# soycan-sim/bendy-tracer

Hardware: AMD Instinct MI355X
Metric: Msamples/s (pixels x spp / s) at 1080p (higher is better)
Workload: dtype f32; 1 GPU; C3: scene.json.gz 1920x1080x64spp Subsample::None, Config=main.rs (max_bounces 8, max_volume_bounces 32, clip 0.01..1000, volume_step 0.1, Output::Full), flat space (the reference has no lens code), seed 0x5EED; parallelism=single

## Files before the change

### bendy_tracer_amd/api.py

```python
from __future__ import annotations

import ctypes as C
import enum
import os
from dataclasses import dataclass
from typing import Optional

import numpy as np

_HERE = os.path.dirname(os.path.abspath(__file__))
LIB_PATH = os.path.join(_HERE, "libbendy_hip.so")
BT_TILE = 16


class BendyError(RuntimeError):

    def __init__(self, code, message):
        super().__init__(f"[bt_status {code}] {message}")
        self.code = code


class Output(enum.IntEnum):
    Full = 0
    Albedo = 1
    Normal = 2
    Depth = 3


class ColorSpace(enum.IntEnum):
    NONE = 0
    Normal = 1
    Linear = 2
    SRgb = 3


class Status(enum.IntEnum):
    Done = 0
    InProgress = 1


@dataclass(frozen=True)
class Subsample:
    n: int = 0

    @staticmethod
    def none():
        return Subsample(0)

    @staticmethod
    def subpixel(n):
        return Subsample(int(n))

    def subpixel_size(self):
        return 1.0 if self.n == 0 else float(np.float32(1.0) / np.float32(self.n))

    def subpixel_count(self):
        return 1 if self.n == 0 else self.n * self.n

    def __iter__(self):
        if self.n == 0:
            yield (0.0, 0.0)
            return
        w = np.float32(1.0) / np.float32(self.n)
        for c in range(self.n * self.n):
            yield (float(np.float32(c % self.n) * w), float(np.float32(c // self.n) * w))


@dataclass
class Config:
    max_bounces: int = 8
    max_volume_bounces: int = 32
    clip_min: float = 0.01
    clip_max: float = 1000.0
    volume_step: float = 0.1
    chunks_x: int = 4
    chunks_y: int = 2
    output: Output = Output.Full


@dataclass
class RenderConfig:
    subsample: Subsample = Subsample(0)
    samples: int = 64
    output: Optional[Output] = None
    max_bounces: Optional[int] = None
    max_volume_bounces: Optional[int] = None
    volume_step: Optional[float] = None

    @staticmethod
    def with_samples(samples):
        return RenderConfig(samples=samples)

    @staticmethod
    def with_samples_subsample(samples, subsample):
        return RenderConfig(samples=samples, subsample=subsample)


class _CConfig(C.Structure):
    _fields_ = [("max_bounces", C.c_uint32), ("max_volume_bounces", C.c_uint32), ("clip_min", C.c_float),
                ("clip_max", C.c_float), ("volume_step", C.c_float), ("chunks_x", C.c_uint32),
                ("chunks_y", C.c_uint32), ("output", C.c_int32)]


class _CRenderConfig(C.Structure):
    _fields_ = [("subsample_n", C.c_uint32), ("samples", C.c_uint32), ("has_output", C.c_int32),
                ("output", C.c_int32), ("has_max_bounces", C.c_int32), ("max_bounces", C.c_uint32),
                ("has_max_volume_bounces", C.c_int32), ("max_volume_bounces", C.c_uint32),
                ("has_volume_step", C.c_int32), ("volume_step", C.c_float), ("sample_base", C.c_uint32)]


class Stats(C.Structure):
    _fields_ = [("samples", C.c_uint64), ("segments", C.c_uint64), ("pixels", C.c_uint64), ("kernel_ms", C.c_float),
                ("lens_steps", C.c_uint64), ("slices", C.c_uint32), ("launches", C.c_uint32),
                ("scratch_bytes", C.c_uint64), ("parked_bytes", C.c_uint64), ("workgroups", C.c_uint32), ("packed", C.c_uint32)]


class _CTuning(C.Structure):
    _fields_ = [("slices", C.c_uint32), ("phase_vote", C.c_int32), ("scratch_cap_bytes", C.c_uint64), ("packed", C.c_int32),
                ("reserved", C.c_int32)]


class _CDenoiseParams(C.Structure):
    _fields_ = [("levels", C.c_uint32), ("sigma_color", C.c_float), ("sigma_normal", C.c_float), ("sigma_depth", C.c_float),
                ("eps_albedo", C.c_float)]


class _CAdaptiveParams(C.Structure):
    _fields_ = [("threshold", C.c_float), ("min_samples", C.c_uint32), ("max_samples", C.c_uint32), ("eps", C.c_float)]


class AdaptiveStats(C.Structure):
    _fields_ = [("active_tiles", C.c_uint32), ("tiles", C.c_uint32), ("min_count", C.c_uint32), ("max_count", C.c_uint32),
                ("pixel_samples", C.c_uint64), ("passes", C.c_uint32), ("reserved", C.c_uint32)]


class _CLens(C.Structure):
    _fields_ = [("centre", C.c_float * 3), ("rs", C.c_float), ("step", C.c_float), ("radius", C.c_float),
                ("max_steps", C.c_uint32)]


EXPORTS = [
    "bt_config_default", "bt_render_config_default", "bt_last_error", "bt_last_error_code", "bt_version", "bt_scene_load",
    "bt_scene_from_json", "bt_scene_free", "bt_scene_find_by_tag", "bt_scene_set_camera_aspect", "bt_scene_set_lens",
    "bt_scene_object_count", "bt_scene_data_count", "bt_scene_export_prims", "bt_render", "bt_render_device",
    "bt_shard_floats", "bt_render_shard_device", "bt_unshard_device", "bt_preview_device", "bt_preview",
    "bt_comm_unique_id", "bt_comm_init", "bt_comm_free", "bt_comm_rank", "bt_comm_world", "bt_allgather_shards_device",
    "bt_exchange_frame_device", "bt_scene_last_stats", "bt_tuning_default", "bt_scene_set_tuning", "bt_scene_get_tuning", "bt_scene_default", "bt_scene_to_json", "bt_scene_save", "bt_write_png",
    "bt_scene_trim", "bt_denoise_params_default", "bt_denoiser_new", "bt_denoiser_free", "bt_denoise_device",
    "bt_denoise", "bt_debug_primary_mask", "bt_debug_block_masks_device", "bt_debug_mask_key", "bt_debug_set_object",
    "bt_debug_plan_launch",
    "bt_render_guided_device", "bt_adaptive_params_default", "bt_adaptive_new", "bt_adaptive_free", "bt_adaptive_reset",
    "bt_render_adaptive_device", "bt_adaptive_poll", "bt_adaptive_counts", "bt_adaptive_errors", "bt_debug_adaptive_moments",
    "bt_adaptive_resolve_device",
]


def _load():
    if not os.path.exists(LIB_PATH):
        raise ImportError(
            f"{LIB_PATH} is missing: the HIP extension has not been built (run `python -c 'import __graft_entry__ "
            "as g; g.build()'` or `make -C bendy_tracer_amd/csrc`).  There is no CPU fallback.")
    try:
        import torch
    except ImportError:
        pass
    L = C.CDLL(LIB_PATH)
    vp, fp = C.c_void_p, C.POINTER(C.c_float)
    L.bt_last_error.restype = C.c_char_p
    L.bt_version.restype = C.c_char_p
    L.bt_config_default.argtypes = [C.POINTER(_CConfig)]
    L.bt_render_config_default.argtypes = [C.POINTER(_CRenderConfig)]
    L.bt_scene_load.restype = vp
    L.bt_scene_load.argtypes = [C.c_char_p]
    L.bt_scene_from_json.restype = vp
    L.bt_scene_from_json.argtypes = [C.c_char_p, C.c_size_t]
    L.bt_scene_free.argtypes = [vp]
    L.bt_scene_default.restype = vp
    L.bt_scene_to_json.argtypes = [vp, C.c_char_p, C.c_size_t]
    L.bt_scene_save.argtypes = [vp, C.c_char_p]
    L.bt_write_png.argtypes = [C.c_char_p, C.POINTER(C.c_uint8), C.c_uint32, C.c_uint32]
    L.bt_scene_find_by_tag.argtypes = [vp, C.c_char_p, C.POINTER(C.c_uint64)]
    L.bt_scene_set_camera_aspect.argtypes = [vp, C.c_uint64, C.c_float]
    L.bt_scene_set_lens.argtypes = [vp, C.POINTER(_CLens)]
    L.bt_scene_object_count.argtypes = [vp]
    L.bt_scene_data_count.argtypes = [vp]
    L.bt_scene_export_prims.argtypes = [vp, fp, C.c_int]
    L.bt_debug_primary_mask.argtypes = [vp, C.c_uint64, C.POINTER(_CConfig), C.POINTER(_CRenderConfig), C.c_uint32, C.c_uint32,
                                        C.c_uint32, C.c_uint32, C.c_uint32, C.POINTER(C.c_uint64), C.c_uint32]
    L.bt_debug_set_object.argtypes = [vp, C.c_uint64, fp, C.c_float]
    L.bt_debug_block_masks_device.argtypes = L.bt_debug_primary_mask.argtypes
    L.bt_debug_mask_key.argtypes = [vp, C.c_uint64, C.POINTER(_CConfig), C.POINTER(_CRenderConfig), C.c_uint32, C.c_uint32,
                                    C.c_uint32, C.c_uint32, C.c_uint32, C.POINTER(C.c_uint8), C.c_uint32]
    L.bt_debug_plan_launch.argtypes = [vp, C.c_uint64, C.POINTER(_CConfig), C.POINTER(_CRenderConfig), C.c_uint32, C.c_uint32,
                                       C.c_uint32, C.c_uint32, C.c_int32, C.c_uint32, C.c_int32, C.c_uint32, C.c_uint64,
                                       C.POINTER(Stats)]
    L.bt_render.argtypes = [vp, C.c_uint64, C.POINTER(_CConfig), C.POINTER(_CRenderConfig), fp, C.c_uint32,
                            C.c_uint32, C.c_uint64]
    L.bt_render_device.argtypes = [vp, C.c_uint64, C.POINTER(_CConfig), C.POINTER(_CRenderConfig), vp, C.c_uint32,
                                   C.c_uint32, C.c_uint64, vp]
    L.bt_render_guided_device.argtypes = [vp, C.c_uint64, C.POINTER(_CConfig), C.POINTER(_CRenderConfig), vp, vp, vp, vp,
                                          C.c_uint32, C.c_uint32, C.c_uint64, vp]
    L.bt_shard_floats.restype = C.c_size_t
    L.bt_shard_floats.argtypes = [C.c_uint32, C.c_uint32, C.c_uint32]
    L.bt_render_shard_device.argtypes = [vp, C.c_uint64, C.POINTER(_CConfig), C.POINTER(_CRenderConfig), vp,
                                         C.c_uint32, C.c_uint32, C.c_uint32, C.c_uint32, C.c_uint64, vp]
    L.bt_unshard_device.argtypes = [vp, vp, C.c_uint32, C.c_uint32, C.c_uint32, vp]
    L.bt_preview_device.argtypes = [vp, vp, C.c_uint32, C.c_uint32, C.c_uint32, C.c_int32, vp]
    L.bt_preview.argtypes = [fp, C.POINTER(C.c_uint8), C.c_uint32, C.c_uint32, C.c_uint32, C.c_int32]
    L.bt_scene_last_stats.argtypes = [vp, C.POINTER(Stats)]
    L.bt_comm_unique_id.argtypes = [C.c_void_p, C.c_size_t]
    L.bt_comm_init.restype = vp
    L.bt_comm_init.argtypes = [C.c_uint32, C.c_uint32, C.c_void_p, C.c_size_t]
    L.bt_comm_free.argtypes = [vp]
    L.bt_comm_rank.argtypes = [vp]
    L.bt_comm_world.argtypes = [vp]
    L.bt_allgather_shards_device.argtypes = [vp, vp, vp, C.c_uint32, C.c_uint32, vp]
    L.bt_exchange_frame_device.argtypes = [vp, vp, vp, vp, C.c_uint32, C.c_uint32, vp]
    L.bt_tuning_default.argtypes = [C.POINTER(_CTuning)]
    L.bt_scene_set_tuning.argtypes = [vp, C.POINTER(_CTuning)]
    L.bt_scene_get_tuning.argtypes = [vp, C.POINTER(_CTuning)]
    L.bt_scene_trim.argtypes = [vp]
    L.bt_denoise_params_default.argtypes = [C.POINTER(_CDenoiseParams)]
    L.bt_denoiser_new.restype = vp
    L.bt_denoiser_free.argtypes = [vp]
    L.bt_denoise_device.argtypes = [vp, vp, C.c_uint32, vp, C.c_uint32, vp, C.c_uint32, vp, C.c_uint32, vp, C.c_uint32,
                                    C.c_uint32, C.POINTER(_CDenoiseParams), vp]
    L.bt_denoise.argtypes = [vp, fp, C.c_uint32, fp, C.c_uint32, fp, C.c_uint32, fp, C.c_uint32, fp, C.c_uint32, C.c_uint32,
                             C.POINTER(_CDenoiseParams)]
    L.bt_adaptive_params_default.argtypes = [C.POINTER(_CAdaptiveParams)]
    L.bt_adaptive_new.restype = vp
    L.bt_adaptive_new.argtypes = [C.c_uint32, C.c_uint32]
    L.bt_adaptive_free.argtypes = [vp]
    L.bt_adaptive_reset.argtypes = [vp]
    L.bt_render_adaptive_device.argtypes = [vp, C.c_uint64, C.POINTER(_CConfig), C.POINTER(_CRenderConfig), vp,
                                            C.POINTER(_CAdaptiveParams), vp, C.c_uint32, C.c_uint32, C.c_uint64, vp]
    L.bt_adaptive_poll.argtypes = [vp, C.POINTER(AdaptiveStats)]
    L.bt_adaptive_counts.argtypes = [vp, C.POINTER(C.c_uint32), C.c_uint32]
    L.bt_adaptive_errors.argtypes = [vp, fp, C.c_uint32]
    L.bt_debug_adaptive_moments.argtypes = [vp, fp, C.c_uint32]
    L.bt_adaptive_resolve_device.argtypes = [vp, vp, vp, vp]
    return L


lib = _load()


def _check(rc):
    if rc < 0:
        raise BendyError(rc, lib.bt_last_error().decode("utf-8", "replace"))
    return rc


def _c_configs(config: Config, render: RenderConfig, sample_base: int):
    c = _CConfig(config.max_bounces, config.max_volume_bounces, config.clip_min, config.clip_max, config.volume_step,
                 config.chunks_x, config.chunks_y, int(config.output))
    r = _CRenderConfig()
    r.subsample_n = render.subsample.n
    r.samples = render.samples
    r.has_output = render.output is not None
    r.output = int(render.output) if render.output is not None else 0
    r.has_max_bounces = render.max_bounces is not None
    r.max_bounces = render.max_bounces or 0
    r.has_max_volume_bounces = render.max_volume_bounces is not None
    r.max_volume_bounces = render.max_volume_bounces or 0
    r.has_volume_step = render.volume_step is not None
    r.volume_step = render.volume_step or 0.0
    r.sample_base = sample_base
    return c, r


class Scene:

    def __init__(self, handle):
        if not handle:
            raise BendyError(lib.bt_last_error_code(), lib.bt_last_error().decode("utf-8", "replace"))
        self._h = C.c_void_p(handle)

    @classmethod
    def load(cls, path):
        return cls(lib.bt_scene_load(os.fspath(path).encode()))

    @classmethod
    def from_json(cls, text):
        data = text.encode() if isinstance(text, str) else bytes(text)
        return cls(lib.bt_scene_from_json(data, len(data)))

    @classmethod
    def default(cls):
        return cls(lib.bt_scene_default())

    def to_json(self) -> str:
        n = _check(lib.bt_scene_to_json(self._h, None, 0))
        buf = C.create_string_buffer(n + 1)
        _check(lib.bt_scene_to_json(self._h, buf, n + 1))
        return buf.value.decode()

    def save(self, path):
        _check(lib.bt_scene_save(self._h, os.fspath(path).encode()))

    def __del__(self):
        h = getattr(self, "_h", None)
        if h:
            lib.bt_scene_free(h)
            self._h = None

    def find_by_tag(self, tag) -> Optional[int]:
        ref = C.c_uint64()
        rc = lib.bt_scene_find_by_tag(self._h, tag.encode(), C.byref(ref))
        return ref.value if rc == 0 else None

    def set_camera_aspect(self, camera_ref, aspect_ratio):
        _check(lib.bt_scene_set_camera_aspect(self._h, camera_ref, aspect_ratio))

    def debug_set_object(self, object_ref, translation=None, radius=0.0):
        t = None if translation is None else (C.c_float * 3)(*[float(v) for v in translation])
        _check(lib.bt_debug_set_object(self._h, object_ref, t, float(radius)))

    def set_lens(self, centre, rs, step, radius, max_steps=4096):
        lens = _CLens((C.c_float * 3)(*[float(v) for v in centre]), rs, step, radius, max_steps)
        _check(lib.bt_scene_set_lens(self._h, C.byref(lens)))

    def clear_lens(self):
        _check(lib.bt_scene_set_lens(self._h, None))

    @property
    def object_count(self):
        return lib.bt_scene_object_count(self._h)

    @property
    def data_count(self):
        return lib.bt_scene_data_count(self._h)

    def export_prims(self):
        n = _check(lib.bt_scene_export_prims(self._h, None, 0))
        out = np.zeros(n, dtype=np.float32)
        _check(lib.bt_scene_export_prims(self._h, out.ctypes.data_as(C.POINTER(C.c_float)), n))
        return out.reshape(-1, 36)

    def set_tuning(self, **knobs):
        t = _CTuning()
        if not knobs:
            _check(lib.bt_scene_set_tuning(self._h, None))
            return
        _check(lib.bt_scene_get_tuning(self._h, C.byref(t)))
        for k, v in knobs.items():
            if not hasattr(t, k):
                raise TypeError(f"bt_tuning has no field {k!r}")
            setattr(t, k, int(v))
        _check(lib.bt_scene_set_tuning(self._h, C.byref(t)))

    def tuning(self) -> dict:
        t = _CTuning()
        _check(lib.bt_scene_get_tuning(self._h, C.byref(t)))
        return {k: getattr(t, k) for k, _ in _CTuning._fields_}

    def tuning_from_env(self, environ=None):
        env = os.environ if environ is None else environ
        names = {"BT_SLICES": "slices", "BT_PHASE_VOTE": "phase_vote", "BT_SCRATCH_CAP": "scratch_cap_bytes", "BT_PACKED": "packed"}
        knobs = {f: int(env[e]) for e, f in names.items() if env.get(e) not in (None, "", "-")}
        if knobs:
            self.set_tuning(**knobs)
        return knobs

    def trim(self):
        _check(lib.bt_scene_trim(self._h))

    def last_stats(self) -> Stats:
        st = Stats()
        _check(lib.bt_scene_last_stats(self._h, C.byref(st)))
        return st


class Buffer:

    def __init__(self, width, height, color_space=ColorSpace.SRgb, device="cuda"):
        self.width, self.height = int(width), int(height)
        self.color_space = ColorSpace(color_space)
        self.samples = 0
        self.device = device
        if device == "cpu":
            self.data = np.zeros((self.height, self.width, 4), dtype=np.float32)
            self.data[..., 3] = 1.0
        else:
            import torch
            self.data = torch.zeros((self.height, self.width, 4), dtype=torch.float32, device=device)
            self.data[..., 3] = 1.0

    @classmethod
    def new(cls, width, height, color_space=ColorSpace.SRgb, device="cuda"):
        return cls(width, height, color_space, device)

    def dimensions(self):
        return (self.width, self.height)

    def pixel_width(self):
        return float(np.float32(2.0) * (np.float32(1.0) / np.float32(self.width)))

    def pixel_height(self):
        return float(np.float32(2.0) * (np.float32(1.0) / np.float32(self.height)))

    def clear(self):
        self.data[...] = 0.0
        self.data[..., 3] = 1.0
        self.samples = 0

    def inc_samples(self, n):
        self.samples += n

    def chunks(self, chunks_x, chunks_y):
        cw = self.width // chunks_x + (1 if self.width % chunks_x else 0)
        ch = self.height // chunks_y + (1 if self.height % chunks_y else 0)
        out, oy = [], 0
        while oy < self.height:
            h = min(ch, self.height - oy)
            ox = 0
            while ox < self.width:
                w = min(cw, self.width - ox)
                out.append((ox, oy, ox + w, oy + h))
                ox += w
            oy += h
        return out

    def numpy(self):
        return self.data if self.device == "cpu" else self.data.cpu().numpy()

    def mean(self):
        return self.numpy()[..., :3] / np.float32(max(self.samples, 1))

    def preview(self):
        if self.device == "cpu":
            out = np.zeros((self.height, self.width, 4), dtype=np.uint8)
            _check(lib.bt_preview(self.data.ctypes.data_as(C.POINTER(C.c_float)),
                                  out.ctypes.data_as(C.POINTER(C.c_uint8)), self.width, self.height,
                                  max(self.samples, 1), int(self.color_space)))
            return out
        import torch
        out = torch.empty((self.height, self.width, 4), dtype=torch.uint8, device=self.data.device)
        _check(lib.bt_preview_device(self.data.data_ptr(), out.data_ptr(), self.width, self.height,
                                     max(self.samples, 1), int(self.color_space),
                                     torch.cuda.current_stream().cuda_stream))
        return out.cpu().numpy()


class Tracer:

    DEFAULT_SEED = 0x5EED

    def __init__(self, config: Optional[Config] = None):
        self.config = config or Config()

    @classmethod
    def new(cls):
        return cls()

    @classmethod
    def with_config(cls, config):
        return cls(config)

    def render(self, scene: Scene, camera: int, config: RenderConfig, buffer: Buffer, seed: Optional[int] = None,
               sample_base: Optional[int] = None) -> Status:
        seed = self.DEFAULT_SEED if seed is None else seed
        nn = config.subsample.subpixel_count()
        if sample_base is None:
            sample_base = (buffer.samples + nn - 1) // nn
        c, r = _c_configs(self.config, config, sample_base)
        if buffer.device == "cpu":
            rc = lib.bt_render(scene._h, camera, C.byref(c), C.byref(r),
                               buffer.data.ctypes.data_as(C.POINTER(C.c_float)), buffer.width, buffer.height, seed)
        else:
            import torch
            rc = lib.bt_render_device(scene._h, camera, C.byref(c), C.byref(r), buffer.data.data_ptr(), buffer.width,
                                      buffer.height, seed, torch.cuda.current_stream().cuda_stream)
        _check(rc)
        if rc == Status.InProgress:
            buffer.inc_samples(config.samples * nn)
        return Status(rc)

    def render_guided(self, scene: Scene, camera: int, config: RenderConfig, color: Buffer, albedo: Optional[Buffer] = None,
                      normal: Optional[Buffer] = None, depth: Optional[Buffer] = None, seed: Optional[int] = None,
                      sample_base: Optional[int] = None) -> Status:
        seed = self.DEFAULT_SEED if seed is None else seed
        output = config.output if config.output is not None else self.config.output
        if int(output) != int(Output.Full):
            raise BendyError(-1, f"render_guided renders Output.Full plus its guides, not output {int(output)}")
        guides = [albedo, normal, depth]
        for b in [color] + [g for g in guides if g is not None]:
            if b.device == "cpu":
                raise BendyError(-1, "render_guided needs device-resident buffers (there is no host-buffer variant)")
            if (b.width, b.height) != (color.width, color.height):
                raise BendyError(-1, f"buffer of {b.width}x{b.height} next to a {color.width}x{color.height} colour buffer")
        nn = config.subsample.subpixel_count()
        if sample_base is None:
            sample_base = (color.samples + nn - 1) // nn
        c, r = _c_configs(self.config, config, sample_base)
        import torch
        rc = lib.bt_render_guided_device(scene._h, camera, C.byref(c), C.byref(r), color.data.data_ptr(),
                                         *[g.data.data_ptr() if g is not None else None for g in guides], color.width,
                                         color.height, seed, torch.cuda.current_stream().cuda_stream)
        _check(rc)
        if rc == Status.InProgress:
            for b in [color] + [g for g in guides if g is not None]:
                b.inc_samples(config.samples * nn)
        return Status(rc)

    def render_adaptive(self, scene: Scene, camera: int, config: RenderConfig, buffer: Buffer, adaptive: "Adaptive",
                        seed: Optional[int] = None) -> Status:
        seed = self.DEFAULT_SEED if seed is None else seed
        if buffer.device == "cpu":
            raise BendyError(-1, "render_adaptive needs a device-resident buffer (there is no host-buffer variant)")
        c, r = _c_configs(self.config, config, 0)
        p = adaptive.params._c()
        import torch
        rc = _check(lib.bt_render_adaptive_device(scene._h, camera, C.byref(c), C.byref(r), adaptive._h, C.byref(p),
                                                  buffer.data.data_ptr(), buffer.width, buffer.height, seed,
                                                  torch.cuda.current_stream().cuda_stream))
        if rc == Status.Done:
            return Status.Done
        return Status(_check(lib.bt_adaptive_poll(adaptive._h, None)))

    def primary_masks(self, scene: Scene, camera: int, config: RenderConfig, width, height, slices, rank=0, world=1):
        c, r = _c_configs(self.config, config, 0)
        n = _check(lib.bt_debug_primary_mask(scene._h, camera, C.byref(c), C.byref(r), width, height, slices, rank, world,
                                             None, 0))
        out = np.zeros(n, dtype=np.uint64)
        _check(lib.bt_debug_primary_mask(scene._h, camera, C.byref(c), C.byref(r), width, height, slices, rank, world,
                                         out.ctypes.data_as(C.POINTER(C.c_uint64)), n))
        return out

    def block_masks_device(self, scene: Scene, camera: int, config: RenderConfig, width, height, slices, rank=0, world=1):
        c, r = _c_configs(self.config, config, 0)
        n = _check(lib.bt_debug_block_masks_device(scene._h, camera, C.byref(c), C.byref(r), width, height, slices, rank,
                                                   world, None, 0))
        out = np.zeros(n, dtype=np.uint64)
        _check(lib.bt_debug_block_masks_device(scene._h, camera, C.byref(c), C.byref(r), width, height, slices, rank, world,
                                               out.ctypes.data_as(C.POINTER(C.c_uint64)), n))
        return out

    def mask_key(self, scene: Scene, camera: int, config: RenderConfig, width, height, slices, rank=0, world=1) -> bytes:
        c, r = _c_configs(self.config, config, 0)
        n = _check(lib.bt_debug_mask_key(scene._h, camera, C.byref(c), C.byref(r), width, height, slices, rank, world, None, 0))
        out = (C.c_uint8 * n)()
        _check(lib.bt_debug_mask_key(scene._h, camera, C.byref(c), C.byref(r), width, height, slices, rank, world, out, n))
        return bytes(out)

    def plan_launch(self, scene: Scene, camera: int, config: RenderConfig, width, height, n_cu, rank=0, world=1, sharded=False,
                    kind=0, guides=0, alloc_limit=0) -> Stats:
        c, r = _c_configs(self.config, config, 0)
        st = Stats()
        _check(lib.bt_debug_plan_launch(scene._h, camera, C.byref(c), C.byref(r), width, height, rank, world, int(sharded),
                                        n_cu, kind, guides, alloc_limit, C.byref(st)))
        return st

    def render_shard(self, scene: Scene, camera: int, config: RenderConfig, shard, width, height, rank, world,
                     seed: Optional[int] = None, sample_base: int = 0) -> Status:
        import torch
        seed = self.DEFAULT_SEED if seed is None else seed
        c, r = _c_configs(self.config, config, sample_base)
        assert shard.numel() == shard_floats(width, height, world) and shard.dtype == torch.float32
        rc = lib.bt_render_shard_device(scene._h, camera, C.byref(c), C.byref(r), shard.data_ptr(), width, height, rank,
                                        world, seed, torch.cuda.current_stream().cuda_stream)
        return Status(_check(rc))


class Comm:

    ID_BYTES = 128

    @staticmethod
    def unique_id() -> bytes:
        buf = C.create_string_buffer(Comm.ID_BYTES)
        _check(lib.bt_comm_unique_id(buf, Comm.ID_BYTES))
        return buf.raw

    def __init__(self, rank, world, uid: bytes):
        assert len(uid) == self.ID_BYTES
        h = lib.bt_comm_init(rank, world, uid, len(uid))
        if not h:
            raise BendyError(lib.bt_last_error_code(), lib.bt_last_error().decode("utf-8", "replace"))
        self._h = C.c_void_p(h)
        self.rank, self.world = rank, world

    def close(self):
        if getattr(self, "_h", None):
            lib.bt_comm_free(self._h)
            self._h = None

    __del__ = close

    def allgather(self, shard, gathered, width, height):
        import torch
        assert gathered.numel() == self.world * shard.numel() == self.world * shard_floats(width, height, self.world)
        _check(lib.bt_allgather_shards_device(self._h, shard.data_ptr(), gathered.data_ptr(), width, height,
                                              torch.cuda.current_stream().cuda_stream))

    def exchange(self, shard, gathered, buffer: "Buffer"):
        import torch
        _check(lib.bt_exchange_frame_device(self._h, shard.data_ptr(), gathered.data_ptr(), buffer.data.data_ptr(),
                                            buffer.width, buffer.height, torch.cuda.current_stream().cuda_stream))


@dataclass
class DenoiseParams:
    levels: int = 2
    sigma_color: float = 16.0
    sigma_normal: float = 16.0
    sigma_depth: float = 1.0
    eps_albedo: float = 1e-3

    def _c(self):
        return _CDenoiseParams(int(self.levels), self.sigma_color, self.sigma_normal, self.sigma_depth, self.eps_albedo)


class Denoiser:

    def __init__(self):
        h = lib.bt_denoiser_new()
        if not h:
            raise BendyError(-1, "bt_denoiser_new failed")
        self._h = C.c_void_p(h)

    def close(self):
        if getattr(self, "_h", None):
            lib.bt_denoiser_free(self._h)
            self._h = None

    __del__ = close

    def denoise(self, color: Buffer, albedo: Optional[Buffer] = None, normal: Optional[Buffer] = None,
                depth: Optional[Buffer] = None, *, out: Optional[Buffer] = None, **params) -> Buffer:
        p = DenoiseParams(**params)
        bufs = [b for b in (albedo, normal, depth) if b is not None]
        for b in bufs + ([out] if out is not None else []):
            if (b.width, b.height) != (color.width, color.height):
                raise BendyError(-1, f"buffer of {b.width}x{b.height} next to a {color.width}x{color.height} colour buffer")
            if b.device != color.device or (color.device != "cpu" and b.data.device != color.data.device):
                raise BendyError(-1, f"buffer on {b.device} next to a colour buffer on {color.device}")
        if out is not None and any(out is b or out.data is b.data for b in [color] + bufs):
            raise BendyError(-1, "out must not be one of the inputs: the inputs are running sums, out is a mean")
        if out is None:
            out = Buffer(color.width, color.height, color.color_space, device=color.device)
        out.color_space = color.color_space

        def arg(b):
            if b is None:
                return None, 0
            if b.device == "cpu":
                return b.data.ctypes.data_as(C.POINTER(C.c_float)), b.samples
            return b.data.data_ptr(), b.samples

        args = []
        for b in (color, albedo, normal, depth):
            args += list(arg(b))
        cp = p._c()
        if color.device == "cpu":
            _check(lib.bt_denoise(self._h, *args, arg(out)[0], color.width, color.height, C.byref(cp)))
        else:
            import torch
            _check(lib.bt_denoise_device(self._h, *args, out.data.data_ptr(), color.width, color.height, C.byref(cp),
                                         torch.cuda.current_stream().cuda_stream))
        out.samples = 1
        return out


def _adaptive_defaults():
    p = _CAdaptiveParams()
    lib.bt_adaptive_params_default(C.byref(p))
    return p


@dataclass
class AdaptiveParams:
    threshold: Optional[float] = None
    min_samples: Optional[int] = None
    max_samples: Optional[int] = None
    eps: Optional[float] = None

    def __post_init__(self):
        d = _adaptive_defaults()
        for k, _ in _CAdaptiveParams._fields_:
            if getattr(self, k) is None:
                setattr(self, k, getattr(d, k))

    def _c(self):
        return _CAdaptiveParams(float(self.threshold), int(self.min_samples), int(self.max_samples), float(self.eps))


class Adaptive:

    def __init__(self, width, height, **params):
        self.params = AdaptiveParams(**params)
        self.width, self.height = int(width), int(height)
        self.tiles_x, self.tiles_y = (self.width + BT_TILE - 1) // BT_TILE, (self.height + BT_TILE - 1) // BT_TILE
        h = lib.bt_adaptive_new(self.width, self.height)
        if not h:
            raise BendyError(lib.bt_last_error_code(), lib.bt_last_error().decode("utf-8", "replace"))
        self._h = C.c_void_p(h)

    def close(self):
        if getattr(self, "_h", None):
            lib.bt_adaptive_free(self._h)
            self._h = None

    __del__ = close

    def reset(self):
        _check(lib.bt_adaptive_reset(self._h))

    def poll(self) -> AdaptiveStats:
        st = AdaptiveStats()
        _check(lib.bt_adaptive_poll(self._h, C.byref(st)))
        return st

    def counts(self):
        n = _check(lib.bt_adaptive_counts(self._h, None, 0))
        out = np.zeros(n, dtype=np.uint32)
        _check(lib.bt_adaptive_counts(self._h, out.ctypes.data_as(C.POINTER(C.c_uint32)), n))
        return out.reshape(self.tiles_y, self.tiles_x)

    def errors(self):
        n = _check(lib.bt_adaptive_errors(self._h, None, 0))
        out = np.zeros(n, dtype=np.float32)
        _check(lib.bt_adaptive_errors(self._h, out.ctypes.data_as(C.POINTER(C.c_float)), n))
        return out.reshape(self.tiles_y, self.tiles_x)

    def moments(self):
        n = _check(lib.bt_debug_adaptive_moments(self._h, None, 0))
        out = np.zeros(n, dtype=np.float32)
        _check(lib.bt_debug_adaptive_moments(self._h, out.ctypes.data_as(C.POINTER(C.c_float)), n))
        return out.reshape(self.height, self.width)

    def resolve(self, buffer: Buffer, out: Optional[Buffer] = None) -> Buffer:
        if buffer.device == "cpu":
            raise BendyError(-1, "resolve needs a device-resident buffer")
        if (buffer.width, buffer.height) != (self.width, self.height):
            raise BendyError(-1, f"buffer of {buffer.width}x{buffer.height} on an adaptive handle of {self.width}x{self.height}")
        if out is not None and (out is buffer or out.data is buffer.data):
            raise BendyError(-1, "out must not be the input: the input holds running sums, out is a mean")
        if out is None:
            out = Buffer(buffer.width, buffer.height, buffer.color_space, device=buffer.device)
        if (out.width, out.height) != (self.width, self.height) or out.device == "cpu":
            raise BendyError(-1, "out must be a device-resident buffer of the handle's size")
        out.color_space = buffer.color_space
        import torch
        _check(lib.bt_adaptive_resolve_device(self._h, buffer.data.data_ptr(), out.data.data_ptr(),
                                              torch.cuda.current_stream().cuda_stream))
        out.samples = 1
        return out


_default_denoiser = None


def denoise(color: Buffer, albedo: Optional[Buffer] = None, normal: Optional[Buffer] = None, depth: Optional[Buffer] = None,
            *, out: Optional[Buffer] = None, **params) -> Buffer:
    global _default_denoiser
    if _default_denoiser is None:
        _default_denoiser = Denoiser()
    return _default_denoiser.denoise(color, albedo, normal, depth, out=out, **params)


def write_png(path, rgba8):
    a = np.ascontiguousarray(rgba8, dtype=np.uint8)
    _check(lib.bt_write_png(os.fspath(path).encode(), a.ctypes.data_as(C.POINTER(C.c_uint8)), a.shape[1], a.shape[0]))


def shard_floats(width, height, world):
    return lib.bt_shard_floats(width, height, world)


def new_shard(width, height, world, device="cuda"):
    import torch
    s = torch.zeros(shard_floats(width, height, world), dtype=torch.float32, device=device)
    s.view(-1, 4)[:, 3] = 1.0
    return s


def unshard(gathered, buffer: Buffer, world):
    import torch
    _check(lib.bt_unshard_device(gathered.data_ptr(), buffer.data.data_ptr(), buffer.width, buffer.height, world,
                                 torch.cuda.current_stream().cuda_stream))


def tile_owner_map(width, height, world):
    tx, ty = (width + BT_TILE - 1) // BT_TILE, (height + BT_TILE - 1) // BT_TILE
    return (np.arange(tx * ty) % world).reshape(ty, tx)
```

### bendy_tracer_amd/csrc/bt_api.cpp

```cpp
#include <hip/hip_runtime.h>

#include <algorithm>
#include <cmath>
#include <cstdlib>
#include <cstdio>
#include <cstring>
#include <memory>
#include <string>

#include "../../include/bendy_hip.h"
#include "bt_internal.hpp"
#include "bt_scene.hpp"
#include "bt_types.h"
#include "bt_cull.hpp"
#include "bt_plan.hpp"

#pragma STDC FP_CONTRACT OFF

namespace {

thread_local std::string g_error;
thread_local int g_error_code = 0;
constexpr uint32_t kCounterSlots = 64;

template <class T> struct DeviceArray {
    T *ptr = nullptr;
    size_t count = 0;
    ~DeviceArray() { release(); }
    size_t bytes() const { return sizeof(T) * count; }
    void release() {
        if (ptr) (void)hipFree(ptr);
        ptr = nullptr;
        count = 0;
    }
    hipError_t allocate(size_t n) {
        release();
        hipError_t e = hipMalloc((void **)&ptr, sizeof(T) * n);
        if (e == hipSuccess) count = n;
        return e;
    }
    hipError_t upload(const std::vector<T> &src) {
        hipError_t e = allocate(src.size() ? src.size() : 1);
        count = src.size();
        if (e == hipSuccess && count) e = hipMemcpy(ptr, src.data(), sizeof(T) * count, hipMemcpyHostToDevice);
        return e;
    }
};

}

struct bt_scene {
    bt::Scene scene;
    std::string source;
    bt::FlatScene flat;
    bool flat_valid = false;
    bool device_valid = false;
    int device = -1;
    DeviceArray<BtPrim> d_prims;
    DeviceArray<BtMaterial> d_materials;
    DeviceArray<BtVolume> d_volumes;
    DeviceArray<BtLight> d_lights;
    DeviceArray<BtLightFace> d_light_faces;
    DeviceArray<BtSpherePair> d_sphere_pairs;
    DeviceArray<BtSphereRow> d_sphere_rows;
    DeviceArray<BtRectAAN> d_aan_rows;
    DeviceArray<BtRectLA> d_la_rows;
    DeviceArray<int32_t> d_other_rows;
    DeviceArray<float> d_density;
    DeviceArray<int32_t> d_lens_prims;
    bt_lens lens_prims_for{};
    bool lens_prims_valid = false;
    unsigned long long *d_counters = nullptr;
    uint32_t render_seq = 0;
    uint32_t last_slot = 0;
    DeviceArray<float> d_scratch;
    uint32_t scratch_small_streak = 0;
    btplan::Scratch plan_scratch;
    DeviceArray<uint64_t> d_block_masks;
    btcull::MaskKey masks_for{};
    uint64_t rows_generation = 0;
    DeviceArray<float> d_host_frame;
    int n_cu = 0;
    bt_tuning tuning{};
    hipEvent_t ev_start = nullptr, ev_stop = nullptr;
    bt_stats last{};
    bool lens_on = false;
    bt_lens lens{};
    bool stats_pending = false;

    bt_scene() { bt_tuning_default(&tuning); }
    void release_device_state() {
        if (d_counters) (void)hipFree(d_counters);
        if (ev_start) (void)hipEventDestroy(ev_start);
        if (ev_stop) (void)hipEventDestroy(ev_stop);
        d_counters = nullptr;
        ev_start = ev_stop = nullptr;
        stats_pending = false;
        release_buffers();
    }
    void release_buffers() {
        d_scratch.release();
        d_host_frame.release();
        d_block_masks.release();
        masks_for = btcull::MaskKey{};
        scratch_small_streak = 0;
    }
    ~bt_scene() { release_device_state(); }
};

namespace {

int ensure_flat(bt_scene *s) {
    if (s->flat_valid) return 0;
    try {
        s->flat = bt::flatten_scene(s->scene);
    } catch (const bt::Error &e) {
        return fail(e.code, e.message);
    }
    s->flat_valid = true;
    s->device_valid = false;
    s->rows_generation += 1;
    return 0;
}

std::vector<BtSphereRow> sphere_rows_of(const std::vector<BtPrim> &pr) {
    std::vector<BtSphereRow> rows;
    bool spheres_only = true;
    for (const BtPrim &R : pr) spheres_only = spheres_only && (R.kind & BT_PRIM_SHAPE_MASK) == BT_PRIM_SPHERE;
    if (spheres_only)
        for (const BtPrim &R : pr) rows.push_back(BtSphereRow{R.c.x, R.c.y, R.c.z, R.radius * R.radius});
    if (rows.size() & 1) rows.push_back(rows.back());
    return rows;
}

int ensure_device(bt_scene *s) {
    int rc = ensure_flat(s);
    if (rc) return rc;
    int dev = -1;
    BT_HIP(hipGetDevice(&dev));
    if (s->device_valid && s->device == dev) return 0;
    if (s->device >= 0 && s->device != dev) {
        (void)hipSetDevice(s->device);
        s->release_device_state();
        BT_HIP(hipSetDevice(dev));
    }
    {
        hipDeviceProp_t prop;
        BT_HIP(hipGetDeviceProperties(&prop, dev));
        s->n_cu = prop.multiProcessorCount > 0 ? prop.multiProcessorCount : 256;
    }
    BT_HIP(s->d_prims.upload(s->flat.prims));
    BT_HIP(s->d_materials.upload(s->flat.materials));
    BT_HIP(s->d_volumes.upload(s->flat.volumes));
    BT_HIP(s->d_lights.upload(s->flat.lights));
    BT_HIP(s->d_light_faces.upload(s->flat.light_faces));
    {
        std::vector<BtSpherePair> pairs;
        const std::vector<BtPrim> &pr = s->flat.prims;
        bool spheres_only = true;
        for (const BtPrim &R : pr) spheres_only = spheres_only && (R.kind & BT_PRIM_SHAPE_MASK) == BT_PRIM_SPHERE;
        if (spheres_only)
            for (size_t i = 0; i < pr.size(); i += 2) {
                const BtPrim &A = pr[i], &B = pr[i + 1 < pr.size() ? i + 1 : i];
                BtSpherePair q{};
                q.cx[0] = A.c.x; q.cy[0] = A.c.y; q.cz[0] = A.c.z; q.radius[0] = A.radius; q.object[0] = A.object;
                q.cx[1] = B.c.x; q.cy[1] = B.c.y; q.cz[1] = B.c.z; q.radius[1] = B.radius; q.object[1] = B.object;
                pairs.push_back(q);
            }
        BT_HIP(s->d_sphere_pairs.upload(pairs));
        BT_HIP(s->d_sphere_rows.upload(sphere_rows_of(pr)));
        s->rows_generation += 1;
    }
    BT_HIP(s->d_density.upload(s->flat.density));
    BT_HIP(s->d_aan_rows.upload(s->flat.aan_rows));
    BT_HIP(s->d_la_rows.upload(s->flat.la_rows));
    BT_HIP(s->d_other_rows.upload(s->flat.other_rows));
    if (!s->d_counters) {
        BT_HIP(hipMalloc((void **)&s->d_counters, kCounterSlots * 16 * sizeof(unsigned long long)));
        s->render_seq = 0;
    }
    if (!s->ev_start) BT_HIP(hipEventCreate(&s->ev_start));
    if (!s->ev_stop) BT_HIP(hipEventCreate(&s->ev_stop));
    s->device = dev;
    s->device_valid = true;
    s->lens_prims_valid = false;
    return 0;
}

std::vector<int32_t> lens_candidates(const std::vector<BtPrim> &prims, const bt_lens &lens, double reach) {
    std::vector<int32_t> rows;
    const double cx = lens.centre[0], cy = lens.centre[1], cz = lens.centre[2];
    reach *= 1.001;
    for (size_t i = 0; i < prims.size(); ++i) {
        const BtPrim &R = prims[i];
        bool near_ = true;
        if ((R.kind & BT_PRIM_SHAPE_MASK) == BT_PRIM_SPHERE) {
            const double d = std::sqrt((R.c.x - cx) * (R.c.x - cx) + (R.c.y - cy) * (R.c.y - cy) + (R.c.z - cz) * (R.c.z - cz));
            near_ = std::fabs(d - (double)R.radius) <= reach + 1e-3 * (double)R.radius;
        } else {
            const double a[3][3] = {{R.icx.x, R.icy.x, R.icz.x}, {R.icx.y, R.icy.y, R.icz.y}, {R.icx.z, R.icy.z, R.icz.z}};
            const double det = a[0][0] * (a[1][1] * a[2][2] - a[1][2] * a[2][1]) - a[0][1] * (a[1][0] * a[2][2] - a[1][2] * a[2][0]) +
                               a[0][2] * (a[1][0] * a[2][1] - a[1][1] * a[2][0]);
            if (std::isfinite(det) && std::fabs(det) > 1e-30) {
                double m[3][3];
                for (int r = 0; r < 3; ++r)
                    for (int c = 0; c < 3; ++c) {
                        const int r1 = (c + 1) % 3, r2 = (c + 2) % 3, c1 = (r + 1) % 3, c2 = (r + 2) % 3;
                        m[r][c] = (a[r1][c1] * a[r2][c2] - a[r1][c2] * a[r2][c1]) / det;
                    }
                const double hw = std::sqrt((double)R.w_sqr), hh = std::sqrt((double)R.h_sqr);
                double lx[3] = {R.ax.x, R.ax.y, R.ax.z}, ly[3] = {R.ay.x, R.ay.y, R.ay.z};
                if ((R.kind & BT_PRIM_SHAPE_MASK) == BT_PRIM_RECT_LA || (R.kind & BT_PRIM_SHAPE_MASK) == BT_PRIM_RECT_AAN)
                    for (int i = 0; i < 3; ++i) {
                        lx[i] = i == R.aa_u ? 1.0 : 0.0;
                        ly[i] = i == R.aa_v ? 1.0 : 0.0;
                    }
                double bound = 0.0;
                for (int sx = -1; sx <= 1; sx += 2)
                    for (int sy = -1; sy <= 1; sy += 2) {
                        const double l[3] = {sx * hw * lx[0] + sy * hh * ly[0], sx * hw * lx[1] + sy * hh * ly[1],
                                             sx * hw * lx[2] + sy * hh * ly[2]};
                        double wv[3];
                        for (int r = 0; r < 3; ++r) wv[r] = m[r][0] * l[0] + m[r][1] * l[1] + m[r][2] * l[2];
                        bound = std::max(bound, std::sqrt(wv[0] * wv[0] + wv[1] * wv[1] + wv[2] * wv[2]));
                    }
                const double d = std::sqrt((R.t.x - cx) * (R.t.x - cx) + (R.t.y - cy) * (R.t.y - cy) + (R.t.z - cz) * (R.t.z - cz));
                near_ = d - bound * 1.001 <= reach;
            }
        }
        if (near_) rows.push_back((int32_t)i);
    }
    return rows;
}

int fill_launch(bt_scene *s, uint64_t camera_ref, const bt_config *cfg, const bt_render_config *rc, uint32_t width,
                uint32_t height, uint64_t seed, BtLaunch &P, int &output) {
    if (!s || !cfg || !rc) return fail(BT_ERR_INVALID_ARG, "null argument");
    if (width == 0 || height == 0) return fail(BT_ERR_INVALID_ARG, "zero-sized buffer");
    int ci = s->scene.object_index(camera_ref);
    if (ci < 0) return fail(BT_ERR_INVALID_REF, "invalid object ref " + std::to_string(camera_ref));
    const bt::Object &cam = s->scene.objects[ci];
    if (cam.kind != bt::OBJ_CAMERA) return fail(BT_ERR_NOT_CAMERA, "expected a camera object");

    std::memset(&P, 0, sizeof P);
    const bt::FlatScene &f = s->flat;
    P.prims = s->d_prims.ptr;
    P.materials = s->d_materials.ptr;
    P.volumes = s->d_volumes.ptr;
    P.lights = s->d_lights.ptr;
    P.light_faces = s->d_light_faces.ptr;
    P.sphere_pairs = s->d_sphere_pairs.count ? s->d_sphere_pairs.ptr : nullptr;
    P.sphere_rows = s->d_sphere_rows.count ? s->d_sphere_rows.ptr : nullptr;
    P.density = s->d_density.ptr;
    P.n_prims = (int32_t)f.prims.size();
    P.n_materials = (int32_t)f.materials.size();
    P.n_volumes = (int32_t)f.volumes.size();
    P.n_lights = (int32_t)f.lights.size();
    P.n_light_faces = (int32_t)f.light_faces.size();
    P.n_density = (int32_t)f.density.size();
    P.any_rects = 0;
    for (const BtPrim &R : f.prims)
        if ((R.kind & BT_PRIM_SHAPE_MASK) != BT_PRIM_SPHERE) P.any_rects = 1;
    P.any_volumes = btplan::any_prim_carries_volume(f.prims) ? 1 : 0;
    P.aan_rows = s->d_aan_rows.ptr;
    P.la_rows = s->d_la_rows.ptr;
    P.n_la = (int32_t)f.la_rows.size();
    P.other_rows = s->d_other_rows.ptr;
    P.n_aan[0] = f.n_aan[0]; P.n_aan[1] = f.n_aan[1]; P.n_aan[2] = f.n_aan[2];
    P.n_other = (int32_t)f.other_rows.size();
    P.root_color = f.root_color;
    P.root_albedo = f.root_albedo;
    P.root_has_albedo = f.root_has_albedo;

    P.cam_cx = cam.world.cx; P.cam_cy = cam.world.cy; P.cam_cz = cam.world.cz; P.cam_t = cam.world.t;
    P.yfov = 2.0f * atan2f(cam.sensor_size, 2.0f * cam.focal_length);
    P.xfov = P.yfov * cam.aspect_ratio;
    P.pixel_width = 2.0f * (1.0f / (float)width);
    P.pixel_height = 2.0f * (1.0f / (float)height);
    const uint32_t n = rc->subsample_n >= 2 ? rc->subsample_n : 1;
    const float subpixel_scale = rc->subsample_n >= 2 ? 1.0f / (float)rc->subsample_n : 1.0f;
    const float umin = -0.5f * P.pixel_width * subpixel_scale, umax = 0.5f * P.pixel_width * subpixel_scale;
    const float vmin = -0.5f * P.pixel_height * subpixel_scale, vmax = 0.5f * P.pixel_height * subpixel_scale;
    P.jitter_u_lo = umin;
    P.jitter_u_scale = bt::uniform_scale(umin, umax, false);
    P.jitter_v_lo = vmin;
    P.jitter_v_scale = bt::uniform_scale(vmin, vmax, false);
    P.has_focus = cam.has_focus ? 1 : 0;
    P.focus = cam.focus;
    P.aperture = 0.5f * cam.focal_length / cam.fstop;
    BtV3 neg_z; neg_z.x = 0.0f; neg_z.y = 0.0f; neg_z.z = -1.0f;
    bt::orthonormal_pair(neg_z, P.disk_x, P.disk_y);
    P.tau_scale = bt::uniform_scale(0.0f, 6.28318530717958647692f, true);
    P.one_scale = bt::uniform_scale(0.0f, 1.0f, true);

    output = rc->has_output ? rc->output : cfg->output;
    if (output < 0 || output > 3) return fail(BT_ERR_INVALID_ARG, "invalid output mode");
    P.max_bounces = (int32_t)(rc->has_max_bounces ? rc->max_bounces : cfg->max_bounces);
    P.max_volume_bounces = (int32_t)(rc->has_max_bounces ? rc->max_bounces : cfg->max_volume_bounces);
    P.clip_min = cfg->clip_min;
    P.clip_max = cfg->clip_max;
    P.volume_step = rc->has_volume_step ? rc->volume_step : cfg->volume_step;
    if (P.any_rects && !P.any_volumes &&
        !(P.clip_min >= 0x1p-30f && P.clip_max <= 0x1p60f && f.prims.size() < 0x7fffu))
        P.any_volumes = 1;
    if (rc->samples > 0x7fffffffu / (n * n)) return fail(BT_ERR_INVALID_ARG, "samples * n^2 overflows");
    P.samples = (int32_t)rc->samples;
    P.subsample_n = (int32_t)n;
    P.sample_base = rc->sample_base;
    P.seed_lo = (uint32_t)seed;
    P.seed_hi = (uint32_t)(seed >> 32);
    P.width = width;
    P.height = height;
    P.tiles_x = btplan::tiles_across(width);
    P.tiles_x_magic = P.tiles_x == 1 ? 0xffffffffu : (uint32_t)(0x100000000ull / P.tiles_x);
    P.tiles_y = btplan::tiles_across(height);
    P.rank = 0;
    P.world = 1;
    P.sharded = 0;
    P.counters = s->d_counters;
    P.lens_on = s->lens_on ? 1 : 0;
    P.lens_c.x = s->lens.centre[0]; P.lens_c.y = s->lens.centre[1]; P.lens_c.z = s->lens.centre[2];
    P.lens_rs = s->lens.rs;
    P.lens_step = s->lens.step;
    P.lens_radius = s->lens.radius;
    P.lens_max_steps = (int32_t)s->lens.max_steps;
    P.lens_prims = nullptr;
    P.n_lens_prims = 0;
    P.lens_margin = s->lens_on ? 3.0f * s->lens.step : 0.0f;
    return 0;
}

int upload_lens_prims(bt_scene *s, BtLaunch &P) {
    if (!s->lens_on) return 0;
    if (!s->lens_prims_valid || std::memcmp(&s->lens_prims_for, &s->lens, sizeof(bt_lens)) != 0) {
        BT_HIP(s->d_lens_prims.upload(lens_candidates(s->flat.prims, s->lens, (double)s->lens.radius + (double)P.lens_margin)));
        s->lens_prims_for = s->lens;
        s->lens_prims_valid = true;
    }
    P.lens_prims = s->d_lens_prims.ptr;
    P.n_lens_prims = (int32_t)s->d_lens_prims.count;
    return 0;
}

int ensure_block_masks(bt_scene *s, BtLaunch &P, uint32_t n_blocks, hipStream_t stream) {
    btcull::MaskKey key;
    btcull::mask_key(key, P, n_blocks, s->rows_generation, (const void *)stream);
    if (!bt_mask_cache_enabled() || std::memcmp(&key, &s->masks_for, sizeof key) != 0) {
        if (s->d_block_masks.count < n_blocks) {
            if (s->d_block_masks.ptr) BT_HIP(hipDeviceSynchronize());
            s->masks_for = btcull::MaskKey{};
            BT_HIP(s->d_block_masks.allocate(n_blocks));
        }
        s->masks_for = btcull::MaskKey{};
        BT_HIP(bt_launch_block_masks(&P, n_blocks, s->d_block_masks.ptr, stream));
        s->masks_for = key;
    }
    P.block_masks = s->d_block_masks.ptr;
    return 0;
}

uint64_t realloc_scratch(bt_scene *s, hipStream_t stream, uint64_t need) {
    if (s->d_scratch.ptr && hipStreamSynchronize(stream) != hipSuccess) return s->d_scratch.bytes();
    s->d_scratch.release();
    if (need && s->d_scratch.allocate(need / sizeof(float)) != hipSuccess) (void)hipGetLastError();
    return s->d_scratch.bytes();
}

struct RenderPass {
    int kind = btplan::PLAIN;
    float *guides[3] = {nullptr, nullptr, nullptr};
    const uint32_t *tile_active = nullptr;
    float *moment = nullptr;
    uint32_t guide_mask() const { return (guides[0] ? 1u : 0u) | (guides[1] ? 2u : 0u) | (guides[2] ? 4u : 0u); }
};

int render_common(bt_scene *s, uint64_t camera_ref, const bt_config *cfg, const bt_render_config *rc, float *out_device,
                  uint32_t width, uint32_t height, uint32_t rank, uint32_t world, bool sharded, uint64_t seed,
                  hipStream_t stream, const RenderPass &pass = RenderPass{}) {
    if (!s || !cfg || !rc || !out_device) return fail(BT_ERR_INVALID_ARG, "null argument");
    if (rc->samples == 0) return BT_DONE;
    if (world == 0 || rank >= world) return fail(BT_ERR_INVALID_ARG, "rank/world out of range");
    int rcode = ensure_device(s);
    if (rcode) return rcode;
    BtLaunch P;
    int output = 0;
    rcode = fill_launch(s, camera_ref, cfg, rc, width, height, seed, P, output);
    if (rcode) return rcode;
    rcode = upload_lens_prims(s, P);
    if (rcode) return rcode;
    btplan::shard_launch(P, rank, world, sharded);
    P.out = out_device;

    btplan::Plan plan;
    btplan::Scratch held{s->d_scratch.bytes(), s->scratch_small_streak};
    rcode = btplan::plan_launch(P, output, s->flat, s->tuning, (uint32_t)s->n_cu, pass.kind, pass.guide_mask(), held,
                                [&](uint64_t need) { return realloc_scratch(s, stream, need); }, plan);
    s->scratch_small_streak = held.small_streak;
    if (rcode) return fail(rcode, plan.error);
    P.scratch = s->d_scratch.ptr;
    for (int g = 0; g < 3; ++g) {
        P.guide_out[g] = plan.output == 4 ? pass.guides[g] : nullptr;
        P.guide_scratch[g] = plan.guide_values[g] ? P.scratch + plan.guide_values[g] : nullptr;
    }
    P.tile_active = pass.tile_active;
    P.moment = pass.moment;

    s->last_slot = s->render_seq % kCounterSlots;
    if (s->last_slot == 0) BT_HIP(hipMemsetAsync(s->d_counters, 0, kCounterSlots * 16 * sizeof(unsigned long long), stream));
    s->render_seq += 1;
    P.counters = s->d_counters + (size_t)s->last_slot * 16;
    BT_HIP(hipEventRecord(s->ev_start, stream));
    P.block_masks = nullptr;
    if (bt_launch_reads_masks(&P, plan.output)) {
        rcode = ensure_block_masks(s, P, plan.grid * (uint32_t)P.slices, stream);
        if (rcode) return rcode;
    }
    {
        const uint32_t all = (uint32_t)P.samples, base = P.sample_base;
        for (uint32_t done = 0; done < all; done += plan.chunk) {
            P.samples = (int32_t)std::min(plan.chunk, all - done);
            P.sample_base = base + done;
            BT_HIP(bt_launch_render(&P, plan.output, plan.grid, plan.lds_bytes, stream));
        }
        P.samples = (int32_t)all;
        P.sample_base = base;
    }
    BT_HIP(hipEventRecord(s->ev_stop, stream));

    btplan::plan_stats(P, plan, held, s->last);
    s->stats_pending = true;
    return BT_IN_PROGRESS;
}

}

extern "C" {

void bt_config_default(bt_config *c) {
    if (!c) return;
    c->max_bounces = 8;
    c->max_volume_bounces = 32;
    c->clip_min = 0.01f;
    c->clip_max = 1000.0f;
    c->volume_step = 0.1f;
    c->chunks_x = 4;
    c->chunks_y = 2;
    c->output = BT_OUTPUT_FULL;
}

void bt_render_config_default(bt_render_config *r) {
    if (!r) return;
    std::memset(r, 0, sizeof *r);
    r->samples = 64;
}

const char *bt_last_error(void) { return g_error.c_str(); }
int bt_set_error_internal(int code, const char *msg) {
    g_error = msg ? msg : "";
    g_error_code = code;
    return code;
}
int bt_last_error_code(void) { return g_error_code; }

void bt_tuning_default(bt_tuning *t) {
    if (!t) return;
    std::memset(t, 0, sizeof *t);
    t->phase_vote = -1;
    t->packed = -1;
}

int bt_scene_set_tuning(bt_scene *scene, const bt_tuning *t) {
    if (!scene) return fail(BT_ERR_INVALID_ARG, "null scene");
    if (!t) {
        bt_tuning_default(&scene->tuning);
        return 0;
    }
    const uint32_t S = t->slices;
    if (!(S == 0 || S == 1 || S == 2 || S == 4 || S == 8 || S == 16 || S == 32))
        return fail(BT_ERR_INVALID_ARG, "bt_tuning.slices must be 0 (auto), 1, 2, 4, 8, 16 or 32");
    if (t->phase_vote < -1 || t->phase_vote > 64)
        return fail(BT_ERR_INVALID_ARG, "bt_tuning.phase_vote must be -1 .. 64");
    if (t->packed < -1 || t->packed > 2) return fail(BT_ERR_INVALID_ARG, "bt_tuning.packed must be -1, 0, 1 or 2");
    scene->tuning = *t;
    return 0;
}

int bt_scene_get_tuning(const bt_scene *scene, bt_tuning *out) {
    if (!scene || !out) return fail(BT_ERR_INVALID_ARG, "null argument");
    *out = scene->tuning;
    return 0;
}

const char *bt_version(void) { return "bendy-hip 0.1 (gfx950)"; }

bt_scene *bt_scene_from_json(const char *json, size_t len) {
    if (!json) {
        fail(BT_ERR_INVALID_ARG, "null json");
        return nullptr;
    }
    try {
        std::unique_ptr<bt_scene> s(new bt_scene());
        s->scene = bt::parse_scene(json, len);
        s->source.assign(json, len);
        return s.release();
    } catch (const bt::Error &e) {
        fail(e.code, e.message);
    } catch (const std::exception &e) {
        fail(BT_ERR_PARSE, e.what());
    }
    return nullptr;
}

bt_scene *bt_scene_load(const char *path) {
    if (!path) {
        fail(BT_ERR_INVALID_ARG, "null path");
        return nullptr;
    }
    try {
        std::string text = bt::read_scene_file(path);
        return bt_scene_from_json(text.data(), text.size());
    } catch (const bt::Error &e) {
        fail(e.code, e.message);
    } catch (const std::exception &e) {
        fail(BT_ERR_IO, e.what());
    }
    return nullptr;
}

bt_scene *bt_scene_default(void) {
    std::string text = bt::default_scene_json();
    return bt_scene_from_json(text.data(), text.size());
}

void bt_scene_free(bt_scene *scene) { delete scene; }

int bt_scene_to_json(const bt_scene *scene, char *out, size_t cap) {
    if (!scene) return fail(BT_ERR_INVALID_ARG, "null scene");
    try {
        std::string text = bt::scene_to_pretty_json(scene->scene, scene->source);
        if (out && cap > 0) {
            size_t n = std::min(cap - 1, text.size());
            std::memcpy(out, text.data(), n);
            out[n] = 0;
        }
        return (int)text.size();
    } catch (const bt::Error &e) {
        return fail(e.code, e.message);
    } catch (const std::exception &e) {
        return fail(BT_ERR_PARSE, e.what());
    }
}

int bt_scene_save(const bt_scene *scene, const char *path) {
    if (!scene || !path) return fail(BT_ERR_INVALID_ARG, "null argument");
    try {
        bt::write_text_file(path, bt::scene_to_pretty_json(scene->scene, scene->source));
        return 0;
    } catch (const bt::Error &e) {
        return fail(e.code, e.message);
    } catch (const std::exception &e) {
        return fail(BT_ERR_IO, e.what());
    }
}

int bt_write_png(const char *path, const uint8_t *rgba8, uint32_t width, uint32_t height) {
    if (!path || !rgba8 || width == 0 || height == 0) return fail(BT_ERR_INVALID_ARG, "invalid argument");
    try {
        bt::write_png(path, rgba8, width, height);
        return 0;
    } catch (const bt::Error &e) {
        return fail(e.code, e.message);
    }
}

int bt_scene_find_by_tag(const bt_scene *scene, const char *tag, uint64_t *object_ref) {
    if (!scene || !tag || !object_ref) return fail(BT_ERR_INVALID_ARG, "null argument");
    for (const bt::Object &o : scene->scene.objects)
        if (o.has_tag && o.tag == tag) {
            *object_ref = o.object_ref;
            return 0;
        }
    return fail(BT_ERR_INVALID_REF, std::string("no object tagged `") + tag + "`");
}

int bt_scene_set_camera_aspect(bt_scene *scene, uint64_t camera_ref, float aspect_ratio) {
    if (!scene) return fail(BT_ERR_INVALID_ARG, "null scene");
    int i = scene->scene.object_index(camera_ref);
    if (i < 0) return fail(BT_ERR_INVALID_REF, "invalid object ref " + std::to_string(camera_ref));
    if (scene->scene.objects[i].kind != bt::OBJ_CAMERA) return fail(BT_ERR_NOT_CAMERA, "expected a camera object");
    scene->scene.objects[i].aspect_ratio = aspect_ratio;
    return 0;
}

int bt_scene_set_lens(bt_scene *scene, const bt_lens *lens) {
    if (!scene) return fail(BT_ERR_INVALID_ARG, "null scene");
    if (!lens) {
        scene->lens_on = false;
        return 0;
    }
    if (!(lens->rs >= 0.0f) || !(lens->step > 0.0f) || !(lens->radius > lens->rs) || lens->max_steps == 0 ||
        lens->max_steps > 0x7fffffffu)
        return fail(BT_ERR_INVALID_ARG, "lens needs rs >= 0, step > 0, radius > rs, max_steps > 0");
    scene->lens = *lens;
    scene->lens_on = true;
    return 0;
}

int bt_scene_object_count(const bt_scene *scene) { return scene ? (int)scene->scene.objects.size() : 0; }
int bt_scene_data_count(const bt_scene *scene) { return scene ? (int)scene->scene.data.size() : 0; }

int bt_scene_export_prims(const bt_scene *scene, float *out, int cap) {
    if (!scene) return fail(BT_ERR_INVALID_ARG, "null scene");
    bt_scene *s = const_cast<bt_scene *>(scene);
    int rc = ensure_flat(s);
    if (rc) return rc;
    const size_t words = sizeof(BtPrim) / 4;
    const int total = (int)(s->flat.prims.size() * words);
    if (out && cap > 0) std::memcpy(out, s->flat.prims.data(), sizeof(float) * (size_t)std::min(cap, total));
    return total;
}

int bt_debug_set_object(bt_scene *scene, uint64_t object_ref, const float *translation, float radius) {
    if (!scene) return fail(BT_ERR_INVALID_ARG, "null scene");
    const int i = scene->scene.object_index(object_ref);
    if (i < 0) return fail(BT_ERR_INVALID_REF, "invalid object ref " + std::to_string(object_ref));
    bt::Object &o = scene->scene.objects[i];
    if (translation) { o.world.t.x = translation[0]; o.world.t.y = translation[1]; o.world.t.z = translation[2]; }
    if (radius > 0.0f && o.kind == bt::OBJ_SPHERE) o.radius = radius;
    scene->flat_valid = false;
    return 0;
}

static int debug_mask_launch(bt_scene *scene, uint64_t camera_ref, const bt_config *config, const bt_render_config *render,
                             uint32_t width, uint32_t height, uint32_t slices, uint32_t rank, uint32_t world, BtLaunch &P) {
    if (!scene || !config || !render) return fail(BT_ERR_INVALID_ARG, "null argument");
    if (slices == 0 || slices > 32 || (slices & (slices - 1)) != 0) return fail(BT_ERR_INVALID_ARG, "slices must be 1, 2, 4, ..., 32");
    if (world == 0 || rank >= world) return fail(BT_ERR_INVALID_ARG, "rank/world out of range");
    int rc = ensure_flat(scene);
    if (rc) return rc;
    int output = 0;
    rc = fill_launch(scene, camera_ref, config, render, width, height, 0, P, output);
    if (rc) return rc;
    const uint32_t grid = btplan::shard_launch(P, rank, world, world > 1);
    P.slices = (int32_t)slices;
    const uint64_t n_blocks = (uint64_t)grid * slices;
    if (n_blocks > 0x7fffffffu) return fail(BT_ERR_INVALID_ARG, "too many blocks");
    return (int)n_blocks;
}

int bt_debug_primary_mask(bt_scene *scene, uint64_t camera_ref, const bt_config *config, const bt_render_config *render,
                          uint32_t width, uint32_t height, uint32_t slices, uint32_t rank, uint32_t world, uint64_t *masks,
                          uint32_t cap) {
    BtLaunch P;
    const int n_blocks = debug_mask_launch(scene, camera_ref, config, render, width, height, slices, rank, world, P);
    if (n_blocks < 0) return n_blocks;
    if (masks && cap > 0) {
        const std::vector<BtSphereRow> rows = sphere_rows_of(scene->flat.prims);
        std::vector<uint64_t> all((size_t)n_blocks, ~0ull);
        if (P.any_rects == 0 && P.any_volumes == 0) bt_primary_masks_host(&P, rows.data(), (uint32_t)n_blocks, all.data());
        std::memcpy(masks, all.data(), sizeof(uint64_t) * (size_t)std::min<uint64_t>(cap, (uint64_t)n_blocks));
    }
    return n_blocks;
}

int bt_debug_block_masks_device(bt_scene *scene, uint64_t camera_ref, const bt_config *config, const bt_render_config *render,
                                uint32_t width, uint32_t height, uint32_t slices, uint32_t rank, uint32_t world,
                                uint64_t *masks, uint32_t cap) {
    BtLaunch P;
    int n_blocks = debug_mask_launch(scene, camera_ref, config, render, width, height, slices, rank, world, P);
    if (n_blocks < 0) return n_blocks;
    if (!masks || cap == 0) return n_blocks;
    if (P.any_rects || P.any_volumes) return fail(BT_ERR_INVALID_ARG, "the scene does not run the build that reads block masks");
    int rc = ensure_device(scene);
    if (rc) return rc;
    n_blocks = debug_mask_launch(scene, camera_ref, config, render, width, height, slices, rank, world, P);
    if (n_blocks < 0) return n_blocks;
    uint64_t *d = nullptr;
    BT_HIP(hipMalloc((void **)&d, sizeof(uint64_t) * (size_t)n_blocks));
    hipError_t e = bt_launch_block_masks(&P, (uint32_t)n_blocks, d, nullptr);
    if (e == hipSuccess)
        e = hipMemcpy(masks, d, sizeof(uint64_t) * (size_t)std::min<uint32_t>(cap, (uint32_t)n_blocks), hipMemcpyDeviceToHost);
    (void)hipFree(d);
    if (e != hipSuccess) return fail(BT_ERR_DEVICE, hipGetErrorString(e));
    return n_blocks;
}

int bt_debug_mask_key(bt_scene *scene, uint64_t camera_ref, const bt_config *config, const bt_render_config *render,
                      uint32_t width, uint32_t height, uint32_t slices, uint32_t rank, uint32_t world, uint8_t *out,
                      uint32_t cap) {
    BtLaunch P;
    const int n_blocks = debug_mask_launch(scene, camera_ref, config, render, width, height, slices, rank, world, P);
    if (n_blocks < 0) return n_blocks;
    btcull::MaskKey key;
    P.sphere_rows = nullptr;
    btcull::mask_key(key, P, (uint32_t)n_blocks, scene->rows_generation, nullptr);
    if (out && cap > 0) std::memcpy(out, &key, std::min<size_t>(cap, sizeof key));
    return (int)sizeof key;
}

int bt_debug_plan_launch(bt_scene *scene, uint64_t camera_ref, const bt_config *config, const bt_render_config *render,
                         uint32_t width, uint32_t height, uint32_t rank, uint32_t world, int32_t sharded, uint32_t n_cu,
                         int32_t pass_kind, uint32_t guides, uint64_t alloc_limit, bt_stats *out) {
    if (!scene || !config || !render || !out) return fail(BT_ERR_INVALID_ARG, "null argument");
    if (world == 0 || rank >= world) return fail(BT_ERR_INVALID_ARG, "rank/world out of range");
    if (n_cu == 0 || render->samples == 0 || pass_kind < btplan::PLAIN || pass_kind > btplan::ADAPTIVE)
        return fail(BT_ERR_INVALID_ARG, "bt_debug_plan_launch: n_cu and samples must not be 0, pass_kind is 0, 1 or 2");
    int rc = ensure_flat(scene);
    if (rc) return rc;
    BtLaunch P;
    int output = 0;
    rc = fill_launch(scene, camera_ref, config, render, width, height, 0, P, output);
    if (rc) return rc;
    if (pass_kind != btplan::PLAIN && (output != BT_OUTPUT_FULL || scene->lens_on))
        return fail(BT_ERR_INVALID_ARG, "a guided or adaptive pass renders the Full output without the lens");
    btplan::shard_launch(P, rank, world, sharded != 0);
    btplan::Plan plan;
    btplan::Scratch &held = scene->plan_scratch;
    rc = btplan::plan_launch(P, output, scene->flat, scene->tuning, n_cu, pass_kind, guides, held,
                             [&](uint64_t need) -> uint64_t { return alloc_limit == 0 || need <= alloc_limit ? need : 0; }, plan);
    if (rc) return fail(rc, plan.error);
    btplan::plan_stats(P, plan, held, *out);
    out->lens_steps = 0;
    return 0;
}

int bt_render_device(bt_scene *scene, uint64_t camera_ref, const bt_config *config, const bt_render_config *render,
                     float *rgba_device, uint32_t width, uint32_t height, uint64_t seed, void *stream) {
    return render_common(scene, camera_ref, config, render, rgba_device, width, height, 0, 1, false, seed,
                         (hipStream_t)stream);
}

int bt_render_adaptive_pass_internal(bt_scene *scene, uint64_t camera_ref, const bt_config *config, const bt_render_config *render,
                                     float *rgba_device, uint32_t width, uint32_t height, uint64_t seed, void *stream,
                                     const uint32_t *tile_active, float *moment) {
    RenderPass pass;
    pass.kind = btplan::ADAPTIVE;
    pass.tile_active = tile_active;
    pass.moment = moment;
    return render_common(scene, camera_ref, config, render, rgba_device, width, height, 0, 1, false, seed, (hipStream_t)stream, pass);
}
int bt_scene_lens_on_internal(const bt_scene *scene) { return scene && scene->lens_on ? 1 : 0; }

int bt_render_guided_device(bt_scene *scene, uint64_t camera_ref, const bt_config *config, const bt_render_config *render,
                            float *color_device, float *albedo_device, float *normal_device, float *depth_device,
                            uint32_t width, uint32_t height, uint64_t seed, void *stream) {
    if (!scene || !config || !render || !color_device) return fail(BT_ERR_INVALID_ARG, "null argument");
    const int output = render->has_output ? render->output : config->output;
    if (output != BT_OUTPUT_FULL)
        return fail(BT_ERR_INVALID_ARG, "a guided render is the Full output plus its guides: the effective output must be BT_OUTPUT_FULL");
    float *const frames[4] = {color_device, albedo_device, normal_device, depth_device};
    for (int i = 0; i < 4; ++i)
        for (int j = i + 1; j < 4; ++j)
            if (frames[i] && frames[i] == frames[j]) return fail(BT_ERR_INVALID_ARG, "two frames of a guided render are the same buffer");
    if (scene->lens_on) return fail(BT_ERR_UNSUPPORTED, "the lens extension has no guided builds");
    if (render->samples == 0) return BT_DONE;
    RenderPass pass;
    pass.kind = btplan::GUIDED;
    for (int g = 0; g < 3; ++g) pass.guides[g] = frames[g + 1];
    return render_common(scene, camera_ref, config, render, color_device, width, height, 0, 1, false, seed, (hipStream_t)stream, pass);
}

int bt_render(bt_scene *scene, uint64_t camera_ref, const bt_config *config, const bt_render_config *render,
              float *rgba_host, uint32_t width, uint32_t height, uint64_t seed) {
    if (!scene) return fail(BT_ERR_INVALID_ARG, "null scene");
    if (!rgba_host) return fail(BT_ERR_INVALID_ARG, "null buffer");
    if (render && render->samples == 0) return BT_DONE;
    if (width == 0 || height == 0) return fail(BT_ERR_INVALID_ARG, "zero-sized buffer");
    int rc = ensure_device(scene);
    if (rc) return rc;
    const size_t bytes = (size_t)width * height * 4 * sizeof(float);
    const size_t held = scene->d_host_frame.bytes();
    if (held < bytes || held / 4 > bytes) {
        if (scene->d_host_frame.ptr) BT_HIP(hipDeviceSynchronize());
        BT_HIP(scene->d_host_frame.allocate(bytes / sizeof(float)));
    }
    float *d = scene->d_host_frame.ptr;
    BT_HIP(hipMemcpyAsync(d, rgba_host, bytes, hipMemcpyHostToDevice, nullptr));
    rc = bt_render_device(scene, camera_ref, config, render, d, width, height, seed, nullptr);
    if (rc < 0) return rc;
    BT_HIP(hipMemcpy(rgba_host, d, bytes, hipMemcpyDeviceToHost));
    return rc;
}

size_t bt_shard_floats(uint32_t width, uint32_t height, uint32_t world) {
    if (world == 0) return 0;
    const size_t per_rank = btplan::tiles_per_rank(btplan::frame_tiles(width, height), world);
    return per_rank * BT_TILE * BT_TILE * 4;
}

int bt_render_shard_device(bt_scene *scene, uint64_t camera_ref, const bt_config *config,
                           const bt_render_config *render, float *shard_device, uint32_t width, uint32_t height,
                           uint32_t rank, uint32_t world, uint64_t seed, void *stream) {
    return render_common(scene, camera_ref, config, render, shard_device, width, height, rank, world, true, seed,
                         (hipStream_t)stream);
}

int bt_unshard_device(const float *gathered_device, float *rgba_device, uint32_t width, uint32_t height, uint32_t world,
                      void *stream) {
    if (!gathered_device || !rgba_device || world == 0 || width == 0 || height == 0)
        return fail(BT_ERR_INVALID_ARG, "invalid argument");
    const uint32_t tiles_x = btplan::tiles_across(width), tiles_y = btplan::tiles_across(height);
    const uint32_t per_rank = btplan::tiles_per_rank(tiles_x * tiles_y, world);
    BT_HIP(bt_launch_unshard(gathered_device, rgba_device, width, height, tiles_x, tiles_y, world, per_rank,
                             (hipStream_t)stream));
    return 0;
}

int bt_preview_device(const float *rgba_device, uint8_t *rgba8_device, uint32_t width, uint32_t height, uint32_t samples,
                      int32_t color_space, void *stream) {
    if (!rgba_device || !rgba8_device || width == 0 || height == 0)
        return fail(BT_ERR_INVALID_ARG, "invalid argument");
    BT_HIP(bt_launch_preview(rgba_device, rgba8_device, width * height, samples, color_space, (hipStream_t)stream));
    return 0;
}

int bt_preview(const float *rgba_host, uint8_t *rgba8_host, uint32_t width, uint32_t height, uint32_t samples,
               int32_t color_space) {
    if (!rgba_host || !rgba8_host || width == 0 || height == 0) return fail(BT_ERR_INVALID_ARG, "invalid argument");
    const size_t n = (size_t)width * height;
    float *d_in = nullptr;
    uint8_t *d_out = nullptr;
    BT_HIP(hipMalloc((void **)&d_in, n * 16));
    hipError_t e = hipMalloc((void **)&d_out, n * 4);
    int rc = 0;
    if (e == hipSuccess) e = hipMemcpy(d_in, rgba_host, n * 16, hipMemcpyHostToDevice);
    if (e == hipSuccess) rc = bt_preview_device(d_in, d_out, width, height, samples, color_space, nullptr);
    if (e == hipSuccess && rc == 0) e = hipMemcpy(rgba8_host, d_out, n * 4, hipMemcpyDeviceToHost);
    (void)hipFree(d_in);
    if (d_out) (void)hipFree(d_out);
    if (e != hipSuccess) return fail(BT_ERR_DEVICE, hipGetErrorString(e));
    return rc;
}

int bt_scene_trim(bt_scene *scene) {
    if (!scene) return fail(BT_ERR_INVALID_ARG, "null scene");
    scene->plan_scratch = btplan::Scratch{};
    if (scene->device < 0 || (!scene->d_scratch.ptr && !scene->d_host_frame.ptr && !scene->d_block_masks.ptr)) return 0;
    int cur = -1;
    BT_HIP(hipGetDevice(&cur));
    if (cur != scene->device) BT_HIP(hipSetDevice(scene->device));
    BT_HIP(hipDeviceSynchronize());
    scene->release_buffers();
    if (cur != scene->device) BT_HIP(hipSetDevice(cur));
    return 0;
}

int bt_scene_last_stats(bt_scene *scene, bt_stats *out) {
    if (!scene || !out) return fail(BT_ERR_INVALID_ARG, "null argument");
    if (scene->stats_pending) {
        BT_HIP(hipEventSynchronize(scene->ev_stop));
        unsigned long long c[16] = {0, 0};
        BT_HIP(hipMemcpy(c, scene->d_counters + (size_t)scene->last_slot * 16, sizeof c, hipMemcpyDeviceToHost));
#ifdef BT_LANESTAT
        if (c[2]) {
            const double it = (double)c[2] * 64.0;
            fprintf(stderr, "[bt lanes] wave-iterations %llu; of 64 lanes per iteration: trace %.1f%% | camera %.1f%% diffuse %.1f%% metallic %.1f%% glass %.1f%% volume %.1f%% | waiting for phase %.1f%% | left the loop %.1f%%\n",
                    c[2], 100.0 * c[3] / it, 100.0 * c[4] / it, 100.0 * c[5] / it, 100.0 * c[6] / it, 100.0 * c[7] / it,
                    100.0 * c[8] / it, 100.0 * c[9] / it, 100.0 * c[10] / it);
        }
#elif defined(BT_PROFILE)
        {
            unsigned long long tot = 0;
            for (int i = 2; i < BT_N_COUNTERS; ++i) tot += c[i];
            fprintf(stderr, "[bt profile] section share of wave cycles:");
            for (int i = 2; i < BT_N_COUNTERS; ++i) fprintf(stderr, " s%d=%.1f%%", i - 2, tot ? 100.0 * (double)c[i] / (double)tot : 0.0);
            fprintf(stderr, "\n");
        }
#endif
        float ms = 0.0f;
        BT_HIP(hipEventElapsedTime(&ms, scene->ev_start, scene->ev_stop));
        scene->last.segments = c[0];
        scene->last.lens_steps = c[1];
        scene->last.kernel_ms = ms;
        scene->stats_pending = false;
    }
    *out = scene->last;
    return 0;
}

}
```

### bendy_tracer_amd/csrc/bt_kernels.hip

```cpp
#include "bt_device.hpp"
#include "bt_cull.hpp"
#include "bt_internal.hpp"

#define BT_SUM_BATCH 8

#ifdef BT_LANESTAT
#define BT_LS(i, mask) do { ls_acc[i] += (unsigned long long)__popcll(mask); } while (0)
#else
#define BT_LS(i, mask)
#endif
#ifdef BT_PROFILE
#define BT_PROF_DECL unsigned long long prof_t = __builtin_readcyclecounter(), prof_acc[BT_N_COUNTERS - 2] = {}
#define BT_PROF(i) do { const unsigned long long now_ = __builtin_readcyclecounter(); prof_acc[i] += now_ - prof_t; prof_t = now_; } while (0)
#else
#define BT_PROF_DECL
#define BT_PROF(i)
#endif

namespace {

struct Parked { float x, y, z; };
struct Parked1 { float x; };
BT_DEV V3 v3_of(const Parked &v) { return mk(v.x, v.y, v.z); }
BT_DEV V3 v3_of(const Parked1 &v) { return mk(v.x, v.x, v.x); }
BT_DEV V3 shfl_v3(const Parked &v, int from) { return mk(__shfl(v.x, from, 64), __shfl(v.y, from, 64), __shfl(v.z, from, 64)); }
BT_DEV V3 shfl_v3(const Parked1 &v, int from) { const float d = __shfl(v.x, from, 64); return mk(d, d, d); }

enum { EV_GEN = 0, EV_DIFFUSE = 1, EV_METALLIC = 2, EV_GLASS = 3, EV_VOLUME = 4 };

struct __attribute__((aligned(16))) PathRec { float f[12]; uint32_t w[8]; };

BT_DEV uint32_t lanes_below(unsigned long long m) {
    return __builtin_amdgcn_mbcnt_hi((uint32_t)(m >> 32), __builtin_amdgcn_mbcnt_lo((uint32_t)m, 0u));
}
struct PixelRef { uint32_t px, py; bool in_frame; };
BT_DEV PixelRef pixel_of(const BtLaunch &P, const BlockGeom &g, const BlockRef &B, uint32_t q) {
    PixelRef r;
    r.px = B.px0 + (q & g.WMASK) + ((q >> 3) & 8u);
    r.py = B.py0 + ((q & 63u) >> g.LBW) + ((q >> 4) & 8u);
    r.in_frame = B.tile_ok && r.px < P.width && r.py < P.height;
    return r;
}
BT_DEV float *out_of(const BtLaunch &P, float *frame, const BlockRef &B, const PixelRef &r) {
    return P.sharded ? frame + ((size_t)B.slot * (BT_TILE_DIM * BT_TILE_DIM) + (r.py & 15u) * BT_TILE_DIM + (r.px & 15u)) * 4
                     : frame + ((size_t)r.py * P.width + r.px) * 4;
}

BT_DEV float moment_add(float m, const V3 &v) {
    const float Y = (0.2126f * v.x + 0.7152f * v.y) + 0.0722f * v.z;
    return m + Y * Y;
}

template <class PK, bool MOMENT = false>
BT_DEV void sum_block(const BtLaunch &P, const BlockGeom &g, uint32_t b, uint32_t T, const PK *src, uint32_t lane, float *frame,
                      float *moment = nullptr) {
    const BlockRef B = block_ref(P, g, b);
    const uint32_t pxb = g.pxb;
    if (pxb >= 64) {
        for (uint32_t q = lane; q < pxb; q += 64) {
            const PixelRef r = pixel_of(P, g, B, q);
            if (!r.in_frame) continue;
            float *o = out_of(P, frame, B, r);
            const PK *s = src + q;
            V3 sum = mk(o[0], o[1], o[2]);
            float *mo = nullptr;
            float m = 0.0f;
            if constexpr (MOMENT) {
                mo = moment + ((size_t)r.py * P.width + r.px);
                m = *mo;
            }
            uint32_t kk = 0;
            for (; kk + BT_SUM_BATCH <= T; kk += BT_SUM_BATCH) {
                PK v[BT_SUM_BATCH];
#pragma unroll
                for (int j = 0; j < BT_SUM_BATCH; ++j) v[j] = s[(size_t)(kk + j) * pxb];
#pragma unroll
                for (int j = 0; j < BT_SUM_BATCH; ++j) {
                    sum = sum + v3_of(v[j]);
                    if constexpr (MOMENT) m = moment_add(m, v3_of(v[j]));
                }
            }
            for (; kk < T; ++kk) {
                const PK v = s[(size_t)kk * pxb];
                sum = sum + v3_of(v);
                if constexpr (MOMENT) m = moment_add(m, v3_of(v));
            }
            o[0] = sum.x;
            o[1] = sum.y;
            o[2] = sum.z;
            if constexpr (MOMENT) *mo = m;
        }
    } else {
        const uint32_t J = 64u >> g.LOG_PXB, q = lane & (pxb - 1u), jl = lane >> g.LOG_PXB;
        const PixelRef r = pixel_of(P, g, B, q);
        const bool owner = jl == 0 && r.in_frame;
        float *o = out_of(P, frame, B, r);
        const PK *s = src + q;
        V3 sum = mk(0.0f, 0.0f, 0.0f);
        if (owner) sum = mk(o[0], o[1], o[2]);
        float *mo = nullptr;
        float m = 0.0f;
        if constexpr (MOMENT) {
            mo = moment + ((size_t)r.py * P.width + r.px);
            if (owner) m = *mo;
        }
        for (uint32_t kk = 0; kk < T; kk += 8 * J) {
            PK v[8];
#pragma unroll
            for (int u = 0; u < 8; ++u) {
                const uint32_t k2 = kk + (uint32_t)u * J + jl;
                v[u] = k2 < T ? s[(size_t)k2 * pxb] : PK{};
            }
#pragma unroll
            for (int u = 0; u < 8; ++u)
                for (uint32_t jj = 0; jj < J; ++jj) {
                    const int from = (int)(q + jj * pxb);
                    const V3 val = shfl_v3(v[u], from);
                    if (kk + (uint32_t)u * J + jj < T) {
                        sum = sum + val;
                        if constexpr (MOMENT) m = moment_add(m, val);
                    }
                }
        }
        if (owner) {
            o[0] = sum.x;
            o[1] = sum.y;
            o[2] = sum.z;
            if constexpr (MOMENT) *mo = m;
        }
    }
}


template <class PK>
BT_DEV void sum_blocks(const BtLaunch &P, const BlockGeom &g, uint32_t first, uint32_t stride, uint32_t n, uint32_t T,
                       const PK *src, uint32_t thread, uint32_t n_threads, float *frame) {
    const uint32_t LOG_ROWS = P.log_rows;
    for (uint32_t p = thread; p < (n << g.LOG_PXB); p += n_threads) {
        const uint32_t j = p >> g.LOG_PXB, q = p & (g.pxb - 1u);
        const BlockRef B = block_ref(P, g, first + j * stride);
        const PixelRef r = pixel_of(P, g, B, q);
        if (!r.in_frame) continue;
        float *o = out_of(P, frame, B, r);
        const PK *s = src + ((size_t)j << (LOG_ROWS + g.LOG_PXB)) + q;
        V3 sum = mk(o[0], o[1], o[2]);
        uint32_t kk = 0;
        for (; kk + BT_SUM_BATCH <= T; kk += BT_SUM_BATCH) {
            PK v[BT_SUM_BATCH];
#pragma unroll
            for (int u = 0; u < BT_SUM_BATCH; ++u) v[u] = s[(size_t)(kk + u) << g.LOG_PXB];
#pragma unroll
            for (int u = 0; u < BT_SUM_BATCH; ++u) sum = sum + v3_of(v[u]);
        }
        for (; kk < T; ++kk) {
            const PK v = s[(size_t)kk << g.LOG_PXB];
            sum = sum + v3_of(v);
        }
        o[0] = sum.x;
        o[1] = sum.y;
        o[2] = sum.z;
    }
}

template <int OUTPUT> BT_DEV void fill_empty_block(const BtLaunch &P) {
    const BlockGeom G = block_geom(P);
    const BlockRef B_own = block_ref(P, G, blockIdx.x);
    const uint32_t T = (uint32_t)P.samples * (uint32_t)(P.subsample_n * P.subsample_n);
    uint32_t nx = 0, ny = 0;
    block_extent(P, G, B_own, nx, ny);
    V3 value;
    if (OUTPUT == 0) {
        value = mk(0, 0, 0) + mk(1, 1, 1) * mk(P.root_color);
    } else if (OUTPUT == 1) {
        value = mk(P.root_albedo);
    } else {
        const float fd = P.root_has_albedo ? P.clip_max : __builtin_inff();
        float depth = (fd - P.clip_min) / (P.clip_max - P.clip_min);
        depth = fminf(fmaxf(depth, 0.0f), 1.0f);
        value = mk(depth, depth, depth);
    }
    for (uint32_t q = threadIdx.x; q < G.pxb; q += blockDim.x) {
        const PixelRef r = pixel_of(P, G, B_own, q);
        if (!r.in_frame) continue;
        float *o = out_of(P, P.out, B_own, r);
        V3 sum = mk(o[0], o[1], o[2]);
        for (uint32_t k = 0; k < T; ++k) sum = sum + value;
        o[0] = sum.x;
        o[1] = sum.y;
        o[2] = sum.z;
    }
    if (P.counters && threadIdx.x == 0 && nx * ny != 0u) atomicAdd(&P.counters[0], (unsigned long long)(nx * ny) * T);
}

}

__global__ __launch_bounds__(256) void bt_block_mask_kernel(BtLaunch P, uint32_t n_blocks, unsigned long long *masks) {
    const uint32_t b = blockIdx.x * blockDim.x + threadIdx.x;
    if (b >= n_blocks) return;
    typedef const __attribute__((address_space(4))) BtSphereRow RowK;
    masks[b] = btcull::block_mask(P, (RowK *)P.sphere_rows, b);
}

#ifndef BT_WAVES_PER_SIMD
#define BT_WAVES_PER_SIMD 7
#endif
#ifndef BT_WAVES_PER_SIMD_VOLS
#define BT_WAVES_PER_SIMD_VOLS BT_WAVES_PER_SIMD
#endif
#ifndef BT_WAVES_PER_SIMD_RECTS
#define BT_WAVES_PER_SIMD_RECTS 7
#endif
#ifndef BT_WAVES_PER_SIMD_LENS
#define BT_WAVES_PER_SIMD_LENS 6
#endif
#ifndef BT_WAVES_PER_SIMD_GUIDED_RECTS
#define BT_WAVES_PER_SIMD_GUIDED_RECTS 7
#endif
#ifndef BT_SKIP_DIR
#define BT_SKIP_DIR 1
#endif
#ifndef BT_LENS_BATCH
#define BT_LENS_BATCH 8
#endif
template <int OUTPUT, bool LENS, bool RECTS, bool VOLS, bool PACKED>
__global__ __launch_bounds__(256, (OUTPUT == 4 && RECTS && !VOLS) ? BT_WAVES_PER_SIMD_GUIDED_RECTS : LENS ? BT_WAVES_PER_SIMD_LENS : (RECTS ? BT_WAVES_PER_SIMD_RECTS : (VOLS ? BT_WAVES_PER_SIMD_VOLS : BT_WAVES_PER_SIMD))) void bt_render_kernel(BtLaunch P) {
    constexpr bool GUIDED = OUTPUT == 4;
    constexpr bool ADAPT = OUTPUT == 5;
    constexpr bool AOV = OUTPUT != 0 && !ADAPT;
    constexpr bool CULL = !LENS && !RECTS && !VOLS && !PACKED && OUTPUT != 2 && !GUIDED && !ADAPT;
    if (ADAPT) {
        typedef const __attribute__((address_space(4))) BtLaunch BtLaunchK;
        typedef const __attribute__((address_space(4))) uint32_t ActiveK;
        BtLaunchK *C = (BtLaunchK *)__builtin_amdgcn_kernarg_segment_ptr();
        asm volatile("" : "+s"(C));
        const uint32_t slot = blockIdx.x >> (uint32_t)__builtin_ctz((uint32_t)C->slices);
        if (((ActiveK *)C->tile_active)[slot] == 0u) return;
    }
    if (CULL && P.max_bounces >= 0) {
        typedef const __attribute__((address_space(4))) unsigned long long MaskK;
        if (((MaskK *)P.block_masks)[blockIdx.x] == 0ull) {
            typedef const __attribute__((address_space(4))) BtLaunch BtLaunchK;
            BtLaunchK *C = (BtLaunchK *)__builtin_amdgcn_kernarg_segment_ptr();
            asm volatile("" : "+s"(C));
            fill_empty_block<OUTPUT>(*(const BtLaunch *)C);
            return;
        }
    }
    extern __shared__ __align__(16) unsigned char smem[];
    __shared__ uint32_t s_waves_done;
    __shared__ uint32_t s_next_item;
    __shared__ uint32_t s_segments;
    __shared__ uint32_t s_pool_paths[2], s_pool_waves[2];
    if (threadIdx.x == 0) {
        s_waves_done = 0;
        s_next_item = 0;
        s_segments = 0;
        if (PACKED && RECTS && !VOLS && OUTPUT == 0) s_pool_paths[0] = s_pool_paths[1] = s_pool_waves[0] = s_pool_waves[1] = 0;
    }

    SceneLds S;
    {
        unsigned char *p = smem;
        BtPrimLite *lite = (BtPrimLite *)p;        p += sizeof(BtPrimLite) * P.n_prims;
        BtMaterial *mats = (BtMaterial *)p;        p += sizeof(BtMaterial) * P.n_materials;
        BtVolume *vols = (BtVolume *)p;            p += sizeof(BtVolume) * P.n_volumes;
        BtLight *lights = (BtLight *)p;            p += sizeof(BtLight) * P.n_lights;
        BtLightFace *faces = (BtLightFace *)p;     p += sizeof(BtLightFace) * P.n_light_faces;
        float *dens = (float *)p;
        for (int i = threadIdx.x; i < P.n_prims; i += blockDim.x) {
            const BtPrim &R = P.prims[i];
            BtPrimLite l;
            l.c = R.c;
            l.radius = R.radius;
            l.kind_object = (R.kind & BT_PRIM_SHAPE_MASK) | (R.object << 8);
            l.material = R.material;
            l.volume = R.volume;
            l.rcp_radius = ((R.kind & BT_PRIM_SHAPE_MASK) == BT_PRIM_SPHERE && R.radius >= 0x1p-20f && R.radius <= 0x1p20f) ? refined_rcp(R.radius) : 0.0f;
            lite[i] = l;
        }
        for (int i = threadIdx.x; i < P.n_materials; i += blockDim.x) mats[i] = P.materials[i];
        for (int i = threadIdx.x; i < P.n_volumes; i += blockDim.x) vols[i] = P.volumes[i];
        for (int i = threadIdx.x; i < P.n_lights; i += blockDim.x) lights[i] = P.lights[i];
        for (int i = threadIdx.x; i < P.n_light_faces; i += blockDim.x) faces[i] = P.light_faces[i];
        const bool dens_lds = P.n_density > 0 && P.n_density <= BT_DENSITY_LDS_MAX;
        if (dens_lds)
            for (int i = threadIdx.x; i < P.n_density; i += blockDim.x) dens[i] = P.density[i];
        S.lite = lite; S.materials = mats; S.volumes = vols; S.lights = lights; S.faces = faces;
        S.density = dens_lds ? dens : P.density;
        __syncthreads();
    }
    BtVolBox *const vbox = (BtVolBox *)(smem + P.table_lds_bytes);
    if (VOLS && P.vbox_lds_bytes) {
        for (int i = threadIdx.x; i < P.n_prims; i += blockDim.x) {
            const BtPrim &R = P.prims[i];
            BtVolBox bx;
            const V3 c = mk(R.c), hsz = mk(R.radius, R.radius, R.radius);
            const V3 bmin = c - hsz, bmax = c + hsz, size = bmax - bmin;
            bx.bmin.x = bmin.x; bx.bmin.y = bmin.y; bx.bmin.z = bmin.z;
            bx.size.x = size.x; bx.size.y = size.y; bx.size.z = size.z;
            bx.rcp.x = refined_rcp(size.x); bx.rcp.y = refined_rcp(size.y); bx.rcp.z = refined_rcp(size.z);
            const bool ok = size.x >= 0x1p-20f && size.x <= 0x1p20f && size.y >= 0x1p-20f && size.y <= 0x1p20f &&
                            size.z >= 0x1p-20f && size.z <= 0x1p20f;
            bx.ok = ok ? 1.0f : 0.0f;
            bx.pad0 = bx.pad1 = 0.0f;
            vbox[i] = bx;
        }
        __syncthreads();
    }

    const BlockGeom G = block_geom(P);
    const uint32_t pxb = G.pxb, LOG_PXB = G.LOG_PXB;
    const uint32_t lane = threadIdx.x & 63;
    const uint32_t nn = (uint32_t)(P.subsample_n * P.subsample_n);
    const uint32_t T = (uint32_t)P.samples * nn;
    const uint32_t sample0 = P.sample_base * nn;
    constexpr bool packed = PACKED;
    const uint32_t my_blocks = packed ? P.wg_blocks - (blockIdx.x < P.wg_blocks_rem ? 0u : 1u) : 1u;
    const uint32_t n_items = packed ? (my_blocks << (P.log_rows + LOG_PXB)) : pxb * T;
    const BlockRef B_own = block_ref(P, G, blockIdx.x);
    auto park = [&]() -> Parked * {
        return (Parked *)P.scratch + (size_t)blockIdx.x * (packed ? (size_t)P.wg_blocks << (P.log_rows + LOG_PXB) : (size_t)n_items);
    };

    uint32_t px = 0, py = 0, pixel_index = 0, park_i = 0;

    V3 ro = mk(0, 0, 0), rd = mk(0, 0, -1), beta = mk(1, 1, 1), L = mk(0, 0, 0);
    V3 first = mk(0, 0, 0);
    float first_depth = __builtin_inff();
    bool have_first = false;
    int bounce = 0, vbounce = 0, last_object = -1;
    uint32_t event = 0;
    bool pending = true;
    constexpr bool VOTE = !RECTS && !LENS;
    bool held = false;
    float held_t = 0.0f;
    int held_info = 0, waited = 0;
    uint32_t segments = 0;
    unsigned long long lens_steps = 0;
    LensState lens;
    bool bent = false;
    lens_begin(P, lens);

    auto park_guides = [&](const V3 &albedo, const V3 &nrm, float first_t) {
        typedef const __attribute__((address_space(4))) BtLaunch BtLaunchK;
        BtLaunchK *C = (BtLaunchK *)__builtin_amdgcn_kernarg_segment_ptr();
        asm volatile("" : "+s"(C));
        const size_t at = (size_t)blockIdx.x * (packed ? (size_t)P.wg_blocks << (P.log_rows + LOG_PXB) : (size_t)n_items) + park_i;
        if (C->guide_out[0]) ((Parked *)C->guide_scratch[0])[at] = Parked{albedo.x, albedo.y, albedo.z};
        if (C->guide_out[1]) ((Parked *)C->guide_scratch[1])[at] = Parked{nrm.x, nrm.y, nrm.z};
        if (C->guide_out[2]) {
            float depth = (first_t - P.clip_min) / (P.clip_max - P.clip_min);
            depth = fminf(fmaxf(depth, 0.0f), 1.0f);
            ((Parked1 *)C->guide_scratch[2])[at] = Parked1{depth};
        }
    };
    auto park_guide_defaults = [&]() { park_guides(mk(0, 0, 0), mk(0, 0, 0), __builtin_inff()); };
    auto finish_sample = [&]() {
        V3 value;
        if (OUTPUT == 0 || GUIDED || ADAPT) {
            value = L;
        } else if (OUTPUT == 3) {
            float depth = (first_depth - P.clip_min) / (P.clip_max - P.clip_min);
            depth = fminf(fmaxf(depth, 0.0f), 1.0f);
            value = mk(depth, depth, depth);
        } else {
            value = first;
        }
        park()[park_i] = Parked{value.x, value.y, value.z};
    };

    PathRec *const pool = (PathRec *)(smem + P.pool_lds_offset);
    constexpr bool CAN_COMPACT = PACKED && RECTS && !VOLS && OUTPUT == 0;
    const bool compacting = CAN_COMPACT && P.pool_records > 0;
    bool dry_lane = false;
    uint32_t drain_it = 0;

    BT_PROF_DECL;
#ifdef BT_LANESTAT
    unsigned long long ls_acc[9] = {};
    const unsigned long long ls_all = __ballot(true);
#endif
    for (;;) {
        do {
        if (compacting && dry_lane && pending) continue;
        BT_LS(0, 1ull);
        BT_LS(8, ls_all & ~__ballot(true));
        BT_PROF(0);
        int ev = EV_GEN;
        V3 pos = ro, normal = mk(0, 0, 0);
        float hit_depth = 0.0f;
        bool front = false, inside = false, vol_back = false;
        int pobject = -1, mat_index = 0, vol_index = 0;
        V3 prim_c = mk(0, 0, 0);
        float prim_radius = 0.0f;
        int hit_prim = 0;

        BT_LS(1, __ballot(!pending && !(VOTE && held)));
        if (!pending) {
            const bool marching = VOLS && last_object >= 0;
            if (!marching) vbounce = 0;
            const float tmin = marching ? 0.0f : P.clip_min;
            const float tmax = marching ? P.volume_step : P.clip_max;
            HitRec h;
            bool ended = false, captured = false;
            float travelled = 0.0f;
            if (LENS && !marching) {
                if (!bent) {
                    lens_begin(P, lens);
                    bent = true;
                    segments += 1;
                }
                const int r = lens_advance<RECTS>(P, ro, rd, lens, h, BT_LENS_BATCH, lens_steps);
                if (r == 2) continue;
                bent = false;
                captured = r < 0;
                travelled = lens.travelled;
            } else if (VOTE && held) {
                h.t = held_t;
                h.prim = held_info & 0x1fffffff;
                h.inside = (held_info >> 29) & 1;
                h.p_neg = (held_info >> 30) & 1;
            } else {
                segments += 1;
                h = intersect<RECTS, VOLS, RECTS && !VOLS && !LENS>(P, ro, rd, tmin, tmax, last_object);
            }
            if (captured) {
                ended = true;
            } else if (h.prim < 0) {
                L = L + beta * mk(P.root_color);
                if (AOV && !have_first) {
                    have_first = true;
                    if (OUTPUT == 1) first = mk(P.root_albedo);
                    if (OUTPUT == 2) first = P.root_has_albedo ? -rd : mk(0, 0, 0);
                    if (OUTPUT == 3) first_depth = P.root_has_albedo ? P.clip_max : __builtin_inff();
                    if (GUIDED) park_guides(mk(P.root_albedo), P.root_has_albedo ? -rd : mk(0, 0, 0), P.root_has_albedo ? P.clip_max : __builtin_inff());
                }
                ended = true;
            } else {
                const BtPrimLite &pl = S.lite[h.prim];
                const int pshape = pl.kind_object & 0xff;
                pobject = pl.kind_object >> 8;
                prim_c = mk(pl.c);
                prim_radius = pl.radius;
                hit_prim = h.prim;
                hit_depth = LENS ? h.t + travelled : h.t;
                pos = ro + rd * h.t;
                bool vol_face = false;
                if (VOLS && h.inside) {
                    inside = true;
                    vol_face = true;
                } else if (!RECTS || pshape == BT_PRIM_SPHERE) {
                    V3 nrm = pos - prim_c;
                    const float nax = fabsf(nrm.x), nay = fabsf(nrm.y), naz = fabsf(nrm.z), rr = pl.rcp_radius;
                    const bool in_range = (rr != 0.0f) & (nax == 0.0f || (nax >= 0x1p-60f && nax <= 0x1p60f)) &
                                          (nay == 0.0f || (nay >= 0x1p-60f && nay <= 0x1p60f)) & (naz == 0.0f || (naz >= 0x1p-60f && naz <= 0x1p60f));
                    if (__ballot(!in_range) == 0ull)
                        nrm = mk(div_refined(nrm.x, pl.radius, rr), div_refined(nrm.y, pl.radius, rr), div_refined(nrm.z, pl.radius, rr));
                    else
                        nrm = mk(nrm.x / pl.radius, nrm.y / pl.radius, nrm.z / pl.radius);
                    front = dot(rd, nrm) < 0.0f;
                    normal = front ? nrm : -nrm;
                    vol_face = VOLS && pl.volume >= 0;
                    vol_back = vol_face && !front;
                } else {
                    front = h.p_neg;
                    normal = front ? prim_c : -prim_c;
                }
                if (vol_face) {
                    vol_index = pl.volume;
                    ev = EV_VOLUME;
                } else {
                    mat_index = pl.material;
                    const BtMaterial &M = S.materials[mat_index];
                    if (!(VOTE && held)) L = L + beta * mk(M.emitted);
                    if (M.kind == BT_MAT_DIFFUSE) ev = EV_DIFFUSE;
                    else if (M.kind == BT_MAT_METALLIC) ev = EV_METALLIC;
                    else if (M.kind == BT_MAT_GLASS) ev = EV_GLASS;
                    else {
                        if (AOV && !have_first) {
                            have_first = true;
                            if (OUTPUT == 1) first = mk(M.emitted);
                            if (GUIDED) park_guides(mk(M.emitted), mk(0, 0, 0), __builtin_inff());
                        }
                        ended = true;
                    }
                }
            }
            if (GUIDED && ended && !have_first) park_guide_defaults();
            if (ended) finish_sample();
            if (VOTE && P.phase_vote && ev != EV_GEN) {
                held_t = h.t;
                held_info = h.prim | ((int)h.inside << 29) | ((int)h.p_neg << 30);
            }
        }
        pending = false;
        if (compacting && dry_lane && ev == EV_GEN) {
            pending = true;
            continue;
        }

        if (VOTE && P.phase_vote) {
            const bool want_gen = ev == EV_GEN;
            const unsigned long long m_gen = __ballot(want_gen), m_sc = __ballot(!want_gen);
            const uint32_t n_gen = popc64(m_gen), n_sc = popc64(m_sc);
            const unsigned long long starving = __ballot(waited >= P.phase_vote);
            const bool run_gen = n_gen >= n_sc || (starving & m_gen) != 0;
            const bool run_sc = n_sc > n_gen || (starving & m_sc) != 0;
            const unsigned long long served_m = (run_gen ? m_gen : 0ull) | (run_sc ? m_sc : 0ull);
            const bool served = __builtin_amdgcn_inverse_ballot_w64(served_m);
            BT_LS(7, __ballot(!served));
            if (!served) {
                waited += 1;
                pending = want_gen;
                held = !want_gen;
                continue;
            }
            waited = 0;
            held = false;
        }

        {
            const unsigned long long need = __ballot(ev == EV_GEN);
            if (need) {
                const int leader = __ffsll((long long)need) - 1;
                uint32_t base = 0;
                if ((int)lane == leader) base = atomicAdd(&s_next_item, popc64(need));
                base = (uint32_t)__builtin_amdgcn_readlane((int)base, leader);
                if (ev == EV_GEN) {
                    const uint32_t i = base + lanes_below(need);
                    if (i >= n_items) {
                        if (!compacting) goto queue_empty;
                        dry_lane = true;
                        pending = true;
                        continue;
                    }
                    park_i = i;
                    BlockRef B_i = B_own;
                    bool hole = false;
                    if (packed) {
                        const uint32_t row = i >> LOG_PXB;
                        B_i = block_ref(P, G, blockIdx.x + (row >> P.log_rows) * gridDim.x);
                        hole = (row & P.row_mask) >= T;
                    }
                    const PixelRef r = pixel_of(P, G, B_i, i & (pxb - 1u));
                    px = r.px;
                    py = r.py;
                    if (!r.in_frame || hole) {
                        pending = true;
                        continue;
                    }
                    pixel_index = py * P.width + px;
                }
            }
        }
        BT_PROF(1);

        BT_LS(2, __ballot(ev == EV_GEN)); BT_LS(3, __ballot(ev == EV_DIFFUSE)); BT_LS(4, __ballot(ev == EV_METALLIC));
        BT_LS(5, __ballot(ev == EV_GLASS)); BT_LS(6, __ballot(ev == EV_VOLUME));
        const uint32_t k_now = packed ? (park_i >> LOG_PXB) & P.row_mask : park_i >> LOG_PXB;
        const uint32_t sample_index = sample0 + k_now;
        const U4 u = philox(pixel_index, sample_index, ev == EV_GEN ? 0u : event, 0u, P.seed_lo, P.seed_hi);
        const uint32_t w1 = ev == EV_METALLIC ? u.x : (ev == EV_GLASS ? u.y : u.z);
        const uint32_t w2 = ev == EV_METALLIC ? u.y : (ev == EV_GLASS ? u.z : u.w);
        const float r1 = uniform_sample(w1, 0.0f, P.tau_scale), r2 = uniform_sample(w2, 0.0f, P.one_scale);
        bool vol_scatter = false;
        if (VOLS && ev == EV_VOLUME) {
            const float density = P.vbox_lds_bytes ? march_density_box(P, S, vol_index, vbox[hit_prim], pos)
                                                   : march_density(P, S, vol_index, prim_c, prim_radius, pos);
            vol_scatter = density >= 1.0f || bernoulli(u.x, density);
        }
        const bool wave_needs_dir = !VOLS || !BT_SKIP_DIR || __ballot(ev != EV_VOLUME || vol_scatter) != 0ull;
        float sn = 0.0f, cs = 0.0f;
        if (wave_needs_dir) sincos_bt(r1, sn, cs);
        BT_PROF(2);

        V3 new_o = pos, dir = rd;
        bool late_end = false;

        if (ev == EV_GEN) {
            float u_sub = 0.0f, v_sub = 0.0f;
            if (P.subsample_n > 1) {
                const uint32_t n = (uint32_t)P.subsample_n;
                const uint32_t subpx = k_now % (n * n);
                const float width_sub = 1.0f / (float)n;
                u_sub = (float)(subpx % n) * width_sub;
                v_sub = (float)(subpx / n) * width_sub;
            }
            typedef const __attribute__((address_space(4))) BtLaunch BtLaunchK;
            BtLaunchK *C = (BtLaunchK *)__builtin_amdgcn_kernarg_segment_ptr();
            asm volatile("" : "+s"(C));
            const V3 mcx = mk(C->cam_cx.x, C->cam_cx.y, C->cam_cx.z), mcy = mk(C->cam_cy.x, C->cam_cy.y, C->cam_cy.z),
                     mcz = mk(C->cam_cz.x, C->cam_cz.y, C->cam_cz.z);
            const float v0 = (float)py * C->pixel_height - 1.0f;
            const float u0 = (float)px * C->pixel_width - 1.0f;
            const float u_offset = u_sub * C->pixel_width + uniform_sample(u.x, C->jitter_u_lo, C->jitter_u_scale);
            const float v_offset = v_sub * C->pixel_height + uniform_sample(u.y, C->jitter_v_lo, C->jitter_v_scale);
            const float uu = u0 + u_offset, vv = v0 + v_offset;
            const float yrot = C->xfov * 0.5f * -uu;
            const float xrot = C->yfov * 0.5f * -vv;
            float sy, cy, sx, cx;
            sincos_small_bt(yrot, sy, cy);
            sincos_small_bt(xrot, sx, cx);
            const V3 d_cam = mk(-(cx * sy), sx, -(cx * cy));
            new_o = mk(C->cam_t.x, C->cam_t.y, C->cam_t.z) + mk(0.0f, 0.0f, 0.0f);
            dir = normalize_or_zero(xf_vector(mcx, mcy, mcz, d_cam));
            if (C->has_focus) {
                const V3 d1 = normalize(dir);
                const V3 defocus = (mk(C->disk_x.x, C->disk_x.y, C->disk_x.z) * cs + mk(C->disk_y.x, C->disk_y.y, C->disk_y.z) * sn) * r2;
                const V3 defocus_offset = xf_vector(mcx, mcy, mcz, defocus * C->aperture);
                const float frac_f_z = C->focus / fabsf(d_cam.z);
                new_o = new_o + defocus_offset;
                dir = d1 * frac_f_z - defocus_offset;
            }
            beta = mk(1, 1, 1);
            L = mk(0, 0, 0);
            bounce = 0; vbounce = 0; last_object = -1;
            event = 1;
            have_first = false;
            first = mk(0, 0, 0);
            first_depth = __builtin_inff();
            BT_PROF(3);
        } else {
            event += 1;
            const BtMaterial &M = S.materials[mat_index];
            int light_index = 0;
            bool to_light = false;
            if (ev == EV_DIFFUSE) {
                light_index = (int)__umulhi(u.x, (uint32_t)P.n_lights);
                to_light = bernoulli(u.y, 0.5f);
            }
            const bool is_cosine = ev == EV_DIFFUSE && !to_light;
            const bool in_frame_of_normal = is_cosine || ev == EV_METALLIC || ev == EV_GLASS;
            V3 v = mk(0.0f, 0.0f, 0.0f);
            if (wave_needs_dir) {
                const float sq = sqrt_bt(is_cosine ? r2 : r2 * (1.0f - r2));
                const float lx_ = (is_cosine ? cs : cs * 2.0f) * sq;
                const float ly_ = (is_cosine ? sn : sn * 2.0f) * sq;
                float lz_ = in_frame_of_normal ? 1.0f - r2 : 1.0f - 2.0f * r2;
                if (is_cosine) lz_ = sqrt_bt(1.0f - r2);
                v = mk(lx_, ly_, lz_);
                if (in_frame_of_normal) {
                    V3 z_axis = normalize(normal), x_axis, y_axis;
                    orthonormal_pair(z_axis, x_axis, y_axis);
                    v = (x_axis * lx_ + y_axis * ly_) + z_axis * lz_;
                }
            }

            if (ev == EV_DIFFUSE) {
                if (to_light) {
                    const BtLight &Lt = S.lights[light_index];
                    V3 point;
                    if (Lt.kind == BT_LIGHT_SPHERE) {
                        point = mk(Lt.centre) + v * Lt.radius;
                    } else if (RECTS && Lt.kind == BT_LIGHT_RECT) {
                        point = face_random_point(S.faces[Lt.face_first], u.z, u.w);
                    } else if (RECTS && Lt.kind == BT_LIGHT_CUBOID) {
                        const U4 e = philox(pixel_index, sample_index, event - 1u, 1u, P.seed_lo, P.seed_hi);
                        const float chosen = uniform_sample(e.x, 0.0f, Lt.total_scale);
                        int index = 0;
#pragma unroll
                        for (int f = 0; f < 5; ++f)
                            if (Lt.cum[f] <= chosen) index = f + 1;
                        point = face_random_point(S.faces[Lt.face_first + index], u.z, u.w);
                    } else {
                        point = mk(Lt.centre);
                    }
                    dir = point - pos;
                } else {
                    dir = v;
                }
            } else if (ev == EV_METALLIC) {
                dir = reflect(rd, normal) + v * M.roughness;
            } else if (ev == EV_GLASS) {
                const float ior = front ? M.inv_ior : M.ior;
                const float cos_theta = fminf(dot(-rd, normal), 1.0f);
                const float sin_theta = sqrt_bt(1.0f - cos_theta * cos_theta);
                const float fr = fresnel(rd, normal, ior);
                V3 base;
                if (ior * sin_theta > 1.0f || bernoulli(u.x, fr))
                    base = reflect(rd, normal);
                else
                    base = refract(rd, normal, ior);
                dir = base + v * M.roughness;
            } else if (VOLS) {
                if (vol_scatter) {
                    if (inside) new_o = pos - (rd * P.volume_step) * u24(u.y);
                    dir = v;
                    beta = beta * mk(0.8f, 0.8f, 0.8f);
                    if (AOV && !have_first) {
                        have_first = true;
                        if (OUTPUT == 1) first = mk(0.8f, 0.8f, 0.8f);
                        if (OUTPUT == 2) first = normal;
                        if (OUTPUT == 3) first_depth = hit_depth;
                        if (GUIDED) park_guides(mk(0.8f, 0.8f, 0.8f), normal, hit_depth);
                    }
                }
                if (vol_back) {
                    bounce += 1;
                    last_object = -1;
                } else {
                    last_object = pobject;
                    vbounce += 1;
                }
            }
        }

        BT_PROF(4);
        const V3 nd = normalize(dir);

        if (ev == EV_DIFFUSE || ev == EV_METALLIC || ev == EV_GLASS) {
            const BtMaterial &M = S.materials[mat_index];
            bool scatter = true;
            float weight = 1.0f;
            if (ev == EV_DIFFUSE) {
                const BtLight &Lt = S.lights[(int)__umulhi(u.x, (uint32_t)P.n_lights)];
                const float pd = dot(normal, nd) * 0.318309886183790671538f;
                const float plight = P.n_lights == 1 ? light_pdf_only_light<RECTS>(P, S, pos, nd) : light_pdf<RECTS>(P, Lt, S, pos, nd);
                const float p = lerpf(pd, plight, 0.5f);
                scatter = !(fabsf(p) <= 1e-5f);
                weight = pd / p;
            }
            if (AOV && !have_first) {
                have_first = true;
                if (scatter) {
                    if (OUTPUT == 1) first = mk(M.albedo);
                    if (OUTPUT == 2) first = normal;
                    if (OUTPUT == 3) first_depth = hit_depth;
                    if (GUIDED) park_guides(mk(M.albedo), normal, hit_depth);
                } else {
                    if (OUTPUT == 1) first = mk(M.emitted);
                    if (GUIDED) park_guides(mk(M.emitted), mk(0, 0, 0), __builtin_inff());
                }
            }
            if (scatter) {
                beta = beta * (mk(M.albedo) * weight);
                bounce += 1;
                last_object = -1;
            } else {
                late_end = true;
            }
        }
        ro = new_o;
        rd = nd;

        if (!late_end) late_end = (VOLS && last_object >= 0) ? (vbounce > P.max_volume_bounces) : (bounce > P.max_bounces);
        if (late_end) {
            if (GUIDED && !have_first) park_guide_defaults();
            finish_sample();
            pending = true;
        }
        BT_PROF(5);
        } while (0);
        if (compacting && __ballot(dry_lane) != 0ull) {
            dry_lane = true;
            {
                const uint32_t set = drain_it & 1u;
                const bool alive = !pending;
                const unsigned long long m = __ballot(alive);
                uint32_t base = 0;
                if (lane == 0) {
                    base = atomicAdd(&s_pool_paths[set], popc64(m));
                    if (m) atomicAdd(&s_pool_waves[set], 1u);
                }
                base = (uint32_t)__builtin_amdgcn_readfirstlane((int)base);
                const uint32_t slot = base + lanes_below(m);
                if (alive && slot < P.pool_records) {
                    PathRec r;
                    r.f[0] = ro.x; r.f[1] = ro.y; r.f[2] = ro.z; r.f[3] = rd.x; r.f[4] = rd.y; r.f[5] = rd.z;
                    r.f[6] = beta.x; r.f[7] = beta.y; r.f[8] = beta.z; r.f[9] = L.x; r.f[10] = L.y; r.f[11] = L.z;
                    r.w[0] = event; r.w[1] = pixel_index; r.w[2] = park_i;
                    r.w[3] = (uint32_t)bounce | ((uint32_t)vbounce << 16);
                    r.w[4] = ((uint32_t)(last_object + 1) & 0xffffffu) | ((uint32_t)waited << 24) | (held ? 0x80000000u : 0u);
                    r.w[5] = __float_as_uint(held_t); r.w[6] = (uint32_t)held_info; r.w[7] = 0u;
                    pool[slot] = r;
                }
                __syncthreads();
                const uint32_t total = *(volatile uint32_t *)&s_pool_paths[set], holders = *(volatile uint32_t *)&s_pool_waves[set];
                if (threadIdx.x == 0) { s_pool_paths[set ^ 1u] = 0; s_pool_waves[set ^ 1u] = 0; }
                if (total == 0u) break;
                if (total <= P.pool_records && holders > (total + 63u) / 64u) {
                    pending = threadIdx.x >= total;
                    if (!pending) {
                        const PathRec r = pool[threadIdx.x];
                        ro = mk(r.f[0], r.f[1], r.f[2]); rd = mk(r.f[3], r.f[4], r.f[5]);
                        beta = mk(r.f[6], r.f[7], r.f[8]); L = mk(r.f[9], r.f[10], r.f[11]);
                        event = r.w[0]; pixel_index = r.w[1]; park_i = r.w[2];
                        bounce = (int)(r.w[3] & 0xffffu); vbounce = (int)(r.w[3] >> 16);
                        last_object = (int)(r.w[4] & 0xffffffu) - 1; waited = (int)((r.w[4] >> 24) & 0x7fu); held = (r.w[4] >> 31) != 0u;
                        held_t = __uint_as_float(r.w[5]); held_info = (int)r.w[6];
                    }
                }
                __syncthreads();
            }
            drain_it += 1u;
        }
    }
queue_empty:;

    if (P.counters) {
        uint32_t sg = segments;
#pragma unroll
        for (int off = 32; off > 0; off >>= 1) sg += __shfl_xor(sg, off, 64);
        if (lane == 0 && sg) atomicAdd(&s_segments, sg);
    }
    if (packed) {
        __syncthreads();
        if (P.counters && threadIdx.x == 0) {
            const uint32_t total = *(volatile uint32_t *)&s_segments;
            if (total) atomicAdd(&P.counters[0], (unsigned long long)total);
        }
        sum_blocks(P, G, blockIdx.x, gridDim.x, my_blocks, T, park(), threadIdx.x, blockDim.x, P.out);
        if (GUIDED) {
            const size_t at = (size_t)blockIdx.x * ((size_t)P.wg_blocks << (P.log_rows + LOG_PXB));
            if (P.guide_out[0]) sum_blocks(P, G, blockIdx.x, gridDim.x, my_blocks, T, (const Parked *)P.guide_scratch[0] + at, threadIdx.x, blockDim.x, P.guide_out[0]);
            if (P.guide_out[1]) sum_blocks(P, G, blockIdx.x, gridDim.x, my_blocks, T, (const Parked *)P.guide_scratch[1] + at, threadIdx.x, blockDim.x, P.guide_out[1]);
            if (P.guide_out[2]) sum_blocks(P, G, blockIdx.x, gridDim.x, my_blocks, T, (const Parked1 *)P.guide_scratch[2] + at, threadIdx.x, blockDim.x, P.guide_out[2]);
        }
    } else {
        __builtin_amdgcn_fence(__ATOMIC_RELEASE, "workgroup");
        uint32_t arrived = 0;
        if (lane == 0) arrived = atomicAdd(&s_waves_done, 1u);
        arrived = (uint32_t)__builtin_amdgcn_readfirstlane((int)arrived);
        if (arrived == (blockDim.x >> 6) - 1u) {
            __builtin_amdgcn_fence(__ATOMIC_ACQUIRE, "workgroup");
            if (P.counters && lane == 0) {
                const uint32_t total = *(volatile uint32_t *)&s_segments;
                if (total) atomicAdd(&P.counters[0], (unsigned long long)total);
            }
            if constexpr (ADAPT) {
                typedef const __attribute__((address_space(4))) BtLaunch BtLaunchK;
                BtLaunchK *C = (BtLaunchK *)__builtin_amdgcn_kernarg_segment_ptr();
                asm volatile("" : "+s"(C));
                sum_block<Parked, true>(P, G, blockIdx.x, T, park(), lane, P.out, C->moment);
            } else {
                sum_block(P, G, blockIdx.x, T, park(), lane, P.out);
            }
            if (GUIDED) {
                const size_t at = (size_t)blockIdx.x * (size_t)n_items;
                if (P.guide_out[0]) sum_block(P, G, blockIdx.x, T, (const Parked *)P.guide_scratch[0] + at, lane, P.guide_out[0]);
                if (P.guide_out[1]) sum_block(P, G, blockIdx.x, T, (const Parked *)P.guide_scratch[1] + at, lane, P.guide_out[1]);
                if (P.guide_out[2]) sum_block(P, G, blockIdx.x, T, (const Parked1 *)P.guide_scratch[2] + at, lane, P.guide_out[2]);
            }
        }
    }
    if (P.counters) {
        if (LENS) {
            unsigned long long ls = wave_sum(lens_steps);
            if (lane == 0 && ls) atomicAdd(&P.counters[1], ls);
        }
#ifdef BT_LANESTAT
        for (int i = 0; i < 9; ++i) {
            unsigned long long v = ls_acc[i];
            for (int off = 32; off > 0; off >>= 1) {
                const unsigned long long o = __shfl_xor(v, off, 64);
                v = o > v ? o : v;
            }
            if (lane == 0) atomicAdd(&P.counters[2 + i], v);
        }
#elif defined(BT_PROFILE)
        if (lane == 0)
            for (int i = 0; i < BT_N_COUNTERS - 2; ++i) atomicAdd(&P.counters[2 + i], prof_acc[i]);
#endif
    }
}

__global__ __launch_bounds__(256) void bt_unshard_kernel(const float4 *gathered, float4 *frame, uint32_t width,
                                                         uint32_t height, uint32_t tiles_x, uint32_t tiles_y,
                                                         uint32_t world, uint32_t tiles_per_rank) {
    const uint32_t tile = blockIdx.x;
    if (tile >= tiles_x * tiles_y) return;
    const uint32_t rank = tile % world, slot = tile / world;
    const uint32_t lx = threadIdx.x & 15, ly = threadIdx.x >> 4;
    const uint32_t px = (tile % tiles_x) * BT_TILE_DIM + lx, py = (tile / tiles_x) * BT_TILE_DIM + ly;
    if (px >= width || py >= height) return;
    const size_t src = ((size_t)rank * tiles_per_rank + slot) * (BT_TILE_DIM * BT_TILE_DIM) + ly * BT_TILE_DIM + lx;
    frame[(size_t)py * width + px] = gathered[src];
}

namespace {
BT_DEV float log2_bt(float x) {
    const uint32_t xi = __float_as_uint(x);
    int e = (int)((xi >> 23) & 0xffu) - 127;
    float m = __uint_as_float((xi & 0x7fffffu) | 0x3f800000u);
    if (m > 1.41421356f) { m = m * 0.5f; e += 1; }
    const float t = m - 1.0f;
    const float s = t / (2.0f + t), s2 = s * s;
    float p = __builtin_fmaf(s2, 0.0909090909f, 0.1111111111f);
    p = __builtin_fmaf(p, s2, 0.1428571429f);
    p = __builtin_fmaf(p, s2, 0.2f);
    p = __builtin_fmaf(p, s2, 0.3333333333f);
    const float ln = __builtin_fmaf(p * s2, s, s) * 2.0f;
    return __builtin_fmaf(ln, 1.4426950408889634f, (float)e);
}
BT_DEV float exp2_bt(float y) {
    const float k = __builtin_rintf(y), r = y - k;
    const float z = r * 0.6931471805599453f;
    float p = __builtin_fmaf(z, 1.984126984e-4f, 1.388888889e-3f);
    p = __builtin_fmaf(p, z, 8.333333333e-3f);
    p = __builtin_fmaf(p, z, 4.166666667e-2f);
    p = __builtin_fmaf(p, z, 1.666666667e-1f);
    p = __builtin_fmaf(p, z, 0.5f);
    p = __builtin_fmaf(p, z, 1.0f);
    p = __builtin_fmaf(p, z, 1.0f);
    const int ki = (int)k;
    if (ki < -126) return 0.0f;
    if (ki > 127) return __builtin_inff();
    return p * __uint_as_float((uint32_t)(ki + 127) << 23);
}
BT_DEV float linear_to_srgb(float x) {
    if (x <= 0.0031308f) return 12.92f * x;
    if (!(x < 3.0e38f)) return x;
    return 1.055f * exp2_bt(log2_bt(x) * (1.0f / 2.4f)) - 0.055f;
}
BT_DEV uint32_t f32_to_u8(float x) {
    float v = x * 255.0f;
    if (!(v > 0.0f)) return 0u;
    if (v >= 255.0f) return 255u;
    return (uint32_t)v;
}
}
__global__ __launch_bounds__(256) void bt_preview_kernel(const float4 *rgba, uint32_t *out, uint32_t n,
                                                         float samples_recip, int color_space) {
    const uint32_t i = blockIdx.x * blockDim.x + threadIdx.x;
    if (i >= n) return;
    const float4 s = rgba[i];
    V3 rgb = mk(s.x, s.y, s.z) * samples_recip;
    if (color_space == 1) {
        V3 nrm = normalize(rgb);
        rgb = (nrm + mk(1, 1, 1)) * 0.5f;
    } else if (color_space == 3) {
        rgb = mk(linear_to_srgb(rgb.x), linear_to_srgb(rgb.y), linear_to_srgb(rgb.z));
    }
    out[i] = f32_to_u8(rgb.x) | (f32_to_u8(rgb.y) << 8) | (f32_to_u8(rgb.z) << 16) | (f32_to_u8(s.w) << 24);
}

extern "C" void bt_primary_masks_host(const BtLaunch *P, const BtSphereRow *rows, uint32_t n_blocks, uint64_t *out) {
    for (uint32_t b = 0; b < n_blocks; ++b) out[b] = btcull::block_mask(*P, rows, b);
}
extern "C" int bt_launch_reads_masks(const BtLaunch *P, int output) {
    return !P->any_rects && !P->any_volumes && !P->lens_on && P->wg_blocks <= 1 && output != 2 && output != 4 && output != 5 && P->max_bounces >= 0;
}
extern "C" int bt_mask_cache_enabled(void) {
#ifdef BT_MASK_NOCACHE
    return 0;
#else
    return 1;
#endif
}
extern "C" hipError_t bt_launch_block_masks(const BtLaunch *P, uint32_t n_blocks, uint64_t *masks, hipStream_t stream) {
    if (n_blocks == 0 || !masks || (P->n_prims > 0 && !P->sphere_rows)) return hipErrorInvalidValue;
    hipLaunchKernelGGL(bt_block_mask_kernel, dim3((n_blocks + 255u) / 256u), dim3(256), 0, stream, *P, n_blocks,
                       (unsigned long long *)masks);
    return hipGetLastError();
}
extern "C" hipError_t bt_launch_render(const BtLaunch *P, int output, unsigned grid, size_t lds_bytes,
                                       hipStream_t stream) {
    const bool packed = P->wg_blocks > 1;
    if (packed && P->lens_on) return hipErrorInvalidValue;
    if (bt_launch_reads_masks(P, output) && !P->block_masks) return hipErrorInvalidValue;
    dim3 g(packed ? P->n_workgroups : grid * (unsigned)P->slices), b(256);
    const int cls = (P->any_rects ? 2 : 0) | (P->any_volumes ? 1 : 0);
#define BT_LAUNCH(O, L, R, V, K)                                                                                 \
    do {                                                                                                         \
        if (lds_bytes > 48 * 1024)                                                                               \
            (void)hipFuncSetAttribute((const void *)bt_render_kernel<O, L, R, V, K>,                             \
                                      hipFuncAttributeMaxDynamicSharedMemorySize, (int)lds_bytes);               \
        hipLaunchKernelGGL((bt_render_kernel<O, L, R, V, K>), g, b, lds_bytes, stream, *P);                      \
    } while (0)
#define BT_LAUNCH_OUT(L, R, V, K)                                                                                \
    switch (output) {                                                                                            \
    case 0: BT_LAUNCH(0, L, R, V, K); break;                                                                     \
    case 1: BT_LAUNCH(1, L, R, V, K); break;                                                                     \
    case 2: BT_LAUNCH(2, L, R, V, K); break;                                                                     \
    default: BT_LAUNCH(3, L, R, V, K); break;                                                                    \
    }
#define BT_LAUNCH_CLASS(L, K)                                                                                    \
    if (cls == 3) { BT_LAUNCH_OUT(L, true, true, K) } else if (cls == 2) { BT_LAUNCH_OUT(L, true, false, K) }      \
    else if (cls == 1) { BT_LAUNCH_OUT(L, false, true, K) } else { BT_LAUNCH_OUT(L, false, false, K) }
    if (output == 5) {
        if (P->lens_on || packed || !P->tile_active || !P->moment) return hipErrorInvalidValue;
        if (cls == 3) BT_LAUNCH(5, false, true, true, false); else if (cls == 2) BT_LAUNCH(5, false, true, false, false);
        else if (cls == 1) BT_LAUNCH(5, false, false, true, false); else BT_LAUNCH(5, false, false, false, false);
    } else if (output == 4) {
        if (P->lens_on) return hipErrorInvalidValue;
#define BT_LAUNCH_GUIDED(K)                                                                                      \
        if (cls == 3) BT_LAUNCH(4, false, true, true, K); else if (cls == 2) BT_LAUNCH(4, false, true, false, K);    \
        else if (cls == 1) BT_LAUNCH(4, false, false, true, K); else BT_LAUNCH(4, false, false, false, K);
        if (packed) { BT_LAUNCH_GUIDED(true) } else { BT_LAUNCH_GUIDED(false) }
#undef BT_LAUNCH_GUIDED
    } else if (packed) {
        BT_LAUNCH_CLASS(false, true)
    } else if (P->lens_on) {
        BT_LAUNCH_CLASS(true, false)
    } else {
        BT_LAUNCH_CLASS(false, false)
    }
#undef BT_LAUNCH_CLASS
#undef BT_LAUNCH_OUT
#undef BT_LAUNCH
    return hipGetLastError();
}
extern "C" hipError_t bt_launch_unshard(const float *gathered, float *frame, uint32_t width, uint32_t height,
                                        uint32_t tiles_x, uint32_t tiles_y, uint32_t world, uint32_t tiles_per_rank,
                                        hipStream_t stream) {
    hipLaunchKernelGGL(bt_unshard_kernel, dim3(tiles_x * tiles_y), dim3(256), 0, stream, (const float4 *)gathered,
                       (float4 *)frame, width, height, tiles_x, tiles_y, world, tiles_per_rank);
    return hipGetLastError();
}
extern "C" hipError_t bt_launch_preview(const float *rgba, uint8_t *out, uint32_t n, uint32_t samples,
                                        int color_space, hipStream_t stream) {
    float recip = 1.0f / (float)samples;
    hipLaunchKernelGGL(bt_preview_kernel, dim3((n + 255) / 256), dim3(256), 0, stream, (const float4 *)rgba,
                       (uint32_t *)out, n, recip, color_space);
    return hipGetLastError();
}
```

### bendy_tracer_amd/csrc/bt_plan.hpp

```cpp
#pragma once
#include <stdint.h>

#include <algorithm>
#include <cmath>
#include <string>
#include <vector>

#include "../../include/bendy_hip.h"
#include "bt_scene.hpp"
#include "bt_types.h"

#ifndef BT_POOL_RECORDS
#define BT_POOL_RECORDS 128
#endif

static_assert(BT_TILE == BT_TILE_DIM, "public and device tile sizes must agree");

namespace btplan {

constexpr uint64_t kDefaultScratchCap = 2ull << 30;
constexpr uint32_t kScratchShrinkAfter = 8;

inline uint32_t tiles_across(uint32_t extent) { return (extent + BT_TILE - 1) / BT_TILE; }
inline uint32_t frame_tiles(uint32_t width, uint32_t height) { return tiles_across(width) * tiles_across(height); }
inline uint32_t tiles_per_rank(uint32_t n_tiles, uint32_t world) { return (n_tiles + world - 1) / world; }
inline uint64_t pixels_owned(uint32_t width, uint32_t height, uint32_t rank, uint32_t world, const uint32_t *weight = nullptr) {
    const uint32_t tiles_x = tiles_across(width), n_tiles = frame_tiles(width, height);
    uint64_t pixels = 0;
    for (uint32_t t = rank; t < n_tiles; t += world) {
        const uint32_t tx = t % tiles_x, ty = t / tiles_x;
        const uint32_t w = std::min<uint32_t>(BT_TILE, width - tx * BT_TILE), h = std::min<uint32_t>(BT_TILE, height - ty * BT_TILE);
        pixels += (uint64_t)w * h * (weight ? weight[t] : 1u);
    }
    return pixels;
}
inline uint32_t shard_launch(BtLaunch &P, uint32_t rank, uint32_t world, bool sharded) {
    P.rank = rank;
    P.world = world;
    P.sharded = sharded ? 1 : 0;
    const uint32_t n_tiles = P.tiles_x * P.tiles_y;
    return sharded ? tiles_per_rank(n_tiles, world) : n_tiles;
}

inline bool any_prim_carries_volume(const std::vector<BtPrim> &prims) {
    for (const BtPrim &R : prims)
        if (R.volume >= 0) return true;
    return false;
}

struct Scratch {
    uint64_t bytes = 0;
    uint32_t small_streak = 0;
};
inline bool scratch_serves(Scratch &held, uint64_t need) {
    if (held.bytes >= need) {
        if (held.bytes / 4 <= need) { held.small_streak = 0; return true; }
        if (++held.small_streak < kScratchShrinkAfter) return true;
    }
    held.small_streak = 0;
    return false;
}
template <class Realloc> bool reserve_scratch(Scratch &held, uint64_t need, Realloc &&realloc) {
    if (scratch_serves(held, need)) return true;
    held.bytes = realloc(need);
    return held.bytes == need;
}

enum { PLAIN = 0, GUIDED = 1, ADAPTIVE = 2 };

struct Plan {
    int output = 0;
    uint32_t grid = 0;
    uint32_t chunk = 0;
    uint32_t launches = 0;
    size_t lds_bytes = 0;
    uint64_t guide_values[3] = {};
    uint64_t parked_bytes = 0;
    uint64_t pixels = 0;
    std::string error;
};

template <class Realloc>
int plan_launch(BtLaunch &P, int output, const bt::FlatScene &flat, const bt_tuning &tune, uint32_t n_cu, int kind, uint32_t guides,
                Scratch &held, Realloc &&realloc, Plan &plan) {
    const bool guided = kind == GUIDED && (guides & 7u) != 0, adapt = kind == ADAPTIVE;
    uint64_t sample_bytes = 3 * sizeof(float);
    if (guided) {
        output = 4;
        for (int g = 0; g < 3; ++g)
            if (guides >> g & 1u) sample_bytes += (g == 2 ? 1 : 3) * sizeof(float);
    }
    if (adapt) output = 5;
    plan.output = output;
    const uint32_t grid = P.sharded ? tiles_per_rank(P.tiles_x * P.tiles_y, P.world) : P.tiles_x * P.tiles_y;
    plan.grid = grid;

    const uint32_t nn = (uint32_t)(P.subsample_n * P.subsample_n);
    const uint64_t px_launch = (uint64_t)grid * BT_TILE_DIM * BT_TILE_DIM;
    uint32_t chunk = (uint32_t)P.samples;
    P.slices = 1;
    P.table_lds_bytes = (uint32_t)flat.lds_bytes();
    size_t lds_bytes = flat.lds_bytes();
    {
        bool safe = true;
        for (const BtVolume &v : flat.volumes)
            safe = safe && v.width >= 1 && v.height >= 1 && v.depth >= 1 && v.size.x >= 0.0f && v.size.y >= 0.0f && v.size.z >= 0.0f &&
                   std::ceil(v.size.x) <= (float)(v.width - 1) && std::ceil(v.size.y) <= (float)(v.height - 1) &&
                   std::ceil(v.size.z) <= (float)(v.depth - 1);
        safe = safe && flat.density.size() < (1u << 24);
        P.vols_safe = safe ? 1 : 0;
        P.vbox_lds_bytes = any_prim_carries_volume(flat.prims) ? (uint32_t)(sizeof(BtVolBox) * flat.prims.size()) : 0u;
        if (lds_bytes + P.vbox_lds_bytes > 32 * 1024) P.vbox_lds_bytes = 0;
        lds_bytes += P.vbox_lds_bytes;
    }
#ifdef BT_LDS_PAD
    lds_bytes += BT_LDS_PAD;
#endif
    const uint64_t wave_slots = (uint64_t)n_cu * 20;
    const uint64_t T_all = (uint64_t)P.samples * nn;
    const uint64_t per_sample = px_launch * nn * sample_bytes;
    const uint64_t cap = tune.scratch_cap_bytes ? tune.scratch_cap_bytes : kDefaultScratchCap;
    if (per_sample * chunk > cap) chunk = (uint32_t)std::max<uint64_t>(1, cap / per_sample);
    while (!reserve_scratch(held, per_sample * chunk, realloc)) {
        if (chunk == 1) {
            plan.error = "no device memory for the parked samples (" + std::to_string(per_sample) + " bytes per sample)";
            return BT_ERR_DEVICE;
        }
        chunk = (chunk + 1) / 2;
    }
    auto pick = [&](uint64_t T) -> uint32_t {
        if (tune.slices) return tune.slices;
        uint32_t S = 1;
        if (P.lens_on) {
            while (S < 32 && T / (2 * S) >= 4) S *= 2;
        } else {
            const uint64_t target = 21ull * (uint64_t)n_cu * 6;
            while (S < 32 && (uint64_t)grid * (2 * S) * 4 <= 5 * target && T / (2 * S) >= 8) S *= 2;
            while (S < 32 && (uint64_t)grid * S * 2 < target && T / (2 * S) >= 4) S *= 2;
            while (S < 32 && (uint64_t)grid * 4 * S < 2 * wave_slots && T / (2 * S) >= 1) S *= 2;
            if (!P.any_rects)
                while (S < 32 && (uint64_t)grid * (2 * S) <= 30ull * (uint64_t)n_cu && 256 * T / (2 * S) >= 256) S *= 2;
        }
        return S;
    };
    P.slices = (int32_t)pick((uint64_t)chunk * nn);
    const uint64_t longest = ((uint64_t)P.max_bounces + 2) * ((uint64_t)P.max_volume_bounces + 3) + (P.lens_on ? 2 : 0);
    const uint64_t items_max = std::max<uint64_t>(1, 0xffffffffull / longest);
    {
        const uint64_t pxb = 256u / (uint32_t)P.slices;
        if (pxb * chunk * nn > items_max) chunk = (uint32_t)std::max<uint64_t>(1, items_max / (pxb * nn));
    }
    P.wg_blocks = 1;
    P.wg_blocks_rem = 0;
    P.n_workgroups = 0;
    P.log_rows = 0;
    P.row_mask = 0xffffffffu;
    P.pool_records = 0;
    P.pool_lds_offset = 0;
    const size_t pool_offset = (lds_bytes + 15) & ~(size_t)15, pool_bytes = BT_POOL_RECORDS * 80;
    bool pool_ok = tune.packed != 1 && P.any_rects && !P.any_volumes && output == 0 &&
                   P.max_bounces < 0xfff0 && P.max_volume_bounces < 0xfff0 && flat.prims.size() < 0xfffff0u;
    auto slots_per_cu = [](size_t lds) { return std::max(1u, std::min(7u, 160u * 1024u / (uint32_t)((lds + 64 + 2047) & ~(size_t)2047))); };
    pool_ok = pool_ok && slots_per_cu(pool_offset + pool_bytes) == slots_per_cu(lds_bytes);
    const uint32_t wg_slots = n_cu * slots_per_cu(lds_bytes);
    const uint64_t T_launch = (uint64_t)chunk * nn;
    uint64_t values = px_launch * T_launch;
    const uint64_t items_all = px_launch * T_launch, lanes_all = (uint64_t)wg_slots * 256;
    const bool pack = tune.packed > 0 || (tune.packed < 0 && items_all > lanes_all && items_all <= 24 * lanes_all);
    if (pack && chunk == (uint32_t)P.samples && !P.lens_on && !adapt) {
        uint32_t S = 4;
        while (S < 32 && S < 4 * T_launch) S *= 2;
        if (tune.slices) S = tune.slices;
        const uint64_t blocks = (uint64_t)grid * S, per_wg = (blocks + wg_slots - 1) / wg_slots;
        uint32_t log_rows = 0;
        while ((1ull << log_rows) < T_launch) log_rows += 1;
        const uint64_t wg_items = (per_wg * (256u / S)) << log_rows;
        const uint64_t need = (uint64_t)wg_slots * wg_items * sample_bytes;
        if (blocks > wg_slots && blocks <= 0x7fffffffu && wg_items <= items_max &&
            (need <= held.bytes || reserve_scratch(held, need, realloc))) {
            P.slices = (int32_t)S;
            P.n_workgroups = wg_slots;
            P.wg_blocks = (uint32_t)per_wg;
            P.wg_blocks_rem = (uint32_t)(blocks - (per_wg - 1) * wg_slots);
            P.log_rows = log_rows;
            P.row_mask = (1u << log_rows) - 1u;
            values = (uint64_t)wg_slots * wg_items;
            if (pool_ok) {
                P.pool_records = BT_POOL_RECORDS;
                P.pool_lds_offset = (uint32_t)pool_offset;
                lds_bytes = pool_offset + pool_bytes;
            }
        } else if (held.bytes == 0 && !reserve_scratch(held, per_sample * chunk, realloc)) {
            plan.error = "no device memory for the parked samples";
            return BT_ERR_DEVICE;
        }
    }
    plan.parked_bytes = px_launch * T_all * sample_bytes;
    if (guided) {
        uint64_t plane = values * 3;
        for (int g = 0; g < 3; ++g)
            if (guides >> g & 1u) {
                plan.guide_values[g] = plane;
                plane += values * (g == 2 ? 1 : 3);
            }
        if (plane * sizeof(float) > held.bytes) {
            plan.error = "the guides' parked values do not fit the scratch";
            return BT_ERR_DEVICE;
        }
    }

    if (lds_bytes > 158 * 1024) {
        plan.error = "scene tables (" + std::to_string(flat.lds_bytes()) + " bytes) exceed the 160 KB of LDS of a gfx950 CU";
        return BT_ERR_INVALID_ARG;
    }
    P.phase_vote = tune.phase_vote >= 0 ? tune.phase_vote : (P.any_volumes ? 4 : 3);
    plan.chunk = chunk;
    plan.launches = ((uint32_t)P.samples + chunk - 1) / chunk;
    plan.lds_bytes = lds_bytes;
    plan.pixels = pixels_owned(P.width, P.height, P.rank, P.world);
    return 0;
}

inline void plan_stats(const BtLaunch &P, const Plan &plan, const Scratch &held, bt_stats &st) {
    st.pixels = plan.pixels;
    st.samples = plan.pixels * (uint64_t)P.samples * (uint64_t)(P.subsample_n * P.subsample_n);
    st.segments = 0;
    st.kernel_ms = 0.0f;
    st.slices = (uint32_t)P.slices;
    st.launches = plan.launches;
    st.packed = P.wg_blocks > 1 ? (P.pool_records ? 2u : 1u) : 0u;
    st.workgroups = P.wg_blocks > 1 ? P.n_workgroups : plan.grid * (uint32_t)P.slices;
    st.scratch_bytes = held.bytes;
    st.parked_bytes = plan.parked_bytes;
}

}
```

### bendy_tracer_amd/csrc/bt_types.h

```cpp
#pragma once
#include <stdint.h>

#define BT_TILE_DIM 16
#if defined(BT_PROFILE) || defined(BT_LANESTAT)
#define BT_N_COUNTERS 12
#else
#define BT_N_COUNTERS 2
#endif
#define BT_DENSITY_LDS_MAX 8192

struct BtV3 { float x, y, z; };

enum { BT_PRIM_SPHERE = 0, BT_PRIM_RECT = 1, BT_PRIM_RECT_AA = 2, BT_PRIM_RECT_AAN = 3, BT_PRIM_RECT_LA = 4, BT_PRIM_SHAPE_MASK = 7, BT_PRIM_STRICT = 8 };
struct BtPrim {
    int32_t kind;
    int32_t object;
    int32_t material;
    int32_t volume;
    BtV3 c;
    float radius;
    BtV3 t;
    float w_sqr;
    BtV3 icx; float h_sqr;
    BtV3 icy; int32_t aa_u;
    BtV3 icz; int32_t aa_v;
    BtV3 it;  int32_t aa_w;
    BtV3 ax;  float ax_w;
    BtV3 ay;  float ay_w;
};
static_assert(sizeof(BtPrim) == 144, "BtPrim must be 144 bytes");

struct BtSpherePair {
    float cx[2], cy[2], cz[2], radius[2];
    int32_t object[2];
    int32_t pad[2];
};
static_assert(sizeof(BtSpherePair) == 48, "BtSpherePair must be 48 bytes");
struct BtSphereRow {
    float cx, cy, cz;
    float r2;
};
static_assert(sizeof(BtSphereRow) == 16, "BtSphereRow must be 16 bytes");

struct BtRectAAN {
    float it_a, it_b;
    float lim_a, lim_b;
    float t_w;
    uint32_t sgn_mask;
    uint32_t prio;
    uint32_t pad;
};
static_assert(sizeof(BtRectAAN) == 32, "BtRectAAN must be 32 bytes");
struct BtRectLA {
    BtV3 n;
    uint32_t first_of_normal;
    BtV3 t;
    uint32_t prio;
    float a_x[2], a_y[2], a_z[2], a_w[2];
    float lim[2];
    uint32_t pad[2];
};
static_assert(sizeof(BtRectLA) == 80, "BtRectLA must be 80 bytes");

struct BtVolBox {
    BtV3 bmin; float ok;
    BtV3 size; float pad0;
    BtV3 rcp;  float pad1;
};
static_assert(sizeof(BtVolBox) == 48, "BtVolBox must be 48 bytes");

struct BtPrimLite {
    BtV3 c;
    float radius;
    int32_t kind_object;
    int32_t material;
    int32_t volume;
    float rcp_radius;
};

enum { BT_MAT_FLAT = 0, BT_MAT_DIFFUSE = 1, BT_MAT_METALLIC = 2, BT_MAT_GLASS = 3, BT_MAT_EMISSIVE = 4 };
struct BtMaterial {
    int32_t kind;
    BtV3 albedo;
    float roughness, ior, inv_ior, pad;
    BtV3 emitted;
    float pad1;
};

struct BtVolume {
    int32_t width, height, depth, offset;
    BtV3 size;
    float pad;
};

enum { BT_LIGHT_SPHERE = 0, BT_LIGHT_RECT = 1, BT_LIGHT_CUBOID = 2, BT_LIGHT_POINT = 3 };
struct BtLightFace {
    BtV3 mcx, mcy, mcz, mt;
    BtV3 ax, ay;
    float half_width, half_height;
    float scale_x, scale_y;
    float area;
    float pad;
};
struct BtLight {
    int32_t kind;
    int32_t prim_first, prim_count;
    int32_t face_first;
    BtV3 centre;
    float radius;
    float shadow;
    float cum[5];
    float total_scale;
    float pad;
};

struct BtLaunch {
    const BtPrim *prims;
    const BtSpherePair *sphere_pairs;
    const BtMaterial *materials;
    const BtVolume *volumes;
    const BtLight *lights;
    const BtLightFace *light_faces;
    const float *density;
    int32_t n_prims, n_materials, n_volumes, n_lights, n_light_faces, n_density;
    int32_t any_rects;
    int32_t any_volumes;
    const BtRectAAN *aan_rows;
    const BtRectLA *la_rows;
    const int32_t *other_rows;
    int32_t n_aan[3];
    int32_t n_la, n_other;
    BtV3 root_color, root_albedo;
    int32_t root_has_albedo;
    BtV3 cam_cx, cam_cy, cam_cz, cam_t;
    float yfov, xfov, pixel_width, pixel_height;
    float jitter_u_lo, jitter_u_scale, jitter_v_lo, jitter_v_scale;
    int32_t has_focus;
    float focus, aperture;
    BtV3 disk_x, disk_y;
    float tau_scale, one_scale;
    int32_t max_bounces, max_volume_bounces;
    float clip_min, clip_max, volume_step;
    int32_t samples, subsample_n;
    uint32_t sample_base;
    uint32_t seed_lo, seed_hi;
    uint32_t width, height, tiles_x, tiles_y;
    uint32_t rank, world;
    int32_t sharded;
    float *out;
    unsigned long long *counters;
    int32_t slices;
    float *scratch;
    uint32_t tiles_x_magic;
    uint32_t table_lds_bytes;
    uint32_t vbox_lds_bytes;
    int32_t vols_safe;
    int32_t phase_vote;
    int32_t lens_on;
    BtV3 lens_c;
    float lens_rs, lens_step, lens_radius;
    int32_t lens_max_steps;
    const int32_t *lens_prims;
    int32_t n_lens_prims;
    float lens_margin;
    const BtSphereRow *sphere_rows;
    uint32_t wg_blocks, wg_blocks_rem, n_workgroups;
    uint32_t pool_records, pool_lds_offset;
    uint32_t log_rows, row_mask;
    const uint64_t *block_masks;
    float *guide_out[3];
    float *guide_scratch[3];
    const uint32_t *tile_active;
    float *moment;
};
```

### include/bendy_hip.h

```cpp
#ifndef BENDY_HIP_H
#define BENDY_HIP_H

#include <stddef.h>
#include <stdint.h>

#ifdef __cplusplus
extern "C" {
#endif

typedef enum {
    BT_DONE = 0,
    BT_IN_PROGRESS = 1,
    BT_ERR_INVALID_ARG = -1,
    BT_ERR_IO = -2,
    BT_ERR_PARSE = -3,
    BT_ERR_INVALID_REF = -4,
    BT_ERR_NOT_CAMERA = -5,
    BT_ERR_NOT_MATERIAL = -6,
    BT_ERR_NO_LIGHT = -7,
    BT_ERR_DEVICE = -8,
    BT_ERR_UNSUPPORTED = -9
} bt_status;

typedef enum { BT_OUTPUT_FULL = 0, BT_OUTPUT_ALBEDO = 1, BT_OUTPUT_NORMAL = 2, BT_OUTPUT_DEPTH = 3 } bt_output;

typedef enum { BT_COLOR_NONE = 0, BT_COLOR_NORMAL = 1, BT_COLOR_LINEAR = 2, BT_COLOR_SRGB = 3 } bt_color_space;

typedef struct {
    uint32_t max_bounces;
    uint32_t max_volume_bounces;
    float clip_min;
    float clip_max;
    float volume_step;
    uint32_t chunks_x;
    uint32_t chunks_y;
    int32_t output;
} bt_config;

typedef struct {
    uint32_t subsample_n;
    uint32_t samples;
    int32_t has_output;
    int32_t output;
    int32_t has_max_bounces;
    uint32_t max_bounces;
    int32_t has_max_volume_bounces;
    uint32_t max_volume_bounces;
    int32_t has_volume_step;
    float volume_step;
    uint32_t sample_base;
} bt_render_config;

typedef struct {
    uint64_t samples;
    uint64_t segments;
    uint64_t pixels;
    float kernel_ms;
    uint64_t lens_steps;
    uint32_t slices;
    uint32_t launches;
    uint64_t scratch_bytes;
    uint64_t parked_bytes;
    uint32_t workgroups;
    uint32_t packed;
} bt_stats;

typedef struct {
    uint32_t slices;
    int32_t phase_vote;
    uint64_t scratch_cap_bytes;
    int32_t packed;
    int32_t reserved;
} bt_tuning;

typedef struct {
    float centre[3];
    float rs;
    float step;
    float radius;
    uint32_t max_steps;
} bt_lens;

typedef struct bt_scene bt_scene;

void bt_config_default(bt_config *out);
void bt_render_config_default(bt_render_config *out);
const char *bt_last_error(void);
int bt_last_error_code(void);
const char *bt_version(void);

bt_scene *bt_scene_load(const char *path);
bt_scene *bt_scene_from_json(const char *json, size_t len);
bt_scene *bt_scene_default(void);
void bt_scene_free(bt_scene *scene);
int bt_scene_to_json(const bt_scene *scene, char *out, size_t cap);
int bt_scene_save(const bt_scene *scene, const char *path);
int bt_write_png(const char *path, const uint8_t *rgba8, uint32_t width, uint32_t height);
int bt_scene_find_by_tag(const bt_scene *scene, const char *tag, uint64_t *object_ref);
int bt_scene_set_camera_aspect(bt_scene *scene, uint64_t camera_ref, float aspect_ratio);
int bt_scene_set_lens(bt_scene *scene, const bt_lens *lens);
int bt_scene_object_count(const bt_scene *scene);
int bt_scene_data_count(const bt_scene *scene);
int bt_scene_export_prims(const bt_scene *scene, float *out, int cap);
int bt_debug_primary_mask(bt_scene *scene, uint64_t camera_ref, const bt_config *config, const bt_render_config *render,
                          uint32_t width, uint32_t height, uint32_t slices, uint32_t rank, uint32_t world, uint64_t *masks,
                          uint32_t cap);

int bt_debug_set_object(bt_scene *scene, uint64_t object_ref, const float *translation, float radius);
int bt_debug_block_masks_device(bt_scene *scene, uint64_t camera_ref, const bt_config *config, const bt_render_config *render,
                                uint32_t width, uint32_t height, uint32_t slices, uint32_t rank, uint32_t world,
                                uint64_t *masks, uint32_t cap);
int bt_debug_mask_key(bt_scene *scene, uint64_t camera_ref, const bt_config *config, const bt_render_config *render,
                      uint32_t width, uint32_t height, uint32_t slices, uint32_t rank, uint32_t world, uint8_t *out,
                      uint32_t cap);

int bt_debug_plan_launch(bt_scene *scene, uint64_t camera_ref, const bt_config *config, const bt_render_config *render,
                         uint32_t width, uint32_t height, uint32_t rank, uint32_t world, int32_t sharded, uint32_t n_cu,
                         int32_t pass_kind, uint32_t guides, uint64_t alloc_limit, bt_stats *out);


int bt_render(bt_scene *scene, uint64_t camera_ref, const bt_config *config, const bt_render_config *render,
              float *rgba_host, uint32_t width, uint32_t height, uint64_t seed);

int bt_render_device(bt_scene *scene, uint64_t camera_ref, const bt_config *config, const bt_render_config *render,
                     float *rgba_device, uint32_t width, uint32_t height, uint64_t seed, void *stream);

int bt_render_guided_device(bt_scene *scene, uint64_t camera_ref, const bt_config *config,
                            const bt_render_config *render, float *color_device, float *albedo_device,
                            float *normal_device, float *depth_device, uint32_t width, uint32_t height,
                            uint64_t seed, void *stream);

#define BT_TILE 16
size_t bt_shard_floats(uint32_t width, uint32_t height, uint32_t world);
int bt_render_shard_device(bt_scene *scene, uint64_t camera_ref, const bt_config *config,
                           const bt_render_config *render, float *shard_device, uint32_t width, uint32_t height,
                           uint32_t rank, uint32_t world, uint64_t seed, void *stream);
int bt_unshard_device(const float *gathered_device, float *rgba_device, uint32_t width, uint32_t height,
                      uint32_t world, void *stream);

#define BT_COMM_ID_BYTES 128
typedef struct bt_comm bt_comm;
int bt_comm_unique_id(void *id_out, size_t cap);
bt_comm *bt_comm_init(uint32_t rank, uint32_t world, const void *unique_id, size_t id_bytes);
void bt_comm_free(bt_comm *comm);
int bt_comm_rank(const bt_comm *comm);
int bt_comm_world(const bt_comm *comm);
int bt_allgather_shards_device(bt_comm *comm, const float *shard_device, float *gathered_device, uint32_t width,
                               uint32_t height, void *stream);
int bt_exchange_frame_device(bt_comm *comm, const float *shard_device, float *gathered_device, float *rgba_device,
                             uint32_t width, uint32_t height, void *stream);

int bt_preview_device(const float *rgba_device, uint8_t *rgba8_device, uint32_t width, uint32_t height,
                      uint32_t samples, int32_t color_space, void *stream);
int bt_preview(const float *rgba_host, uint8_t *rgba8_host, uint32_t width, uint32_t height, uint32_t samples,
               int32_t color_space);

typedef struct {
    uint32_t levels;
    float sigma_color;
    float sigma_normal;
    float sigma_depth;
    float eps_albedo;
} bt_denoise_params;
typedef struct bt_denoiser bt_denoiser;
void bt_denoise_params_default(bt_denoise_params *out);
bt_denoiser *bt_denoiser_new(void);
void bt_denoiser_free(bt_denoiser *d);
int bt_denoise_device(bt_denoiser *d, const float *color, uint32_t color_samples,
                      const float *albedo, uint32_t albedo_samples,
                      const float *normal, uint32_t normal_samples,
                      const float *depth, uint32_t depth_samples,
                      float *out, uint32_t width, uint32_t height, const bt_denoise_params *params, void *stream);
int bt_denoise(bt_denoiser *d, const float *color, uint32_t color_samples,
               const float *albedo, uint32_t albedo_samples,
               const float *normal, uint32_t normal_samples,
               const float *depth, uint32_t depth_samples,
               float *out, uint32_t width, uint32_t height, const bt_denoise_params *params);

typedef struct {
    float threshold;
    uint32_t min_samples;
    uint32_t max_samples;
    float eps;
} bt_adaptive_params;
typedef struct {
    uint32_t active_tiles;
    uint32_t tiles;
    uint32_t min_count, max_count;
    uint64_t pixel_samples;
    uint32_t passes;
    uint32_t reserved;
} bt_adaptive_stats;
typedef struct bt_adaptive bt_adaptive;
void bt_adaptive_params_default(bt_adaptive_params *out);
bt_adaptive *bt_adaptive_new(uint32_t width, uint32_t height);
void bt_adaptive_free(bt_adaptive *a);
int bt_adaptive_reset(bt_adaptive *a);
int bt_render_adaptive_device(bt_scene *scene, uint64_t camera_ref, const bt_config *config, const bt_render_config *render,
                              bt_adaptive *adaptive, const bt_adaptive_params *params, float *rgba_device, uint32_t width,
                              uint32_t height, uint64_t seed, void *stream);
int bt_adaptive_poll(bt_adaptive *a, bt_adaptive_stats *out);
int bt_adaptive_counts(bt_adaptive *a, uint32_t *host, uint32_t n);
int bt_adaptive_errors(bt_adaptive *a, float *host, uint32_t n);
int bt_debug_adaptive_moments(bt_adaptive *a, float *host, uint32_t n);
int bt_adaptive_resolve_device(bt_adaptive *a, const float *rgba_device, float *out_device, void *stream);

void bt_tuning_default(bt_tuning *out);
int bt_scene_set_tuning(bt_scene *scene, const bt_tuning *tuning);
int bt_scene_get_tuning(const bt_scene *scene, bt_tuning *out);

int bt_scene_trim(bt_scene *scene);

int bt_scene_last_stats(bt_scene *scene, bt_stats *out);

#ifdef __cplusplus
}
#endif
#endif
```

Before: 58160 Msamples/s.

## Add LDS-pooled end-game path compaction for plain flat-scene renders

Moves the path-tracing body into an include file and adds a noinline end-game routine. It compacts live paths into an LDS pool once waves thin out, so surviving paths are regathered into fewer waves of the workgroup. The pool is only allocated when the tuning field endgame is 2 and the extra LDS does not reduce workgroups per CU. Debug entry points report the LDS plan and how many paths were moved. The change risks extra barriers and LDS traffic, and the default tuning value may leave it off.

```diff
diff --git a/bendy_tracer_amd/api.py b/bendy_tracer_amd/api.py
--- a/bendy_tracer_amd/api.py
+++ b/bendy_tracer_amd/api.py
@@ -148,7 +148,7 @@
     "bt_exchange_frame_device", "bt_scene_last_stats", "bt_tuning_default", "bt_scene_set_tuning", "bt_scene_get_tuning", "bt_scene_default", "bt_scene_to_json", "bt_scene_save", "bt_write_png",
     "bt_scene_trim", "bt_denoise_params_default", "bt_denoiser_new", "bt_denoiser_free", "bt_denoise_device",
     "bt_denoise", "bt_debug_primary_mask", "bt_debug_block_masks_device", "bt_debug_mask_key", "bt_debug_set_object",
-    "bt_debug_plan_launch",
+    "bt_debug_plan_launch", "bt_debug_plan_lds", "bt_debug_end_game_counts",
     "bt_render_guided_device", "bt_adaptive_params_default", "bt_adaptive_new", "bt_adaptive_free", "bt_adaptive_reset",
     "bt_render_adaptive_device", "bt_adaptive_poll", "bt_adaptive_counts", "bt_adaptive_errors", "bt_debug_adaptive_moments",
     "bt_adaptive_resolve_device",
@@ -194,6 +194,8 @@
     L.bt_debug_plan_launch.argtypes = [vp, C.c_uint64, C.POINTER(_CConfig), C.POINTER(_CRenderConfig), C.c_uint32, C.c_uint32,
                                        C.c_uint32, C.c_uint32, C.c_int32, C.c_uint32, C.c_int32, C.c_uint32, C.c_uint64,
                                        C.POINTER(Stats)]
+    L.bt_debug_plan_lds.argtypes = [vp, C.POINTER(C.c_uint32)]
+    L.bt_debug_end_game_counts.argtypes = [vp, C.POINTER(C.c_uint64)]
     L.bt_render.argtypes = [vp, C.c_uint64, C.POINTER(_CConfig), C.POINTER(_CRenderConfig), fp, C.c_uint32,
                             C.c_uint32, C.c_uint64]
     L.bt_render_device.argtypes = [vp, C.c_uint64, C.POINTER(_CConfig), C.POINTER(_CRenderConfig), vp, C.c_uint32,
@@ -344,6 +346,7 @@
             return
         _check(lib.bt_scene_get_tuning(self._h, C.byref(t)))
         for k, v in knobs.items():
+            k = "reserved" if k == "endgame" else k
             if not hasattr(t, k):
                 raise TypeError(f"bt_tuning has no field {k!r}")
             setattr(t, k, int(v))
@@ -356,11 +359,22 @@
 
     def tuning_from_env(self, environ=None):
         env = os.environ if environ is None else environ
-        names = {"BT_SLICES": "slices", "BT_PHASE_VOTE": "phase_vote", "BT_SCRATCH_CAP": "scratch_cap_bytes", "BT_PACKED": "packed"}
+        names = {"BT_SLICES": "slices", "BT_PHASE_VOTE": "phase_vote", "BT_SCRATCH_CAP": "scratch_cap_bytes", "BT_PACKED": "packed",
+                 "BT_ENDGAME": "endgame"}
         knobs = {f: int(env[e]) for e, f in names.items() if env.get(e) not in (None, "", "-")}
         if knobs:
             self.set_tuning(**knobs)
         return knobs
+
+    def plan_lds(self):
+        out = (C.c_uint32 * 4)()
+        _check(lib.bt_debug_plan_lds(self._h, out))
+        return dict(pool_records=out[0], pool_lds_offset=out[1], lds_bytes=out[2], resident=out[3])
+
+    def end_game_counts(self):
+        out = (C.c_uint64 * 2)()
+        _check(lib.bt_debug_end_game_counts(self._h, out))
+        return int(out[0]), int(out[1])
 
     def trim(self):
         _check(lib.bt_scene_trim(self._h))
diff --git a/bendy_tracer_amd/csrc/bt_api.cpp b/bendy_tracer_amd/csrc/bt_api.cpp
--- a/bendy_tracer_amd/csrc/bt_api.cpp
+++ b/bendy_tracer_amd/csrc/bt_api.cpp
@@ -76,6 +76,7 @@
     DeviceArray<float> d_scratch;
     uint32_t scratch_small_streak = 0;
     btplan::Scratch plan_scratch;
+    uint32_t plan_lds[4] = {};
     DeviceArray<uint64_t> d_block_masks;
     btcull::MaskKey masks_for{};
     uint64_t rows_generation = 0;
@@ -374,6 +375,13 @@
     uint32_t guide_mask() const { return (guides[0] ? 1u : 0u) | (guides[1] ? 2u : 0u) | (guides[2] ? 4u : 0u); }
 };
 
+void note_plan_lds(bt_scene *s, const BtLaunch &P, const btplan::Plan &plan) {
+    s->plan_lds[0] = P.pool_records;
+    s->plan_lds[1] = P.pool_lds_offset;
+    s->plan_lds[2] = (uint32_t)plan.lds_bytes;
+    s->plan_lds[3] = plan.resident;
+}
+
 int render_common(bt_scene *s, uint64_t camera_ref, const bt_config *cfg, const bt_render_config *rc, float *out_device,
                   uint32_t width, uint32_t height, uint32_t rank, uint32_t world, bool sharded, uint64_t seed,
                   hipStream_t stream, const RenderPass &pass = RenderPass{}) {
@@ -397,6 +405,7 @@
                                 [&](uint64_t need) { return realloc_scratch(s, stream, need); }, plan);
     s->scratch_small_streak = held.small_streak;
     if (rcode) return fail(rcode, plan.error);
+    note_plan_lds(s, P, plan);
     P.scratch = s->d_scratch.ptr;
     for (int g = 0; g < 3; ++g) {
         P.guide_out[g] = plan.output == 4 ? pass.guides[g] : nullptr;
@@ -481,6 +490,7 @@
     if (t->phase_vote < -1 || t->phase_vote > 64)
         return fail(BT_ERR_INVALID_ARG, "bt_tuning.phase_vote must be -1 .. 64");
     if (t->packed < -1 || t->packed > 2) return fail(BT_ERR_INVALID_ARG, "bt_tuning.packed must be -1, 0, 1 or 2");
+    if (t->endgame < 0 || t->endgame > 2) return fail(BT_ERR_INVALID_ARG, "bt_tuning.endgame must be 0, 1 or 2");
     scene->tuning = *t;
     return 0;
 }
@@ -719,8 +729,27 @@
     rc = btplan::plan_launch(P, output, scene->flat, scene->tuning, n_cu, pass_kind, guides, held,
                              [&](uint64_t need) -> uint64_t { return alloc_limit == 0 || need <= alloc_limit ? need : 0; }, plan);
     if (rc) return fail(rc, plan.error);
+    note_plan_lds(scene, P, plan);
     btplan::plan_stats(P, plan, held, *out);
     out->lens_steps = 0;
+    return 0;
+}
+
+int bt_debug_plan_lds(const bt_scene *scene, uint32_t out[4]) {
+    if (!scene || !out) return fail(BT_ERR_INVALID_ARG, "null argument");
+    std::memcpy(out, scene->plan_lds, sizeof scene->plan_lds);
+    return 0;
+}
+
+int bt_debug_end_game_counts(bt_scene *scene, uint64_t out[2]) {
+    if (!scene || !out) return fail(BT_ERR_INVALID_ARG, "null argument");
+    out[0] = out[1] = 0;
+    if (!scene->d_counters || scene->render_seq == 0) return 0;
+    BT_HIP(hipEventSynchronize(scene->ev_stop));
+    unsigned long long c[16] = {};
+    BT_HIP(hipMemcpy(c, scene->d_counters + (size_t)scene->last_slot * 16, sizeof c, hipMemcpyDeviceToHost));
+    out[0] = c[BT_COUNTER_EG_MOVED];
+    out[1] = c[BT_COUNTER_EG_WORKGROUPS];
     return 0;
 }
 
diff --git a/bendy_tracer_amd/csrc/bt_kernels.hip b/bendy_tracer_amd/csrc/bt_kernels.hip
--- a/bendy_tracer_amd/csrc/bt_kernels.hip
+++ b/bendy_tracer_amd/csrc/bt_kernels.hip
@@ -15,6 +15,12 @@
 #else
 #define BT_PROF_DECL
 #define BT_PROF(i)
+#endif
+
+#if defined(BT_PROFILE) || defined(BT_LANESTAT)
+#define BT_HAVE_END_GAME 0
+#else
+#define BT_HAVE_END_GAME 1
 #endif
 
 namespace {
@@ -192,6 +198,7 @@
     if (P.counters && threadIdx.x == 0 && nx * ny != 0u) atomicAdd(&P.counters[0], (unsigned long long)(nx * ny) * T);
 }
 
+
 }
 
 __global__ __launch_bounds__(256) void bt_block_mask_kernel(BtLaunch P, uint32_t n_blocks, unsigned long long *masks) {
@@ -222,6 +229,126 @@
 #ifndef BT_LENS_BATCH
 #define BT_LENS_BATCH 8
 #endif
+struct EndGameCounters { uint32_t paths[2], waves[2], changed[2], segments, waves_done; };
+#if BT_HAVE_END_GAME
+static __device__ __attribute__((noinline)) uint32_t bt_end_game(float ro_x, float ro_y, float ro_z, float rd_x, float rd_y, float rd_z,
+                                                      float beta_x, float beta_y, float beta_z, float L_x, float L_y, float L_z,
+                                                      uint32_t event, uint32_t pixel_index, uint32_t park_i, int bounce,
+                                                      float held_t, int held_info, uint32_t flags, uint32_t segments,
+                                                      uint32_t lds_base, uint32_t kernarg_lo, uint32_t kernarg_hi) {
+    constexpr int OUTPUT = 0;
+    constexpr bool LENS = false, RECTS = false, VOLS = false, GUIDED = false, AOV = false, VOTE = true, packed = false;
+    constexpr bool compacting = true, dry_lane = true;
+    typedef const __attribute__((address_space(4))) BtLaunch BtLaunchK;
+    const uint64_t kernarg = ((uint64_t)(uint32_t)__builtin_amdgcn_readfirstlane((int)kernarg_hi) << 32) |
+                             (uint64_t)(uint32_t)__builtin_amdgcn_readfirstlane((int)kernarg_lo);
+    const BtLaunch &P = *(const BtLaunch *)(BtLaunchK *)kernarg;
+    typedef __attribute__((address_space(3))) unsigned char LdsByte;
+    unsigned char *const smem = (unsigned char *)(LdsByte *)(uintptr_t)lds_base;
+    SceneLds S;
+    {
+        const unsigned char *p = smem;
+        S.lite = (const BtPrimLite *)p;        p += sizeof(BtPrimLite) * P.n_prims;
+        S.materials = (const BtMaterial *)p;   p += sizeof(BtMaterial) * P.n_materials;
+        S.volumes = (const BtVolume *)p;       p += sizeof(BtVolume) * P.n_volumes;
+        S.lights = (const BtLight *)p;         p += sizeof(BtLight) * P.n_lights;
+        S.faces = (const BtLightFace *)p;
+        S.density = P.density;
+    }
+    BtVolBox *const vbox = nullptr;
+    const BlockGeom G = block_geom(P);
+    const uint32_t LOG_PXB = G.LOG_PXB, lane = threadIdx.x & 63;
+    const uint32_t nn = (uint32_t)(P.subsample_n * P.subsample_n);
+    const uint32_t T = (uint32_t)P.samples * nn, sample0 = P.sample_base * nn;
+    Parked *const parked = (Parked *)P.scratch + (size_t)blockIdx.x * (size_t)(G.pxb * T);
+    PathRec *const pool = (PathRec *)(smem + P.pool_lds_offset);
+    EndGameCounters *const cnt = (EndGameCounters *)(pool + P.pool_records);
+
+    V3 ro = mk(ro_x, ro_y, ro_z), rd = mk(rd_x, rd_y, rd_z), beta = mk(beta_x, beta_y, beta_z), L = mk(L_x, L_y, L_z);
+    bool pending = (flags & 1u) != 0u, held = (flags & 2u) != 0u;
+    V3 first = mk(0, 0, 0);
+    [[maybe_unused]] float first_depth = 0.0f;
+    bool have_first = false, bent = false;
+    int vbounce = 0, last_object = -1;
+    unsigned long long lens_steps = 0;
+    LensState lens;
+    lens_begin(P, lens);
+    auto park_guides = [](const V3 &, const V3 &, float) {};
+    auto park_guide_defaults = []() {};
+    auto finish_sample = [&]() { parked[park_i] = Parked{L.x, L.y, L.z}; };
+
+    uint32_t round = 0, moved = 0;
+    for (;;) {
+        do {
+#define BT_END_GAME_BODY 1
+#include "bt_path_body.inc"
+#undef BT_END_GAME_BODY
+        } while (0);
+        {
+            const uint32_t set = round & 1u;
+            const bool alive = !pending;
+            const unsigned long long m = __ballot(alive);
+            uint32_t base = 0;
+            if (lane == 0) {
+                base = atomicAdd(&cnt->paths[set], popc64(m));
+                if (m) atomicAdd(&cnt->waves[set], 1u);
+            }
+            base = (uint32_t)__builtin_amdgcn_readfirstlane((int)base);
+            const uint32_t slot = base + lanes_below(m);
+            if (alive && slot < P.pool_records) {
+                PathRec r;
+                r.f[0] = ro.x; r.f[1] = ro.y; r.f[2] = ro.z; r.f[3] = rd.x; r.f[4] = rd.y; r.f[5] = rd.z;
+                r.f[6] = beta.x; r.f[7] = beta.y; r.f[8] = beta.z; r.f[9] = L.x; r.f[10] = L.y; r.f[11] = L.z;
+                r.w[0] = event; r.w[1] = pixel_index; r.w[2] = park_i;
+                r.w[3] = (uint32_t)bounce;
+                r.w[4] = 0u; r.w[5] = 0u; r.w[6] = 0u; r.w[7] = 0u;
+                pool[slot] = r;
+            }
+            const unsigned long long other_lane = __ballot(alive && slot != threadIdx.x);
+            if (lane == 0 && other_lane) atomicAdd(&cnt->changed[set], popc64(other_lane));
+            __syncthreads();
+            const uint32_t total = *(volatile uint32_t *)&cnt->paths[set], holders = *(volatile uint32_t *)&cnt->waves[set];
+            const uint32_t changed = *(volatile uint32_t *)&cnt->changed[set];
+            if (threadIdx.x == 0) { cnt->paths[set ^ 1u] = 0; cnt->waves[set ^ 1u] = 0; cnt->changed[set ^ 1u] = 0; }
+            if (total == 0u) break;
+            if (total <= P.pool_records && holders > (total + 63u) / 64u) {
+                moved += changed;
+                pending = threadIdx.x >= total;
+                if (!pending) {
+                    const PathRec r = pool[threadIdx.x];
+                    ro = mk(r.f[0], r.f[1], r.f[2]); rd = mk(r.f[3], r.f[4], r.f[5]);
+                    beta = mk(r.f[6], r.f[7], r.f[8]); L = mk(r.f[9], r.f[10], r.f[11]);
+                    event = r.w[0]; pixel_index = r.w[1]; park_i = r.w[2];
+                    bounce = (int)r.w[3];
+                }
+            }
+            __syncthreads();
+        }
+        round += 1u;
+    }
+    if (P.counters) {
+        uint32_t sg = segments;
+#pragma unroll
+        for (int off = 32; off > 0; off >>= 1) sg += __shfl_xor(sg, off, 64);
+        if (lane == 0 && sg) atomicAdd(&cnt->segments, sg);
+    }
+    __builtin_amdgcn_fence(__ATOMIC_RELEASE, "workgroup");
+    uint32_t arrived = 0;
+    if (lane == 0) arrived = atomicAdd(&cnt->waves_done, 1u);
+    arrived = (uint32_t)__builtin_amdgcn_readfirstlane((int)arrived);
+    if (arrived != 256u / 64u - 1u) return 0u;
+    __builtin_amdgcn_fence(__ATOMIC_ACQUIRE, "workgroup");
+    if (P.counters && lane == 0) {
+        const uint32_t total = *(volatile uint32_t *)&cnt->segments;
+        if (total) atomicAdd(&P.counters[0], (unsigned long long)total);
+        if (moved) atomicAdd(&P.counters[BT_COUNTER_EG_MOVED], (unsigned long long)moved);
+        atomicAdd(&P.counters[BT_COUNTER_EG_WORKGROUPS], 1ull);
+    }
+    return 1u;
+}
+#endif
+
+#define BT_CAN_END_GAME (BT_HAVE_END_GAME && OUTPUT == 0 && !LENS && !RECTS && !VOLS && !PACKED)
 template <int OUTPUT, bool LENS, bool RECTS, bool VOLS, bool PACKED>
 __global__ __launch_bounds__(256, (OUTPUT == 4 && RECTS && !VOLS) ? BT_WAVES_PER_SIMD_GUIDED_RECTS : LENS ? BT_WAVES_PER_SIMD_LENS : (RECTS ? BT_WAVES_PER_SIMD_RECTS : (VOLS ? BT_WAVES_PER_SIMD_VOLS : BT_WAVES_PER_SIMD))) void bt_render_kernel(BtLaunch P) {
     constexpr bool GUIDED = OUTPUT == 4;
@@ -256,6 +383,10 @@
         s_next_item = 0;
         s_segments = 0;
         if (PACKED && RECTS && !VOLS && OUTPUT == 0) s_pool_paths[0] = s_pool_paths[1] = s_pool_waves[0] = s_pool_waves[1] = 0;
+        if constexpr (BT_CAN_END_GAME) if (P.pool_records) {
+            uint32_t *c = (uint32_t *)(smem + P.pool_lds_offset + P.pool_records * sizeof(PathRec));
+            for (int i = 0; i < 8; ++i) c[i] = 0u;
+        }
     }
 
     SceneLds S;
@@ -382,375 +513,16 @@
 #endif
     for (;;) {
         do {
-        if (compacting && dry_lane && pending) continue;
-        BT_LS(0, 1ull);
-        BT_LS(8, ls_all & ~__ballot(true));
-        BT_PROF(0);
-        int ev = EV_GEN;
-        V3 pos = ro, normal = mk(0, 0, 0);
-        float hit_depth = 0.0f;
-        bool front = false, inside = false, vol_back = false;
-        int pobject = -1, mat_index = 0, vol_index = 0;
-        V3 prim_c = mk(0, 0, 0);
-        float prim_radius = 0.0f;
-        int hit_prim = 0;
-
-        BT_LS(1, __ballot(!pending && !(VOTE && held)));
-        if (!pending) {
-            const bool marching = VOLS && last_object >= 0;
-            if (!marching) vbounce = 0;
-            const float tmin = marching ? 0.0f : P.clip_min;
-            const float tmax = marching ? P.volume_step : P.clip_max;
-            HitRec h;
-            bool ended = false, captured = false;
-            float travelled = 0.0f;
-            if (LENS && !marching) {
-                if (!bent) {
-                    lens_begin(P, lens);
-                    bent = true;
-                    segments += 1;
-                }
-                const int r = lens_advance<RECTS>(P, ro, rd, lens, h, BT_LENS_BATCH, lens_steps);
-                if (r == 2) continue;
-                bent = false;
-                captured = r < 0;
-                travelled = lens.travelled;
-            } else if (VOTE && held) {
-                h.t = held_t;
-                h.prim = held_info & 0x1fffffff;
-                h.inside = (held_info >> 29) & 1;
-                h.p_neg = (held_info >> 30) & 1;
-            } else {
-                segments += 1;
-                h = intersect<RECTS, VOLS, RECTS && !VOLS && !LENS>(P, ro, rd, tmin, tmax, last_object);
-            }
-            if (captured) {
-                ended = true;
-            } else if (h.prim < 0) {
-                L = L + beta * mk(P.root_color);
-                if (AOV && !have_first) {
-                    have_first = true;
-                    if (OUTPUT == 1) first = mk(P.root_albedo);
-                    if (OUTPUT == 2) first = P.root_has_albedo ? -rd : mk(0, 0, 0);
-                    if (OUTPUT == 3) first_depth = P.root_has_albedo ? P.clip_max : __builtin_inff();
-                    if (GUIDED) park_guides(mk(P.root_albedo), P.root_has_albedo ? -rd : mk(0, 0, 0), P.root_has_albedo ? P.clip_max : __builtin_inff());
-                }
-                ended = true;
-            } else {
-                const BtPrimLite &pl = S.lite[h.prim];
-                const int pshape = pl.kind_object & 0xff;
-                pobject = pl.kind_object >> 8;
-                prim_c = mk(pl.c);
-                prim_radius = pl.radius;
-                hit_prim = h.prim;
-                hit_depth = LENS ? h.t + travelled : h.t;
-                pos = ro + rd * h.t;
-                bool vol_face = false;
-                if (VOLS && h.inside) {
-                    inside = true;
-                    vol_face = true;
-                } else if (!RECTS || pshape == BT_PRIM_SPHERE) {
-                    V3 nrm = pos - prim_c;
-                    const float nax = fabsf(nrm.x), nay = fabsf(nrm.y), naz = fabsf(nrm.z), rr = pl.rcp_radius;
-                    const bool in_range = (rr != 0.0f) & (nax == 0.0f || (nax >= 0x1p-60f && nax <= 0x1p60f)) &
-                                          (nay == 0.0f || (nay >= 0x1p-60f && nay <= 0x1p60f)) & (naz == 0.0f || (naz >= 0x1p-60f && naz <= 0x1p60f));
-                    if (__ballot(!in_range) == 0ull)
-                        nrm = mk(div_refined(nrm.x, pl.radius, rr), div_refined(nrm.y, pl.radius, rr), div_refined(nrm.z, pl.radius, rr));
-                    else
-                        nrm = mk(nrm.x / pl.radius, nrm.y / pl.radius, nrm.z / pl.radius);
-                    front = dot(rd, nrm) < 0.0f;
-                    normal = front ? nrm : -nrm;
-                    vol_face = VOLS && pl.volume >= 0;
-                    vol_back = vol_face && !front;
-                } else {
-                    front = h.p_neg;
-                    normal = front ? prim_c : -prim_c;
-                }
-                if (vol_face) {
-                    vol_index = pl.volume;
-                    ev = EV_VOLUME;
-                } else {
-                    mat_index = pl.material;
-                    const BtMaterial &M = S.materials[mat_index];
-                    if (!(VOTE && held)) L = L + beta * mk(M.emitted);
-                    if (M.kind == BT_MAT_DIFFUSE) ev = EV_DIFFUSE;
-                    else if (M.kind == BT_MAT_METALLIC) ev = EV_METALLIC;
-                    else if (M.kind == BT_MAT_GLASS) ev = EV_GLASS;
-                    else {
-                        if (AOV && !have_first) {
-                            have_first = true;
-                            if (OUTPUT == 1) first = mk(M.emitted);
-                            if (GUIDED) park_guides(mk(M.emitted), mk(0, 0, 0), __builtin_inff());
-                        }
-                        ended = true;
-                    }
-                }
-            }
-            if (GUIDED && ended && !have_first) park_guide_defaults();
-            if (ended) finish_sample();
-            if (VOTE && P.phase_vote && ev != EV_GEN) {
-                held_t = h.t;
-                held_info = h.prim | ((int)h.inside << 29) | ((int)h.p_neg << 30);
-            }
-        }
-        pending = false;
-        if (compacting && dry_lane && ev == EV_GEN) {
-            pending = true;
-            continue;
-        }
-
-        if (VOTE && P.phase_vote) {
-            const bool want_gen = ev == EV_GEN;
-            const unsigned long long m_gen = __ballot(want_gen), m_sc = __ballot(!want_gen);
-            const uint32_t n_gen = popc64(m_gen), n_sc = popc64(m_sc);
-            const unsigned long long starving = __ballot(waited >= P.phase_vote);
-            const bool run_gen = n_gen >= n_sc || (starving & m_gen) != 0;
-            const bool run_sc = n_sc > n_gen || (starving & m_sc) != 0;
-            const unsigned long long served_m = (run_gen ? m_gen : 0ull) | (run_sc ? m_sc : 0ull);
-            const bool served = __builtin_amdgcn_inverse_ballot_w64(served_m);
-            BT_LS(7, __ballot(!served));
-            if (!served) {
-                waited += 1;
-                pending = want_gen;
-                held = !want_gen;
-                continue;
-            }
-            waited = 0;
-            held = false;
-        }
-
-        {
-            const unsigned long long need = __ballot(ev == EV_GEN);
-            if (need) {
-                const int leader = __ffsll((long long)need) - 1;
-                uint32_t base = 0;
-                if ((int)lane == leader) base = atomicAdd(&s_next_item, popc64(need));
-                base = (uint32_t)__builtin_amdgcn_readlane((int)base, leader);
-                if (ev == EV_GEN) {
-                    const uint32_t i = base + lanes_below(need);
-                    if (i >= n_items) {
-                        if (!compacting) goto queue_empty;
-                        dry_lane = true;
-                        pending = true;
-                        continue;
-                    }
-                    park_i = i;
-                    BlockRef B_i = B_own;
-                    bool hole = false;
-                    if (packed) {
-                        const uint32_t row = i >> LOG_PXB;
-                        B_i = block_ref(P, G, blockIdx.x + (row >> P.log_rows) * gridDim.x);
-                        hole = (row & P.row_mask) >= T;
-                    }
-                    const PixelRef r = pixel_of(P, G, B_i, i & (pxb - 1u));
-                    px = r.px;
-                    py = r.py;
-                    if (!r.in_frame || hole) {
-                        pending = true;
-                        continue;
-                    }
-                    pixel_index = py * P.width + px;
-                }
-            }
-        }
-        BT_PROF(1);
-
-        BT_LS(2, __ballot(ev == EV_GEN)); BT_LS(3, __ballot(ev == EV_DIFFUSE)); BT_LS(4, __ballot(ev == EV_METALLIC));
-        BT_LS(5, __ballot(ev == EV_GLASS)); BT_LS(6, __ballot(ev == EV_VOLUME));
-        const uint32_t k_now = packed ? (park_i >> LOG_PXB) & P.row_mask : park_i >> LOG_PXB;
-        const uint32_t sample_index = sample0 + k_now;
-        const U4 u = philox(pixel_index, sample_index, ev == EV_GEN ? 0u : event, 0u, P.seed_lo, P.seed_hi);
-        const uint32_t w1 = ev == EV_METALLIC ? u.x : (ev == EV_GLASS ? u.y : u.z);
-        const uint32_t w2 = ev == EV_METALLIC ? u.y : (ev == EV_GLASS ? u.z : u.w);
-        const float r1 = uniform_sample(w1, 0.0f, P.tau_scale), r2 = uniform_sample(w2, 0.0f, P.one_scale);
-        bool vol_scatter = false;
-        if (VOLS && ev == EV_VOLUME) {
-            const float density = P.vbox_lds_bytes ? march_density_box(P, S, vol_index, vbox[hit_prim], pos)
-                                                   : march_density(P, S, vol_index, prim_c, prim_radius, pos);
-            vol_scatter = density >= 1.0f || bernoulli(u.x, density);
-        }
-        const bool wave_needs_dir = !VOLS || !BT_SKIP_DIR || __ballot(ev != EV_VOLUME || vol_scatter) != 0ull;
-        float sn = 0.0f, cs = 0.0f;
-        if (wave_needs_dir) sincos_bt(r1, sn, cs);
-        BT_PROF(2);
-
-        V3 new_o = pos, dir = rd;
-        bool late_end = false;
-
-        if (ev == EV_GEN) {
-            float u_sub = 0.0f, v_sub = 0.0f;
-            if (P.subsample_n > 1) {
-                const uint32_t n = (uint32_t)P.subsample_n;
-                const uint32_t subpx = k_now % (n * n);
-                const float width_sub = 1.0f / (float)n;
-                u_sub = (float)(subpx % n) * width_sub;
-                v_sub = (float)(subpx / n) * width_sub;
-            }
-            typedef const __attribute__((address_space(4))) BtLaunch BtLaunchK;
-            BtLaunchK *C = (BtLaunchK *)__builtin_amdgcn_kernarg_segment_ptr();
-            asm volatile("" : "+s"(C));
-            const V3 mcx = mk(C->cam_cx.x, C->cam_cx.y, C->cam_cx.z), mcy = mk(C->cam_cy.x, C->cam_cy.y, C->cam_cy.z),
-                     mcz = mk(C->cam_cz.x, C->cam_cz.y, C->cam_cz.z);
-            const float v0 = (float)py * C->pixel_height - 1.0f;
-            const float u0 = (float)px * C->pixel_width - 1.0f;
-            const float u_offset = u_sub * C->pixel_width + uniform_sample(u.x, C->jitter_u_lo, C->jitter_u_scale);
-            const float v_offset = v_sub * C->pixel_height + uniform_sample(u.y, C->jitter_v_lo, C->jitter_v_scale);
-            const float uu = u0 + u_offset, vv = v0 + v_offset;
-            const float yrot = C->xfov * 0.5f * -uu;
-            const float xrot = C->yfov * 0.5f * -vv;
-            float sy, cy, sx, cx;
-            sincos_small_bt(yrot, sy, cy);
-            sincos_small_bt(xrot, sx, cx);
-            const V3 d_cam = mk(-(cx * sy), sx, -(cx * cy));
-            new_o = mk(C->cam_t.x, C->cam_t.y, C->cam_t.z) + mk(0.0f, 0.0f, 0.0f);
-            dir = normalize_or_zero(xf_vector(mcx, mcy, mcz, d_cam));
-            if (C->has_focus) {
-                const V3 d1 = normalize(dir);
-                const V3 defocus = (mk(C->disk_x.x, C->disk_x.y, C->disk_x.z) * cs + mk(C->disk_y.x, C->disk_y.y, C->disk_y.z) * sn) * r2;
-                const V3 defocus_offset = xf_vector(mcx, mcy, mcz, defocus * C->aperture);
-                const float frac_f_z = C->focus / fabsf(d_cam.z);
-                new_o = new_o + defocus_offset;
-                dir = d1 * frac_f_z - defocus_offset;
-            }
-            beta = mk(1, 1, 1);
-            L = mk(0, 0, 0);
-            bounce = 0; vbounce = 0; last_object = -1;
-            event = 1;
-            have_first = false;
-            first = mk(0, 0, 0);
-            first_depth = __builtin_inff();
-            BT_PROF(3);
-        } else {
-            event += 1;
-            const BtMaterial &M = S.materials[mat_index];
-            int light_index = 0;
-            bool to_light = false;
-            if (ev == EV_DIFFUSE) {
-                light_index = (int)__umulhi(u.x, (uint32_t)P.n_lights);
-                to_light = bernoulli(u.y, 0.5f);
-            }
-            const bool is_cosine = ev == EV_DIFFUSE && !to_light;
-            const bool in_frame_of_normal = is_cosine || ev == EV_METALLIC || ev == EV_GLASS;
-            V3 v = mk(0.0f, 0.0f, 0.0f);
-            if (wave_needs_dir) {
-                const float sq = sqrt_bt(is_cosine ? r2 : r2 * (1.0f - r2));
-                const float lx_ = (is_cosine ? cs : cs * 2.0f) * sq;
-                const float ly_ = (is_cosine ? sn : sn * 2.0f) * sq;
-                float lz_ = in_frame_of_normal ? 1.0f - r2 : 1.0f - 2.0f * r2;
-                if (is_cosine) lz_ = sqrt_bt(1.0f - r2);
-                v = mk(lx_, ly_, lz_);
-                if (in_frame_of_normal) {
-                    V3 z_axis = normalize(normal), x_axis, y_axis;
-                    orthonormal_pair(z_axis, x_axis, y_axis);
-                    v = (x_axis * lx_ + y_axis * ly_) + z_axis * lz_;
-                }
-            }
-
-            if (ev == EV_DIFFUSE) {
-                if (to_light) {
-                    const BtLight &Lt = S.lights[light_index];
-                    V3 point;
-                    if (Lt.kind == BT_LIGHT_SPHERE) {
-                        point = mk(Lt.centre) + v * Lt.radius;
-                    } else if (RECTS && Lt.kind == BT_LIGHT_RECT) {
-                        point = face_random_point(S.faces[Lt.face_first], u.z, u.w);
-                    } else if (RECTS && Lt.kind == BT_LIGHT_CUBOID) {
-                        const U4 e = philox(pixel_index, sample_index, event - 1u, 1u, P.seed_lo, P.seed_hi);
-                        const float chosen = uniform_sample(e.x, 0.0f, Lt.total_scale);
-                        int index = 0;
-#pragma unroll
-                        for (int f = 0; f < 5; ++f)
-                            if (Lt.cum[f] <= chosen) index = f + 1;
-                        point = face_random_point(S.faces[Lt.face_first + index], u.z, u.w);
-                    } else {
-                        point = mk(Lt.centre);
-                    }
-                    dir = point - pos;
-                } else {
-                    dir = v;
-                }
-            } else if (ev == EV_METALLIC) {
-                dir = reflect(rd, normal) + v * M.roughness;
-            } else if (ev == EV_GLASS) {
-                const float ior = front ? M.inv_ior : M.ior;
-                const float cos_theta = fminf(dot(-rd, normal), 1.0f);
-                const float sin_theta = sqrt_bt(1.0f - cos_theta * cos_theta);
-                const float fr = fresnel(rd, normal, ior);
-                V3 base;
-                if (ior * sin_theta > 1.0f || bernoulli(u.x, fr))
-                    base = reflect(rd, normal);
-                else
-                    base = refract(rd, normal, ior);
-                dir = base + v * M.roughness;
-            } else if (VOLS) {
-                if (vol_scatter) {
-                    if (inside) new_o = pos - (rd * P.volume_step) * u24(u.y);
-                    dir = v;
-                    beta = beta * mk(0.8f, 0.8f, 0.8f);
-                    if (AOV && !have_first) {
-                        have_first = true;
-                        if (OUTPUT == 1) first = mk(0.8f, 0.8f, 0.8f);
-                        if (OUTPUT == 2) first = normal;
-                        if (OUTPUT == 3) first_depth = hit_depth;
-                        if (GUIDED) park_guides(mk(0.8f, 0.8f, 0.8f), normal, hit_depth);
-                    }
-                }
-                if (vol_back) {
-                    bounce += 1;
-                    last_object = -1;
-                } else {
-                    last_object = pobject;
-                    vbounce += 1;
-                }
-            }
-        }
-
-        BT_PROF(4);
-        const V3 nd = normalize(dir);
-
-        if (ev == EV_DIFFUSE || ev == EV_METALLIC || ev == EV_GLASS) {
-            const BtMaterial &M = S.materials[mat_index];
-            bool scatter = true;
-            float weight = 1.0f;
-            if (ev == EV_DIFFUSE) {
-                const BtLight &Lt = S.lights[(int)__umulhi(u.x, (uint32_t)P.n_lights)];
-                const float pd = dot(normal, nd) * 0.318309886183790671538f;
-                const float plight = P.n_lights == 1 ? light_pdf_only_light<RECTS>(P, S, pos, nd) : light_pdf<RECTS>(P, Lt, S, pos, nd);
-                const float p = lerpf(pd, plight, 0.5f);
-                scatter = !(fabsf(p) <= 1e-5f);
-                weight = pd / p;
-            }
-            if (AOV && !have_first) {
-                have_first = true;
-                if (scatter) {
-                    if (OUTPUT == 1) first = mk(M.albedo);
-                    if (OUTPUT == 2) first = normal;
-                    if (OUTPUT == 3) first_depth = hit_depth;
-                    if (GUIDED) park_guides(mk(M.albedo), normal, hit_depth);
-                } else {
-                    if (OUTPUT == 1) first = mk(M.emitted);
-                    if (GUIDED) park_guides(mk(M.emitted), mk(0, 0, 0), __builtin_inff());
-                }
-            }
-            if (scatter) {
-                beta = beta * (mk(M.albedo) * weight);
-                bounce += 1;
-                last_object = -1;
-            } else {
-                late_end = true;
-            }
-        }
-        ro = new_o;
-        rd = nd;
-
-        if (!late_end) late_end = (VOLS && last_object >= 0) ? (vbounce > P.max_volume_bounces) : (bounce > P.max_bounces);
-        if (late_end) {
-            if (GUIDED && !have_first) park_guide_defaults();
-            finish_sample();
-            pending = true;
-        }
-        BT_PROF(5);
+#include "bt_path_body.inc"
         } while (0);
+        if constexpr (BT_CAN_END_GAME) {
+            if (__ballot(dry_lane) != 0ull) {
+                typedef const __attribute__((address_space(4))) BtLaunch BtLaunchK;
+                BtLaunchK *C = (BtLaunchK *)__builtin_amdgcn_kernarg_segment_ptr();
+                asm volatile("" : "+s"(C));
+                if (C->pool_records || dry_lane) break;
+            }
+        }
         if (compacting && __ballot(dry_lane) != 0ull) {
             dry_lane = true;
             {
@@ -795,6 +567,23 @@
             drain_it += 1u;
         }
     }
+    if constexpr (BT_CAN_END_GAME) if (P.pool_records) {
+        const uint32_t last = bt_end_game(ro.x, ro.y, ro.z, rd.x, rd.y, rd.z, beta.x, beta.y, beta.z, L.x, L.y, L.z, event, pixel_index,
+                                          park_i, bounce, held_t, held_info, (pending ? 1u : 0u) | (held ? 2u : 0u), segments,
+                                          (uint32_t)(uintptr_t)(__attribute__((address_space(3))) unsigned char *)smem,
+                                          (uint32_t)(uintptr_t)__builtin_amdgcn_kernarg_segment_ptr(),
+                                          (uint32_t)((uintptr_t)__builtin_amdgcn_kernarg_segment_ptr() >> 32));
+        if (__builtin_amdgcn_readfirstlane((int)last)) {
+            typedef const __attribute__((address_space(4))) BtLaunch BtLaunchK;
+            BtLaunchK *C = (BtLaunchK *)__builtin_amdgcn_kernarg_segment_ptr();
+            asm volatile("" : "+s"(C));
+            const BtLaunch &Q = *(const BtLaunch *)C;
+            const BlockGeom g = block_geom(Q);
+            const uint32_t t = (uint32_t)Q.samples * (uint32_t)(Q.subsample_n * Q.subsample_n);
+            sum_block(Q, g, blockIdx.x, t, (const Parked *)Q.scratch + (size_t)blockIdx.x * (size_t)(g.pxb * t), threadIdx.x & 63u, Q.out);
+        }
+        return;
+    }
 queue_empty:;
 
     if (P.counters) {
diff --git a/bendy_tracer_amd/csrc/bt_path_body.inc b/bendy_tracer_amd/csrc/bt_path_body.inc
--- /dev/null
+++ b/bendy_tracer_amd/csrc/bt_path_body.inc
@@ -0,0 +1,383 @@
+        if (compacting && dry_lane && pending) continue;
+        BT_LS(0, 1ull);
+        BT_LS(8, ls_all & ~__ballot(true));
+        BT_PROF(0);
+        int ev = EV_GEN;
+        V3 pos = ro, normal = mk(0, 0, 0);
+        float hit_depth = 0.0f;
+        bool front = false, inside = false, vol_back = false;
+        int pobject = -1, mat_index = 0, vol_index = 0;
+        V3 prim_c = mk(0, 0, 0);
+        float prim_radius = 0.0f;
+        int hit_prim = 0;
+
+        BT_LS(1, __ballot(!pending && !(VOTE && held)));
+        if (!pending) {
+            const bool marching = VOLS && last_object >= 0;
+            if (!marching) vbounce = 0;
+            const float tmin = marching ? 0.0f : P.clip_min;
+            const float tmax = marching ? P.volume_step : P.clip_max;
+            HitRec h;
+            bool ended = false, captured = false;
+            float travelled = 0.0f;
+            if (LENS && !marching) {
+                if (!bent) {
+                    lens_begin(P, lens);
+                    bent = true;
+                    segments += 1;
+                }
+                const int r = lens_advance<RECTS>(P, ro, rd, lens, h, BT_LENS_BATCH, lens_steps);
+                if (r == 2) continue;
+                bent = false;
+                captured = r < 0;
+                travelled = lens.travelled;
+            } else if (VOTE && held) {
+                h.t = held_t;
+                h.prim = held_info & 0x1fffffff;
+                h.inside = (held_info >> 29) & 1;
+                h.p_neg = (held_info >> 30) & 1;
+            } else {
+                segments += 1;
+                h = intersect<RECTS, VOLS, RECTS && !VOLS && !LENS>(P, ro, rd, tmin, tmax, last_object);
+            }
+            if (captured) {
+                ended = true;
+            } else if (h.prim < 0) {
+                L = L + beta * mk(P.root_color);
+                if (AOV && !have_first) {
+                    have_first = true;
+                    if (OUTPUT == 1) first = mk(P.root_albedo);
+                    if (OUTPUT == 2) first = P.root_has_albedo ? -rd : mk(0, 0, 0);
+                    if (OUTPUT == 3) first_depth = P.root_has_albedo ? P.clip_max : __builtin_inff();
+                    if (GUIDED) park_guides(mk(P.root_albedo), P.root_has_albedo ? -rd : mk(0, 0, 0), P.root_has_albedo ? P.clip_max : __builtin_inff());
+                }
+                ended = true;
+            } else {
+                const BtPrimLite &pl = S.lite[h.prim];
+                const int pshape = pl.kind_object & 0xff;
+                pobject = pl.kind_object >> 8;
+                prim_c = mk(pl.c);
+                prim_radius = pl.radius;
+                hit_prim = h.prim;
+                hit_depth = LENS ? h.t + travelled : h.t;
+                pos = ro + rd * h.t;
+                bool vol_face = false;
+                if (VOLS && h.inside) {
+                    inside = true;
+                    vol_face = true;
+                } else if (!RECTS || pshape == BT_PRIM_SPHERE) {
+                    V3 nrm = pos - prim_c;
+                    const float nax = fabsf(nrm.x), nay = fabsf(nrm.y), naz = fabsf(nrm.z), rr = pl.rcp_radius;
+                    const bool in_range = (rr != 0.0f) & (nax == 0.0f || (nax >= 0x1p-60f && nax <= 0x1p60f)) &
+                                          (nay == 0.0f || (nay >= 0x1p-60f && nay <= 0x1p60f)) & (naz == 0.0f || (naz >= 0x1p-60f && naz <= 0x1p60f));
+                    if (__ballot(!in_range) == 0ull)
+                        nrm = mk(div_refined(nrm.x, pl.radius, rr), div_refined(nrm.y, pl.radius, rr), div_refined(nrm.z, pl.radius, rr));
+                    else
+                        nrm = mk(nrm.x / pl.radius, nrm.y / pl.radius, nrm.z / pl.radius);
+                    front = dot(rd, nrm) < 0.0f;
+                    normal = front ? nrm : -nrm;
+                    vol_face = VOLS && pl.volume >= 0;
+                    vol_back = vol_face && !front;
+                } else {
+                    front = h.p_neg;
+                    normal = front ? prim_c : -prim_c;
+                }
+                if (vol_face) {
+                    vol_index = pl.volume;
+                    ev = EV_VOLUME;
+                } else {
+                    mat_index = pl.material;
+                    const BtMaterial &M = S.materials[mat_index];
+                    if (!(VOTE && held)) L = L + beta * mk(M.emitted);
+                    if (M.kind == BT_MAT_DIFFUSE) ev = EV_DIFFUSE;
+                    else if (M.kind == BT_MAT_METALLIC) ev = EV_METALLIC;
+                    else if (M.kind == BT_MAT_GLASS) ev = EV_GLASS;
+                    else {
+                        if (AOV && !have_first) {
+                            have_first = true;
+                            if (OUTPUT == 1) first = mk(M.emitted);
+                            if (GUIDED) park_guides(mk(M.emitted), mk(0, 0, 0), __builtin_inff());
+                        }
+                        ended = true;
+                    }
+                }
+            }
+            if (GUIDED && ended && !have_first) park_guide_defaults();
+            if (ended) finish_sample();
+#ifdef BT_END_GAME_BODY
+            held = false;
+#else
+            if (VOTE && P.phase_vote && ev != EV_GEN) {
+                held_t = h.t;
+                held_info = h.prim | ((int)h.inside << 29) | ((int)h.p_neg << 30);
+            }
+#endif
+        }
+        pending = false;
+        if (compacting && dry_lane && ev == EV_GEN) {
+            pending = true;
+            continue;
+        }
+
+#ifndef BT_END_GAME_BODY
+        if (VOTE && P.phase_vote) {
+            const bool want_gen = ev == EV_GEN;
+            const unsigned long long m_gen = __ballot(want_gen), m_sc = __ballot(!want_gen);
+            const uint32_t n_gen = popc64(m_gen), n_sc = popc64(m_sc);
+            const unsigned long long starving = __ballot(waited >= P.phase_vote);
+            const bool run_gen = n_gen >= n_sc || (starving & m_gen) != 0;
+            const bool run_sc = n_sc > n_gen || (starving & m_sc) != 0;
+            const unsigned long long served_m = (run_gen ? m_gen : 0ull) | (run_sc ? m_sc : 0ull);
+            const bool served = __builtin_amdgcn_inverse_ballot_w64(served_m);
+            BT_LS(7, __ballot(!served));
+            if (!served) {
+                waited += 1;
+                pending = want_gen;
+                held = !want_gen;
+                continue;
+            }
+            waited = 0;
+            held = false;
+        }
+
+        {
+            const unsigned long long need = __ballot(ev == EV_GEN);
+            if (need) {
+                const int leader = __ffsll((long long)need) - 1;
+                uint32_t base = 0;
+                if ((int)lane == leader) base = atomicAdd(&s_next_item, popc64(need));
+                base = (uint32_t)__builtin_amdgcn_readlane((int)base, leader);
+                if (ev == EV_GEN) {
+                    const uint32_t i = base + lanes_below(need);
+                    if (i >= n_items) {
+                        if constexpr (BT_CAN_END_GAME) {
+                            dry_lane = true;
+                            pending = true;
+                            continue;
+                        } else {
+                        if (!compacting) goto queue_empty;
+                        dry_lane = true;
+                        pending = true;
+                        continue;
+                        }
+                    }
+                    park_i = i;
+                    BlockRef B_i = B_own;
+                    bool hole = false;
+                    if (packed) {
+                        const uint32_t row = i >> LOG_PXB;
+                        B_i = block_ref(P, G, blockIdx.x + (row >> P.log_rows) * gridDim.x);
+                        hole = (row & P.row_mask) >= T;
+                    }
+                    const PixelRef r = pixel_of(P, G, B_i, i & (pxb - 1u));
+                    px = r.px;
+                    py = r.py;
+                    if (!r.in_frame || hole) {
+                        pending = true;
+                        continue;
+                    }
+                    pixel_index = py * P.width + px;
+                }
+            }
+        }
+#endif
+        BT_PROF(1);
+
+        BT_LS(2, __ballot(ev == EV_GEN)); BT_LS(3, __ballot(ev == EV_DIFFUSE)); BT_LS(4, __ballot(ev == EV_METALLIC));
+        BT_LS(5, __ballot(ev == EV_GLASS)); BT_LS(6, __ballot(ev == EV_VOLUME));
+        const uint32_t k_now = packed ? (park_i >> LOG_PXB) & P.row_mask : park_i >> LOG_PXB;
+        const uint32_t sample_index = sample0 + k_now;
+        const U4 u = philox(pixel_index, sample_index, ev == EV_GEN ? 0u : event, 0u, P.seed_lo, P.seed_hi);
+        const uint32_t w1 = ev == EV_METALLIC ? u.x : (ev == EV_GLASS ? u.y : u.z);
+        const uint32_t w2 = ev == EV_METALLIC ? u.y : (ev == EV_GLASS ? u.z : u.w);
+        const float r1 = uniform_sample(w1, 0.0f, P.tau_scale), r2 = uniform_sample(w2, 0.0f, P.one_scale);
+        bool vol_scatter = false;
+        if (VOLS && ev == EV_VOLUME) {
+            const float density = P.vbox_lds_bytes ? march_density_box(P, S, vol_index, vbox[hit_prim], pos)
+                                                   : march_density(P, S, vol_index, prim_c, prim_radius, pos);
+            vol_scatter = density >= 1.0f || bernoulli(u.x, density);
+        }
+        const bool wave_needs_dir = !VOLS || !BT_SKIP_DIR || __ballot(ev != EV_VOLUME || vol_scatter) != 0ull;
+        float sn = 0.0f, cs = 0.0f;
+        if (wave_needs_dir) sincos_bt(r1, sn, cs);
+        BT_PROF(2);
+
+        V3 new_o = pos, dir = rd;
+        bool late_end = false;
+
+#ifndef BT_END_GAME_BODY
+        if (ev == EV_GEN) {
+            float u_sub = 0.0f, v_sub = 0.0f;
+            if (P.subsample_n > 1) {
+                const uint32_t n = (uint32_t)P.subsample_n;
+                const uint32_t subpx = k_now % (n * n);
+                const float width_sub = 1.0f / (float)n;
+                u_sub = (float)(subpx % n) * width_sub;
+                v_sub = (float)(subpx / n) * width_sub;
+            }
+            typedef const __attribute__((address_space(4))) BtLaunch BtLaunchK;
+            BtLaunchK *C = (BtLaunchK *)__builtin_amdgcn_kernarg_segment_ptr();
+            asm volatile("" : "+s"(C));
+            const V3 mcx = mk(C->cam_cx.x, C->cam_cx.y, C->cam_cx.z), mcy = mk(C->cam_cy.x, C->cam_cy.y, C->cam_cy.z),
+                     mcz = mk(C->cam_cz.x, C->cam_cz.y, C->cam_cz.z);
+            const float v0 = (float)py * C->pixel_height - 1.0f;
+            const float u0 = (float)px * C->pixel_width - 1.0f;
+            const float u_offset = u_sub * C->pixel_width + uniform_sample(u.x, C->jitter_u_lo, C->jitter_u_scale);
+            const float v_offset = v_sub * C->pixel_height + uniform_sample(u.y, C->jitter_v_lo, C->jitter_v_scale);
+            const float uu = u0 + u_offset, vv = v0 + v_offset;
+            const float yrot = C->xfov * 0.5f * -uu;
+            const float xrot = C->yfov * 0.5f * -vv;
+            float sy, cy, sx, cx;
+            sincos_small_bt(yrot, sy, cy);
+            sincos_small_bt(xrot, sx, cx);
+            const V3 d_cam = mk(-(cx * sy), sx, -(cx * cy));
+            new_o = mk(C->cam_t.x, C->cam_t.y, C->cam_t.z) + mk(0.0f, 0.0f, 0.0f);
+            dir = normalize_or_zero(xf_vector(mcx, mcy, mcz, d_cam));
+            if (C->has_focus) {
+                const V3 d1 = normalize(dir);
+                const V3 defocus = (mk(C->disk_x.x, C->disk_x.y, C->disk_x.z) * cs + mk(C->disk_y.x, C->disk_y.y, C->disk_y.z) * sn) * r2;
+                const V3 defocus_offset = xf_vector(mcx, mcy, mcz, defocus * C->aperture);
+                const float frac_f_z = C->focus / fabsf(d_cam.z);
+                new_o = new_o + defocus_offset;
+                dir = d1 * frac_f_z - defocus_offset;
+            }
+            beta = mk(1, 1, 1);
+            L = mk(0, 0, 0);
+            bounce = 0; vbounce = 0; last_object = -1;
+            event = 1;
+            have_first = false;
+            first = mk(0, 0, 0);
+            first_depth = __builtin_inff();
+            BT_PROF(3);
+        } else
+#endif
+        {
+            event += 1;
+            const BtMaterial &M = S.materials[mat_index];
+            int light_index = 0;
+            bool to_light = false;
+            if (ev == EV_DIFFUSE) {
+                light_index = (int)__umulhi(u.x, (uint32_t)P.n_lights);
+                to_light = bernoulli(u.y, 0.5f);
+            }
+            const bool is_cosine = ev == EV_DIFFUSE && !to_light;
+            const bool in_frame_of_normal = is_cosine || ev == EV_METALLIC || ev == EV_GLASS;
+            V3 v = mk(0.0f, 0.0f, 0.0f);
+            if (wave_needs_dir) {
+                const float sq = sqrt_bt(is_cosine ? r2 : r2 * (1.0f - r2));
+                const float lx_ = (is_cosine ? cs : cs * 2.0f) * sq;
+                const float ly_ = (is_cosine ? sn : sn * 2.0f) * sq;
+                float lz_ = in_frame_of_normal ? 1.0f - r2 : 1.0f - 2.0f * r2;
+                if (is_cosine) lz_ = sqrt_bt(1.0f - r2);
+                v = mk(lx_, ly_, lz_);
+                if (in_frame_of_normal) {
+                    V3 z_axis = normalize(normal), x_axis, y_axis;
+                    orthonormal_pair(z_axis, x_axis, y_axis);
+                    v = (x_axis * lx_ + y_axis * ly_) + z_axis * lz_;
+                }
+            }
+
+            if (ev == EV_DIFFUSE) {
+                if (to_light) {
+                    const BtLight &Lt = S.lights[light_index];
+                    V3 point;
+                    if (Lt.kind == BT_LIGHT_SPHERE) {
+                        point = mk(Lt.centre) + v * Lt.radius;
+                    } else if (RECTS && Lt.kind == BT_LIGHT_RECT) {
+                        point = face_random_point(S.faces[Lt.face_first], u.z, u.w);
+                    } else if (RECTS && Lt.kind == BT_LIGHT_CUBOID) {
+                        const U4 e = philox(pixel_index, sample_index, event - 1u, 1u, P.seed_lo, P.seed_hi);
+                        const float chosen = uniform_sample(e.x, 0.0f, Lt.total_scale);
+                        int index = 0;
+#pragma unroll
+                        for (int f = 0; f < 5; ++f)
+                            if (Lt.cum[f] <= chosen) index = f + 1;
+                        point = face_random_point(S.faces[Lt.face_first + index], u.z, u.w);
+                    } else {
+                        point = mk(Lt.centre);
+                    }
+                    dir = point - pos;
+                } else {
+                    dir = v;
+                }
+            } else if (ev == EV_METALLIC) {
+                dir = reflect(rd, normal) + v * M.roughness;
+            } else if (ev == EV_GLASS) {
+                const float ior = front ? M.inv_ior : M.ior;
+                const float cos_theta = fminf(dot(-rd, normal), 1.0f);
+                const float sin_theta = sqrt_bt(1.0f - cos_theta * cos_theta);
+                const float fr = fresnel(rd, normal, ior);
+                V3 base;
+                if (ior * sin_theta > 1.0f || bernoulli(u.x, fr))
+                    base = reflect(rd, normal);
+                else
+                    base = refract(rd, normal, ior);
+                dir = base + v * M.roughness;
+            } else if (VOLS) {
+                if (vol_scatter) {
+                    if (inside) new_o = pos - (rd * P.volume_step) * u24(u.y);
+                    dir = v;
+                    beta = beta * mk(0.8f, 0.8f, 0.8f);
+                    if (AOV && !have_first) {
+                        have_first = true;
+                        if (OUTPUT == 1) first = mk(0.8f, 0.8f, 0.8f);
+                        if (OUTPUT == 2) first = normal;
+                        if (OUTPUT == 3) first_depth = hit_depth;
+                        if (GUIDED) park_guides(mk(0.8f, 0.8f, 0.8f), normal, hit_depth);
+                    }
+                }
+                if (vol_back) {
+                    bounce += 1;
+                    last_object = -1;
+                } else {
+                    last_object = pobject;
+                    vbounce += 1;
+                }
+            }
+        }
+
+        BT_PROF(4);
+        const V3 nd = normalize(dir);
+
+        if (ev == EV_DIFFUSE || ev == EV_METALLIC || ev == EV_GLASS) {
+            const BtMaterial &M = S.materials[mat_index];
+            bool scatter = true;
+            float weight = 1.0f;
+            if (ev == EV_DIFFUSE) {
+                const BtLight &Lt = S.lights[(int)__umulhi(u.x, (uint32_t)P.n_lights)];
+                const float pd = dot(normal, nd) * 0.318309886183790671538f;
+                const float plight = P.n_lights == 1 ? light_pdf_only_light<RECTS>(P, S, pos, nd) : light_pdf<RECTS>(P, Lt, S, pos, nd);
+                const float p = lerpf(pd, plight, 0.5f);
+                scatter = !(fabsf(p) <= 1e-5f);
+                weight = pd / p;
+            }
+            if (AOV && !have_first) {
+                have_first = true;
+                if (scatter) {
+                    if (OUTPUT == 1) first = mk(M.albedo);
+                    if (OUTPUT == 2) first = normal;
+                    if (OUTPUT == 3) first_depth = hit_depth;
+                    if (GUIDED) park_guides(mk(M.albedo), normal, hit_depth);
+                } else {
+                    if (OUTPUT == 1) first = mk(M.emitted);
+                    if (GUIDED) park_guides(mk(M.emitted), mk(0, 0, 0), __builtin_inff());
+                }
+            }
+            if (scatter) {
+                beta = beta * (mk(M.albedo) * weight);
+                bounce += 1;
+                last_object = -1;
+            } else {
+                late_end = true;
+            }
+        }
+        ro = new_o;
+        rd = nd;
+
+        if (!late_end) late_end = (VOLS && last_object >= 0) ? (vbounce > P.max_volume_bounces) : (bounce > P.max_bounces);
+        if (late_end) {
+            if (GUIDED && !have_first) park_guide_defaults();
+            finish_sample();
+            pending = true;
+        }
+        BT_PROF(5);
diff --git a/bendy_tracer_amd/csrc/bt_plan.hpp b/bendy_tracer_amd/csrc/bt_plan.hpp
--- a/bendy_tracer_amd/csrc/bt_plan.hpp
+++ b/bendy_tracer_amd/csrc/bt_plan.hpp
@@ -66,6 +66,12 @@
     return held.bytes == need;
 }
 
+inline uint32_t workgroups_per_cu(size_t lds, uint32_t cap) {
+    return std::max(1u, std::min(cap, 160u * 1024u / (uint32_t)((lds + 64 + 2047) & ~(size_t)2047)));
+}
+constexpr uint32_t kEndGameResident = 8;
+constexpr size_t kEndGameCounterBytes = 32;
+
 enum { PLAIN = 0, GUIDED = 1, ADAPTIVE = 2 };
 
 struct Plan {
@@ -74,6 +80,7 @@
     uint32_t chunk = 0;
     uint32_t launches = 0;
     size_t lds_bytes = 0;
+    uint32_t resident = 0;
     uint64_t guide_values[3] = {};
     uint64_t parked_bytes = 0;
     uint64_t pixels = 0;
@@ -195,6 +202,16 @@
             return BT_ERR_DEVICE;
         }
     }
+    plan.resident = workgroups_per_cu(lds_bytes, 7);
+    if (P.wg_blocks <= 1 && output == 0 && !P.any_rects && !P.any_volumes && !P.lens_on) {
+        const size_t with_pool = pool_offset + pool_bytes + kEndGameCounterBytes;
+        plan.resident = workgroups_per_cu(lds_bytes, kEndGameResident);
+        if (tune.endgame == 2 && workgroups_per_cu(with_pool, kEndGameResident) == plan.resident) {
+            P.pool_records = BT_POOL_RECORDS;
+            P.pool_lds_offset = (uint32_t)pool_offset;
+            lds_bytes = with_pool;
+        }
+    }
     plan.parked_bytes = px_launch * T_all * sample_bytes;
     if (guided) {
         uint64_t plane = values * 3;
diff --git a/bendy_tracer_amd/csrc/bt_types.h b/bendy_tracer_amd/csrc/bt_types.h
--- a/bendy_tracer_amd/csrc/bt_types.h
+++ b/bendy_tracer_amd/csrc/bt_types.h
@@ -7,6 +7,8 @@
 #else
 #define BT_N_COUNTERS 2
 #endif
+#define BT_COUNTER_EG_MOVED 14
+#define BT_COUNTER_EG_WORKGROUPS 15
 #define BT_DENSITY_LDS_MAX 8192
 
 struct BtV3 { float x, y, z; };
diff --git a/include/bendy_hip.h b/include/bendy_hip.h
--- a/include/bendy_hip.h
+++ b/include/bendy_hip.h
@@ -70,7 +70,7 @@
     int32_t phase_vote;
     uint64_t scratch_cap_bytes;
     int32_t packed;
-    int32_t reserved;
+    int32_t endgame;
 } bt_tuning;
 
 typedef struct {
@@ -117,6 +117,8 @@
 int bt_debug_plan_launch(bt_scene *scene, uint64_t camera_ref, const bt_config *config, const bt_render_config *render,
                          uint32_t width, uint32_t height, uint32_t rank, uint32_t world, int32_t sharded, uint32_t n_cu,
                          int32_t pass_kind, uint32_t guides, uint64_t alloc_limit, bt_stats *out);
+int bt_debug_plan_lds(const bt_scene *scene, uint32_t out[4]);
+int bt_debug_end_game_counts(bt_scene *scene, uint64_t out[2]);
 
 
 int bt_render(bt_scene *scene, uint64_t camera_ref, const bt_config *config, const bt_render_config *render,
```

After: 56190 Msamples/s. 0.966x the previous value.
